# wubinzzu/NeuRec

Measured on AMD Instinct MI355X. Metric: BPR triplets/sec (LightGCN-gowalla), higher is better.
Workload: dtype f32; 1 GPU; LightGCN on synthetic gowalla-shaped interactions (U=29858, I=40981, E=813886), 3 layers, dim 64, B=1024 per GPU, adj=pre, Adam lr=0.01 reg=1e-3; global_batch=1024, parallelism=single GPU

## Files before the change

### include/neurec_hip.h

```cpp
#ifndef NEUREC_HIP_H
#define NEUREC_HIP_H

#include <stddef.h>
#include <stdint.h>

#ifdef __cplusplus
extern "C" {
#endif

#define NRHIP_OK 0
#define NRHIP_ERR_ARG 1
#define NRHIP_ERR_UNSUPPORTED 2
#define NRHIP_ERR_HIP 3
#define NRHIP_ERR_WORKSPACE 4

#define NRHIP_ABI_VERSION 4
#define NRHIP_MAX_TOPK 128

int nrhip_abi_version(void);
const char* nrhip_last_error(void);
int nrhip_device_info(int* cu_count, int* clock_khz, size_t* hbm_bytes, char* name, int name_len);


int nrhip_eval_workspace_bytes(int rows, int top_k, size_t* bytes);
// ... 38 lines not shown

int nrhip_tile_strike_plan(const int64_t* d_indptr, const int32_t* d_indices, int n_users, int cols,
                           int32_t* d_plan_user, uint32_t* d_plan_mask, int64_t* d_tile_ptr, int32_t* d_chunk_tile,
                           int64_t* d_chunk_begin, int32_t* d_counts, void* d_ws, size_t ws_bytes, void* stream);
int nrhip_score_filter_workspace_bytes(int rows, int cols, int d, size_t* bytes);
int nrhip_score_filter_kappa(int d, float* kappa);
int nrhip_score_filter_prepare_items(const float* d_Q, int64_t ldq, int cols, int d, void* d_ws, size_t ws_bytes,
                                     int max_rows, void* stream);
int nrhip_score_filter_tilemax(const float* d_P, int64_t ldp, const int32_t* d_users, int rows, int cols, int d,
                               float* d_M, int64_t mld, float* d_eps, void* d_ws, size_t ws_bytes, int max_rows,
                               void* stream);
int nrhip_score_filter_i8_workspace_bytes(int rows, int cols, int d, size_t* bytes);
int nrhip_score_filter_i8_prepare_items(const float* d_Q, int64_t ldq, int cols, int d, void* d_ws, size_t ws_bytes,
                                        int max_rows, void* stream);
int nrhip_score_filter_i8_tilemax(const float* d_P, int64_t ldp, const int32_t* d_users, int rows, int cols, int d,
                                  float* d_M, int64_t mld, float* d_eps, void* d_ws, size_t ws_bytes, int max_rows,
                                  void* stream);
int nrhip_eval_tiles_workspace_bytes(int rows, int top_k, size_t* bytes);
int nrhip_score_gemm_items_kmajor(const void* d_ws, int cols, int d, const float** qt, int* ipad);
int nrhip_eval_tiles(const float* d_M, int64_t mld, const float* d_P, int64_t ldp,
                     const void* d_gemm_ws, int d, const int32_t* d_users, int rows, int cols,
                     const int64_t* d_tr_indptr, const int32_t* d_tr_indices,
                     const int64_t* d_truth_indptr, const int32_t* d_truth_indices,
                     const int32_t* metric_ids_host, int n_metric, int top_k, float* d_out,
                     int32_t* d_flag_out, void* d_ws, size_t ws_bytes, void* stream);
int nrhip_eval_tiles_bounded_workspace_bytes(int rows, int cols, int top_k, int n_keep, size_t* bytes);
int nrhip_eval_tiles_bounded(const float* d_M, int64_t mld, const float* d_eps, int n_keep, const float* d_P,
                             int64_t ldp, const void* d_gemm_ws, int d, const int32_t* d_users, int rows, int cols,
                             const int64_t* d_tr_indptr, const int32_t* d_tr_indices,
                             const int64_t* d_truth_indptr, const int32_t* d_truth_indices,
                             const int32_t* metric_ids_host, int n_metric, int top_k, float* d_out,
                             int32_t* d_flag_out, void* d_ws, size_t ws_bytes, void* stream);

typedef struct nrhip_eval_pruned_args {
  const float* d_P; int64_t ldp;
  const float* d_Q; int64_t ldq;
  int d, cols;
  const int32_t* d_users; int n_users, batch_rows;
  const int64_t* d_tr_indptr; const int32_t* d_tr_indices;
  const int64_t* d_truth_indptr; const int32_t* d_truth_indices;
  const int32_t* d_chunk_tile; const int64_t* d_chunk_begin; int n_chunks;
  const int64_t* d_tile_ptr; const int32_t* d_plan_user; const uint32_t* d_plan_mask;
  const int32_t* d_row_of;
  const int32_t* metric_ids; int n_metric, top_k, n_keep;
  int use_filter, prepare_items;
  void* d_gemm_ws; size_t gemm_ws_bytes;
  void* d_filter_ws; size_t filter_ws_bytes;
  void* d_tiles_ws; size_t tiles_ws_bytes;
  float* d_M; int64_t mld;
  float* d_eps;
  float* d_out;
  int32_t* d_flags;
  double* d_sums;
  void* d_colsum_ws; size_t colsum_ws_bytes;
} NrhipEvalPruned;
int nrhip_eval_pruned(const NrhipEvalPruned* args, void* stream);

typedef struct nrhip_eval_redo_args {
  const NrhipEvalPruned* ev;
  int n_flagged;
  int reload_items;
  float* d_scores; int64_t lds; int slab_rows;
  int32_t* d_rows;
  int32_t* d_row_users;
  int32_t* d_count;
  float* d_fixed;
  void* d_ws; size_t ws_bytes;
} NrhipEvalRedo;
int nrhip_eval_redo(const NrhipEvalRedo* args, void* stream);

int nrhip_sample_bpr_epoch(const int64_t* d_tr_indptr, const int32_t* d_tr_indices,
                           const int32_t* d_row_of, int64_t n_inter, int n_items, int neg_num,
                           uint64_t seed, uint64_t epoch, int shuffle, int64_t out_begin,
                           int64_t out_count, int32_t* d_users_out, int32_t* d_pos_out,
                           int32_t* d_neg_out, void* stream);

int nrhip_sample_instances_epoch(const int64_t* d_seq_ptr, const int32_t* d_seq,
                                 const int64_t* d_excl_ptr, const int32_t* d_excl,
                                 const int64_t* d_inst_ptr, const int32_t* d_inst_row,
                                 const int32_t* d_row_user, int64_t n_inst, int high_order,
                                 int n_items, int neg_num, int pointwise, uint64_t seed,
                                 uint64_t epoch, int shuffle, int64_t out_begin, int64_t out_count,
                                 int32_t* d_users_out, int32_t* d_recent_out, int32_t* d_items_out,
                                 int32_t* d_neg_out, float* d_labels_out, void* stream);

int nrhip_randint_choice_batch(int high, int n_req, int64_t total, const int64_t* d_out_offsets,
                               const int64_t* d_excl_indptr, const int32_t* d_excl, int replace,
                               uint64_t seed, uint64_t call_counter, int32_t* d_out, void* stream);

int nrhip_bpr_plan(const int32_t* d_users, const int32_t* d_items, const int32_t* d_third,
                   int64_t n_total, int batch, int n_users, uint64_t* d_plan_out, void* stream);
int nrhip_bpr_mf_grad(const float* d_P, const float* d_Q, int d, int n_users,
                      const int32_t* d_users, const int32_t* d_pos, const int32_t* d_neg, int batch,
                      float reg, float* d_GP, float* d_GQ, float* d_work, float* d_loss2,
                      const uint64_t* d_plan, void* stream);
int nrhip_adam_sparse_tf(float* d_var, float* d_m, float* d_v, float* d_grad, int64_t n,
                         float alpha, float beta1, float beta2, float eps, void* stream);
int nrhip_adam_sparse_tf_lazy(float* d_var, float* d_m, float* d_v, float* d_grad, int32_t* d_last,
                              const int32_t* d_stamp, int64_t n_rows, int d, const uint64_t* d_plan,
                              int n_occ, const uint64_t* d_next_plan, int n_next_occ,
                              const float* d_alpha_tab, int t, int period, float beta1, float beta2,
                              float eps, void* stream);
int nrhip_bpr_mf_grad_lazy(const float* d_table, const float* d_m, const float* d_v,
                           const int32_t* d_last, const float* d_alpha_tab, int32_t* d_stamp, int t,
                           float beta1, float beta2, float eps, int d, int n_users,
                           const int32_t* d_users, const int32_t* d_pos, const int32_t* d_neg, int batch,
                           float reg, float* d_G, float* d_work, float* d_loss2, const uint64_t* d_plan,
                           void* stream);
int nrhip_adam_dense_tf(float* d_var, float* d_m, float* d_v, float* d_grad, int64_t n,
                        float alpha, float beta1, float beta2, float eps, int clear_grad,
                        void* stream);

int nrhip_adam_dense_tf2(float* d_var, float* d_m, float* d_v, const float* d_grad_a,
                         const float* d_grad_b, int64_t n, float alpha, float beta1, float beta2,
                         float eps, void* stream);
int nrhip_adam_dense_tf_multi(int n_tensors, float* const* d_vars_host, float* const* d_ms_host,
                              float* const* d_vs_host, float* const* d_grads_host,
                              const int64_t* sizes_host, const int32_t* clear_grad_host, float alpha,
                              float beta1, float beta2, float eps, void* stream);
int nrhip_rows_div(const int32_t* d_rows, int n_listed, int d, const float* d_src, float denom,
                   float* d_dst, void* stream);
int nrhip_rows_clear(const int32_t* d_rows, int n_listed, int d, float* d_b0, float* d_b1,
                     float* d_b2, float* d_b3, uint8_t* d_flag, void* stream);

int nrhip_spmm_plan_bytes(int64_t n_rows, int64_t nnz, size_t* bytes);
int nrhip_spmm_plan_create(const int64_t* h_indptr, int64_t n_rows, int item_rows, int item_nnz,
                           int64_t split_row, void* d_plan_buf, size_t plan_bytes, void* stream,
                           void** plan_out);
int nrhip_spmm_plan_destroy(void* plan);
int nrhip_spmm_plan_info(const void* plan, int64_t* n_work_items, int64_t* n_split_rows);
int nrhip_spmm_workspace_bytes(const void* plan, int d, size_t* bytes);
int nrhip_spmm_csr(const void* plan, const int64_t* d_indptr, const int32_t* d_indices,
                   const float* d_vals, const float* d_X, int d, float* d_Y,
                   const float* d_addend, const float* d_sum_in, float* d_sum_out, void* d_ws,
                   size_t ws_bytes, void* stream);

int nrhip_spmm_csr_masked(const void* plan, const int64_t* d_indptr, const int32_t* d_indices,
                          const float* d_vals, const float* d_X, const uint8_t* d_x_row_nonzero,
                          const uint8_t* d_y_row_wanted, int d, float* d_Y, const float* d_addend,
                          const float* d_sum_in, float* d_sum_out, void* d_ws, size_t ws_bytes,
                          void* stream);
int nrhip_spmm_blocked_plan_bytes(int64_t n_rows, int64_t nnz, int d, size_t* bytes);
int nrhip_spmm_blocked_plan_create(const int64_t* h_indptr, const int32_t* h_indices,
                                   int64_t n_rows, int64_t split_row, int d, int64_t block_bytes,
                                   int n_workgroups, int waves_per_wg, int seg_len, int r_max,
                                   int p_max, void* d_plan_buf, size_t plan_bytes, void* stream,
                                   void** plan_out);
int nrhip_spmm_blocked_plan_destroy(void* plan);
int nrhip_spmm_blocked_plan_info(const void* plan, int* n_workgroups, int* n_phases,
                                 int64_t* n_entries, int64_t* n_split);
int nrhip_spmm_blocked_tune(int gathers_in_flight);
int nrhip_spmm_blocked_tune_store(int masked_store);
int nrhip_spmm_blocked_pack(void* plan, const int32_t* d_indices, const float* d_vals, void* stream);
int nrhip_spmm_blocked(const void* plan, const int32_t* d_indices, const float* d_vals,
                       const float* d_X, float* d_Y, const float* d_addend, const float* d_sum_in,
                       float* d_sum_out, const uint8_t* d_x_row_nonzero,
                       const uint8_t* d_y_row_wanted, void* stream);
int nrhip_spmm_blocked_flagged(const void* plan, const int32_t* d_indices, const float* d_vals,
                               const float* d_X, float* d_Y, const float* d_addend,
                               const uint8_t* d_addend_row_flag, const float* d_sum_in, float* d_sum_out,
                               const uint8_t* d_x_row_nonzero, const uint8_t* d_y_row_wanted, void* stream);
int nrhip_spmm_csr_flagged(const void* plan, const int64_t* d_indptr, const int32_t* d_indices,
                           const float* d_vals, const float* d_X, int d, float* d_Y,
                           const float* d_addend, const uint8_t* d_addend_row_flag, const float* d_sum_in,
                           float* d_sum_out, void* d_ws, size_t ws_bytes, void* stream);
int nrhip_spmm_blocked_tune_addend_flag(int on);
int nrhip_spmm_plan_attach_blocked(void* plan, const void* blocked_plan, int d);

int nrhip_spmm_csr_adam(const void* plan, const int32_t* d_indices, const float* d_vals,
                        const float* d_X, int d, float* d_addend, float* d_grad_b, float* d_var,
                        float* d_m, float* d_v, float alpha, float beta1, float beta2, float eps,
                        int clear_consumed, uint8_t* d_row_flag, void* stream);
int nrhip_spmm_blocked_adam(const void* plan, const int32_t* d_indices, const float* d_vals,
                            const float* d_X, float* d_addend, float* d_grad_b, float* d_var,
                            float* d_m, float* d_v, float alpha, float beta1, float beta2,
                            float eps, int clear_consumed, uint8_t* d_row_flag, void* stream);
int nrhip_spmm_plan_has_blocked(const void* plan, int d);

int nrhip_spmm_csr_wanted_layers(const void* plan, const int32_t* d_indices, const float* d_vals,
                                 const float* d_X, int d, const float* d_sum_in,
                                 const float* d_layer_a, const float* d_layer_b, float* d_sum_out,
                                 const uint8_t* d_y_row_wanted, void* stream);
int nrhip_spmm_blocked_wanted_layers(const void* plan, const int32_t* d_indices, const float* d_vals,
                                     const float* d_X, const float* d_sum_in, const float* d_layer_a,
                                     const float* d_layer_b, float* d_sum_out,
                                     const uint8_t* d_y_row_wanted, void* stream);
int nrhip_spmm_csr_wanted_batch(const void* plan, const int32_t* d_indices, const float* d_vals,
                                const float* d_X, int d, const float* d_sum_in, const float* d_layer_a,
                                const float* d_layer_b, float* d_sum_out, const int32_t* d_users,
                                const int32_t* d_pos, const int32_t* d_neg, int batch, int n_users,
                                uint8_t* d_row_flag, int32_t* d_rows_out, void* stream);
int nrhip_spmm_blocked_wanted_batch(const void* plan, const int32_t* d_indices, const float* d_vals,
                                    const float* d_X, const float* d_sum_in, const float* d_layer_a,
                                    const float* d_layer_b, float* d_sum_out, const int32_t* d_users,
                                    const int32_t* d_pos, const int32_t* d_neg, int batch, int n_users,
                                    uint8_t* d_row_flag, int32_t* d_rows_out, void* stream);
int nrhip_spmm_plan_has_wanted(const void* plan, int d);
int nrhip_spmm_blocked_has_wanted(const void* blocked_plan);
int nrhip_spmm_plan_has_wanted_planned(const void* plan, int d);
int nrhip_spmm_blocked_has_wanted_planned(const void* blocked_plan);
int nrhip_spmm_wanted_epoch_plan_bytes(const void* plan, int d, int batch, int64_t n_batches, size_t* bytes,
                                       int* stride);
int nrhip_spmm_blocked_wanted_epoch_plan_bytes(const void* blocked_plan, int batch, int64_t n_batches, size_t* bytes,
                                               int* stride);
int nrhip_spmm_wanted_epoch_plan(const void* plan, int d, const int64_t* d_indptr, const uint64_t* d_plans, int batch,
                                 int64_t n_batches, int last_len, void* d_sched, size_t sched_bytes, void* stream);
int nrhip_spmm_blocked_wanted_epoch_plan(const void* blocked_plan, const int64_t* d_indptr, const uint64_t* d_plans,
                                         int batch, int64_t n_batches, int last_len, void* d_sched, size_t sched_bytes,
                                         void* stream);
int nrhip_spmm_csr_wanted_planned(const void* plan, const int32_t* d_indices, const float* d_vals, const float* d_X,
                                  int d, const float* d_sum_in, const float* d_layer_a, const float* d_layer_b,
                                  float* d_sum_out, const int32_t* d_users, const int32_t* d_pos, const int32_t* d_neg,
                                  int batch, int n_users, uint8_t* d_row_flag, int32_t* d_rows_out,
                                  const void* d_batch_sched, int stride, void* stream);
int nrhip_spmm_blocked_wanted_planned(const void* blocked_plan, const int32_t* d_indices, const float* d_vals,
                                      const float* d_X, const float* d_sum_in, const float* d_layer_a,
                                      const float* d_layer_b, float* d_sum_out, const int32_t* d_users,
                                      const int32_t* d_pos, const int32_t* d_neg, int batch, int n_users,
                                      uint8_t* d_row_flag, int32_t* d_rows_out, const void* d_batch_sched, int stride,
                                      void* stream);

int nrhip_spmm_csr_carry(const void* plan, const int64_t* d_indptr, const int32_t* d_indices, const float* d_vals,
                         const float* d_X, const float* d_X2, int x_split, int d, float* d_Yv, int has_carry,
                         const uint8_t* d_row_mask, void* stream);
int nrhip_spmm_chunks_finish(const int32_t* d_first_vrow, int64_t n_rows, const float* d_Yv, int d, float* d_Y,
                             const float* d_addend, const float* d_sum_in, float* d_sum_out,
                             const uint8_t* d_row_mask, void* stream);

int nrhip_partials_sum_rows(const float* d_parts, int world, int64_t n_rows, int d, float* d_Y, const float* d_addend,
                            const float* d_sum_in, float* d_sum_out, const uint8_t* d_row_mask, void* stream);

int nrhip_spmm_csr_rows(const int64_t* d_indptr, const int32_t* d_indices, const float* d_vals,
                        const float* d_X, int d, const int32_t* d_rows, int n_listed, float* d_Y,
                        const float* d_addend, const float* d_sum_in, float* d_sum_out,
                        void* stream);

int nrhip_lightgcn_bpr_grad(const float* d_Esum, const float* d_E0, int n_users, int d,
                            int n_layers, const int32_t* d_users, const int32_t* d_pos,
                            const int32_t* d_neg, int batch, float reg, float* d_Gstar,
                            float* d_Greg, float* d_work, float* d_loss2, const uint64_t* d_plan,
                            void* stream);

int nrhip_lightgcn_bpr_grad_h(const float* d_Esum, const float* d_E0, int n_users, int d,
                              int n_layers, const int32_t* d_users, const int32_t* d_pos,
                              const int32_t* d_neg, int batch, float reg, float* d_H,
                              float* d_Greg, float* d_work, float* d_loss2, const uint64_t* d_plan,
                              void* stream);

int nrhip_lightgcn_mark_batch(const int32_t* d_users, const int32_t* d_pos, const int32_t* d_neg,
                              int batch, int n_users, int32_t* d_rows_out, uint8_t* d_row_flag,
                              void* stream);

typedef struct nrhip_lightgcn_buffers {
  const void* plan;
  const void* plan_t;
  const int64_t* indptr;  const int32_t* indices;  const float* vals;
  const int64_t* indptr_t; const int32_t* indices_t; const float* vals_t;
  float* E0; float* m; float* v;
  float* Ea; float* Eb; float* Esum; float* Esum_rows;
  float* Gstar; float* Greg; float* H; float* Ga; float* Gb;
  int32_t* batch_rows;
  uint8_t* row_flag;
  float* terms;
  void* spmm_ws; size_t spmm_ws_bytes;
  int n_users; int n_nodes; int d; int n_layers; int max_batch;
  float reg;
} nrhip_lightgcn_buffers;
int nrhip_lightgcn_ctx_create(const nrhip_lightgcn_buffers* bufs, void** ctx_out);
int nrhip_lightgcn_ctx_destroy(void* ctx);
int nrhip_lightgcn_step(void* ctx, const int32_t* d_users, const int32_t* d_pos,
                        const int32_t* d_neg, int batch, const uint64_t* d_plan, float alpha,
                        float beta1, float beta2, float eps, float* d_loss2, void* stream);
int nrhip_lightgcn_step_planned(void* ctx, const int32_t* d_users, const int32_t* d_pos, const int32_t* d_neg,
                                int batch, const uint64_t* d_plan, const void* d_hop_sched, int hop_stride,
                                float alpha, float beta1, float beta2, float eps, float* d_loss2, void* stream);

int nrhip_lightgcn_step_colshard_fwd(void* ctx, const int32_t* d_users, const int32_t* d_pos, const int32_t* d_neg,
                                     int batch, float* d_partials, void* stream);
int nrhip_lightgcn_step_colshard_fwd_planned(void* ctx, const int32_t* d_users, const int32_t* d_pos,
                                             const int32_t* d_neg, int batch, const void* d_hop_sched, int hop_stride,
                                             float* d_partials, void* stream);
int nrhip_lightgcn_step_colshard_bwd(void* ctx, const int32_t* d_users, const int32_t* d_pos, const int32_t* d_neg,
                                     int batch, const uint64_t* d_plan, const float* d_given, float alpha,
                                     float beta1, float beta2, float eps, float* d_loss2, void* stream);
int nrhip_lightgcn_partial_dots(const float* d_Esum, const float* d_E0, int n_users, int d, int n_layers,
                                const int32_t* d_users, const int32_t* d_pos, const int32_t* d_neg, int batch,
                                float* d_out, void* stream);
int nrhip_partials_sum(const float* d_parts, int world, int n, float* d_given, void* stream);
int nrhip_lightgcn_bpr_grad_given(const float* d_Esum, const float* d_E0, int n_users, int d, int n_layers,
                                  const int32_t* d_users, const int32_t* d_pos, const int32_t* d_neg, int batch,
                                  float reg, float* d_Gstar, float* d_Greg, float* d_work, float* d_loss2,
                                  const uint64_t* d_plan, const float* d_given, int divided, void* stream);
int nrhip_lightgcn_step_grad(void* ctx, const int32_t* d_users, const int32_t* d_pos,
                             const int32_t* d_neg, int batch, const uint64_t* d_plan,
                             float* d_loss2, float* d_grad_out, void* stream);
int nrhip_lightgcn_step_apply(void* ctx, float* d_grad, float alpha, float beta1, float beta2,
                              float eps, void* stream);

typedef struct nrhip_mf_buffers {
  float* P; float* Q; float* mP; float* vP; float* mQ; float* vQ; float* GP; float* GQ;
  float* terms;
  int n_users; int n_items; int d; int max_batch;
  float reg;
  int32_t* last; int32_t* stamp; const float* alpha_tab; int alpha_len; int lazy_period;
  int32_t* tw; int32_t* inb;
} nrhip_mf_buffers;
// ... 643 lines not shown
```

### neurec_amd/_lib.py

```python
import ctypes as C
import os

from . import build as _build

_HERE = os.path.dirname(os.path.abspath(__file__))
LIB_PATH = os.path.join(_HERE, "libneurec_hip.so")

ERR_ARG, ERR_UNSUPPORTED, ERR_HIP, ERR_WORKSPACE = 1, 2, 3, 4


class NeuRecHipError(RuntimeError):
    """A HIP runtime failure or workspace error reported by the native library."""


def _load():
    if not os.path.isfile(LIB_PATH):
        raise ImportError(
            "libneurec_hip.so is not built (expected at %s). Run `python -m neurec_amd.build` "
            "(needs hipcc; the engine has no CPU fallback)." % LIB_PATH)
    if os.path.isfile(_build.STAMP) and not _build.is_current() and not os.environ.get("NEUREC_ALLOW_STALE_LIB"):
        raise ImportError(
            "libneurec_hip.so was built from other sources than neurec_amd/csrc now holds (digest in %s differs). "
            "Run `python -m neurec_amd.build`; NEUREC_ALLOW_STALE_LIB=1 loads it anyway." % _build.STAMP)
    try:
# ... 160 lines not shown
    _fields_ = [(n, C.c_void_p) for n in (
        "UI", "IU", "IL", "LI", "W", "b", "h", "G_UI", "G_IU", "G_IL", "G_LI", "G_W", "G_b", "G_h", "flag_UI",
        "flag_IU", "flag_IL", "flag_LI", "users", "recents", "items", "third", "keys", "contrib", "scal", "delta",
        "partial", "loss2")] + \
        [(n, C.c_int) for n in ("n_users", "n_items", "d", "w", "L", "batch", "pairwise", "loss_kind")] + \
        [("reg_mf", C.c_float), ("reg_w", C.c_float)]


class FpmcplusScoresArgs(C.Structure):
    _fields_ = [(n, C.c_void_p) for n in (
        "UI", "IU", "IL", "LI", "W", "b", "h", "last", "users", "c", "p", "out")] + [("ld", C.c_int64)] + \
        [(n, C.c_int) for n in ("n_users", "n_items", "d", "w", "L", "batch")]


class TransrecStepArgs(C.Structure):
    _fields_ = [(n, C.c_void_p) for n in (
        "P", "Q", "b", "T", "G_P", "G_Q", "G_b", "G_T", "flag_P", "flag_Q", "flag_b", "users", "recent", "items",
        "third", "keys", "scal", "partial", "loss2")] + \
        [(n, C.c_int) for n in ("n_users", "n_items", "d", "batch", "pairwise", "loss_kind")] + [("reg", C.c_float)]


GRU4REC_MAX_LAYERS = 3


class Gru4recWeights(C.Structure):
    _fields_ = [(n, C.c_void_p * GRU4REC_MAX_LAYERS) for n in ("Wg", "bg", "Wc", "bc")] + [("width", C.c_int * GRU4REC_MAX_LAYERS),
                                                                          ("n_layers", C.c_int), ("hidden_act", C.c_int)]


class Gru4recStepArgs(C.Structure):
    _fields_ = [(n, C.c_void_p) for n in ("Ein", "Q", "b")] + [("w", Gru4recWeights)] + \
        [(n, C.c_void_p) for n in ("G_Ein", "G_Q", "G_b")] + \
        [(n, C.c_void_p * GRU4REC_MAX_LAYERS) for n in ("G_Wg", "G_bg", "G_Wc", "G_bc", "state", "h_new")] + \
        [(n, C.c_void_p) for n in ("X", "Y", "keys", "ws", "loss2")] + \
        [(n, C.c_int) for n in ("n_items", "batch", "final_act", "loss_kind")] + [("reg", C.c_float)]


SIGNATURES = {
    "nrhip_device_info": [C.POINTER(i32), C.POINTER(i32), psz, C.c_char_p, i32],
    "nrhip_eval_workspace_bytes": [i32, i32, psz],
    "nrhip_mask_train": [p, i64, p, i32, i32, p, p, p],
    "nrhip_eval_scores": [p, i64, i32, i32, p, p, p, C.POINTER(i32), i32, i32, p, p, p, p, sz, p],
    "nrhip_eval_any_k_workspace_bytes": [i32, i32, i32, psz],
    "nrhip_eval_scores_any_k": [p, i64, i32, i32, p, p, p, C.POINTER(i32), i32, i32, p, p, p, sz, p],
    "nrhip_arg_topk": [p, i64, i32, i32, i32, p, p, p, sz, p],
    "nrhip_colsum_workspace_bytes": [i32, i32, psz],
    "nrhip_colsum_f64": [p, i64, i32, i32, p, p, sz, p],
    "nrhip_score_gemm_workspace_bytes": [i32, i32, i32, psz],
    "nrhip_score_gemm_prepare_items": [p, i64, i32, i32, p, sz, p],
    "nrhip_score_tilemax": [p, i64, p, i32, i32, i32, p, p, p, i64, p, sz, p],
    "nrhip_tile_strike_plan": [p, p, i32, i32, p, p, p, p, p, p, p, sz, p],
    "nrhip_score_tilemax_fix": [p, i64, i32, i32, p, p, i32, p, p, p, p, i32, i32, p, i64, p, sz, p],
    "nrhip_score_filter_workspace_bytes": [i32, i32, i32, psz],
    "nrhip_score_filter_kappa": [i32, p],
    "nrhip_score_filter_prepare_items": [p, i64, i32, i32, p, sz, i32, p],
    "nrhip_score_filter_tilemax": [p, i64, p, i32, i32, i32, p, i64, p, p, sz, i32, p],
    "nrhip_score_filter_i8_workspace_bytes": [i32, i32, i32, psz],
    "nrhip_score_filter_i8_prepare_items": [p, i64, i32, i32, p, sz, i32, p],
    "nrhip_score_filter_i8_tilemax": [p, i64, p, i32, i32, i32, p, i64, p, p, sz, i32, p],
    "nrhip_eval_tiles_workspace_bytes": [i32, i32, psz],
    "nrhip_eval_tiles": [p, i64, p, i64, p, i32, p, i32, i32, p, p, p, p, p, i32, i32, p, p, p, sz, p],
    "nrhip_eval_tiles_bounded_workspace_bytes": [i32, i32, i32, i32, psz],
    "nrhip_eval_tiles_bounded": [p, i64, p, i32, p, i64, p, i32, p, i32, i32, p, p, p, p, p, i32, i32, p, p, p, sz, p],
    "nrhip_eval_pruned": [C.POINTER(EvalPrunedArgs), p],
    "nrhip_eval_redo": [C.POINTER(EvalRedoArgs), p],
    "nrhip_vae_step": [C.POINTER(VaeStepArgs), p, i32, f32, f32, f32, u64, i32, i32, p],
    "nrhip_score_gemm_items_kmajor": [p, i32, i32, p, p],
    "nrhip_score_gemm": [p, i64, p, i32, i32, i32, p, i64, p, sz, p],
    "nrhip_sample_bpr_epoch": [p, p, p, i64, i32, i32, u64, u64, i32, i64, i64, p, p, p, p],
    "nrhip_sample_instances_epoch": [p, p, p, p, p, p, p, i64, i32, i32, i32, i32, u64, u64, i32, i64, i64, p, p, p, p, p, p],
    "nrhip_randint_choice_batch": [i32, i32, i64, p, p, p, i32, u64, u64, p, p],
    "nrhip_bpr_plan": [p, p, p, i64, i32, i32, p, p],
    "nrhip_bpr_mf_grad": [p, p, i32, i32, p, p, p, i32, f32, p, p, p, p, p, p],
    "nrhip_adam_sparse_tf": [p, p, p, p, i64, f32, f32, f32, f32, p],
    "nrhip_adam_dense_tf": [p, p, p, p, i64, f32, f32, f32, f32, i32, p],
    "nrhip_adam_dense_tf2": [p, p, p, p, p, i64, f32, f32, f32, f32, p],
    "nrhip_adam_dense_tf_multi": [i32, p, p, p, p, p, p, f32, f32, f32, f32, p],
    "nrhip_rows_div": [p, i32, i32, p, f32, p, p],
    "nrhip_rows_clear": [p, i32, i32, p, p, p, p, p, p],
    "nrhip_spmm_plan_bytes": [i64, i64, psz],
    "nrhip_spmm_plan_create": [p, i64, i32, i32, i64, p, sz, p, C.POINTER(p)],
    "nrhip_spmm_plan_destroy": [p],
    "nrhip_spmm_plan_info": [p, C.POINTER(i64), C.POINTER(i64)],
    "nrhip_spmm_workspace_bytes": [p, i32, psz],
    "nrhip_spmm_csr": [p, p, p, p, p, i32, p, p, p, p, p, sz, p],
    "nrhip_spmm_csr_masked": [p, p, p, p, p, p, p, i32, p, p, p, p, p, sz, p],
    "nrhip_spmm_csr_carry": [p, p, p, p, p, p, i32, i32, p, i32, p, p],
    "nrhip_spmm_chunks_finish": [p, i64, p, i32, p, p, p, p, p, p],
    "nrhip_partials_sum_rows": [p, i32, i64, i32, p, p, p, p, p, p],
    "nrhip_spmm_csr_rows": [p, p, p, p, i32, p, i32, p, p, p, p, p],
    "nrhip_lightgcn_mark_batch": [p, p, p, i32, i32, p, p, p],
    "nrhip_lightgcn_bpr_grad": [p, p, i32, i32, i32, p, p, p, i32, f32, p, p, p, p, p, p],
    "nrhip_lightgcn_bpr_grad_h": [p, p, i32, i32, i32, p, p, p, i32, f32, p, p, p, p, p, p],
    "nrhip_lightgcn_ctx_create": [C.POINTER(LightGCNBuffers), C.POINTER(p)],
    "nrhip_lightgcn_ctx_destroy": [p],
    "nrhip_lightgcn_step": [p, p, p, p, i32, p, f32, f32, f32, f32, p, p],
    "nrhip_lightgcn_step_grad": [p, p, p, p, i32, p, p, p, p],
    "nrhip_lightgcn_step_apply": [p, p, f32, f32, f32, f32, p],
    "nrhip_mf_ctx_create": [C.POINTER(MFBuffers), C.POINTER(p)],
    "nrhip_mf_ctx_destroy": [p],
    "nrhip_mf_step": [p, p, p, p, i32, p, p, i32, i32, f32, f32, f32, f32, p, p],
    "nrhip_mf_flush": [p, i32, f32, f32, f32, p],
    "nrhip_ngcf_ctx_create": [C.POINTER(NGCFBuffers), C.POINTER(p)],
    "nrhip_ngcf_ctx_destroy": [p],
    "nrhip_ngcf_forward": [p, C.c_uint64, C.c_uint64, i32, p],
    "nrhip_ngcf_step": [p, p, p, p, i32, p, C.c_uint64, C.c_uint64, i32, f32, f32, f32, f32, p, p],
    "nrhip_mf_steps": [p, p, p, p, i64, i32, p, i32, p, f32, f32, f32, p, p, p],
    "nrhip_loss_reduce_steps": [p, i32, i32, i32, f32, p, p],
    "nrhip_lightgcn_step_colshard_fwd": [p, p, p, p, i32, p, p],
    "nrhip_lightgcn_step_colshard_fwd_planned": [p, p, p, p, i32, p, i32, p, p],
    "nrhip_lightgcn_step_planned": [p, p, p, p, i32, p, p, i32, f32, f32, f32, f32, p, p],
    "nrhip_lightgcn_step_colshard_bwd": [p, p, p, p, i32, p, p, f32, f32, f32, f32, p, p],
    "nrhip_lightgcn_partial_dots": [p, p, i32, i32, i32, p, p, p, i32, p, p],
    "nrhip_partials_sum": [p, i32, i32, p, p],
    "nrhip_lightgcn_bpr_grad_given": [p, p, i32, i32, i32, p, p, p, i32, f32, p, p, p, p, p, p, i32, p],
    "nrhip_gemm_workspace_bytes": [i32, i32, i32, p],
    "nrhip_gemm_kmajor": [p, i64, p, i64, i32, i32, i32, p, i64, i32, p, i32, i32, p, sz, p],
    "nrhip_gemm_f32": [p, i64, i32, p, i64, i32, i32, i32, i32, p, i64, i32, p, i32, i32, p, sz, p],
    "nrhip_transpose2d": [p, i64, i32, i32, p, i64, p],
    "nrhip_ngcf_wide_forward": [C.POINTER(NGCFWideBuffers), i32, u64, u64, p],
    "nrhip_ngcf_wide_step": [C.POINTER(NGCFWideBuffers), p, p, p, i32, p, i32, u64, u64, f32, f32, f32, f32, p, p],
    "nrhip_vae_bag_fwd": [p, p, p, i32, i32, p, p, i32, f32, p, u64, u64, p, p, p],
    "nrhip_act_bwd": [p, p, i64, i32, p, p],
    "nrhip_vae_sample": [p, i32, i32, p, f32, u64, u64, p, p, p, p],
    "nrhip_vae_sample_bwd": [p, p, p, i32, i32, f32, p, p],
    "nrhip_vae_softmax_dlogits": [p, i64, i32, i32, p, p, p, p, p],
    "nrhip_vae_dwq0_wide": [p, p, p, i32, i32, p, p, p, p],
    "nrhip_colsum_rows": [p, i64, i32, i32, p, p, sz, p],
    "nrhip_ew_mul": [p, i64, p, i64, i64, i32, p, i64, p],
    "nrhip_ngcf_act_fwd": [p, p, i64, i64, i32, i32, f32, p, i32, u64, u64, i32, p, i64, p, i64, p],
    "nrhip_ngcf_act_bwd": [p, i64, p, i64, p, i64, p, p, i64, p, i64, i32, f32, p, p, p],
    "nrhip_lrelu_drop_fwd": [p, i64, i64, i32, i32, f32, p, i32, u64, u64, i32, i32, p, i64, p, i64, p],
    "nrhip_lrelu_drop_bwd": [p, i64, p, i64, p, i64, p, i64, i32, f32, i32, p, p],
    "nrhip_edge_dropout": [p, i64, f32, p, i32, u64, u64, p, p],
    "nrhip_gather_f32": [p, p, i64, p, p],
    "nrhip_ngcf_mix_bwd": [p, p, i64, p, p, i64, i64, i32, i32, p, p, p],
    "nrhip_route_batch": [p, p, p, i32, i32, i32, i32, i32, p, p, p, p, p, i32, p],
    "nrhip_route_owner_keys": [p, p, i32, p, p, i32, i32, i32, p, p, p],
    "nrhip_sort_u64_segments": [p, p, p, i32, i32, p],
    "nrhip_route_epoch": [p, p, p, i64, i32, i32, i32, i32, i32, i32, p, p, p, p, p, p, p, p],
    "nrhip_route_epoch_owner_keys": [p, p, p, i64, p, p, i32, i32, p, p, p, i32, i32, i64, p, p, p],
    "nrhip_bpr_mf_step_fused": [p, p, p, p, p, p, i32, f32, f32, f32, i32, i32, i32, p, p, p, i32, f32, p, p, p,
                                i32, p, i32, i32, p],
    "nrhip_bpr_mf_fused_flush": [p, p, p, p, p, i32, f32, f32, f32, i32, i64, p],
    "nrhip_adam_sparse_tf_lazy": [p, p, p, p, p, p, i64, i32, p, i32, p, i32, p, i32, i32, f32, f32, f32, p],
    "nrhip_bpr_mf_grad_lazy": [p, p, p, p, p, p, i32, f32, f32, f32, i32, i32, p, p, p, i32, f32, p, p, p,
                               p, p],
    "nrhip_ngcf_workspace_bytes": [i64, psz],
    "nrhip_ngcf_layer_fwd": [p, p, p, p, p, p, i64, i32, f32, p, i32, u64, u64, i32, p, p, i64, p],
    "nrhip_ngcf_layer_bwd": [p, p, p, p, p, p, i64, i32, f32, p, p, i64, p, p, p, p, p, p, p, p, p,
                             p, sz, p],
    "nrhip_spmm_blocked_plan_bytes": [i64, i64, i32, psz],
    "nrhip_spmm_blocked_pack": [p, p, p, p],
    "nrhip_spmm_blocked_plan_create": [p, p, i64, i64, i32, i64, i32, i32, i32, i32, i32, p, sz, p,
                                       C.POINTER(p)],
    "nrhip_spmm_blocked_plan_destroy": [p],
    "nrhip_spmm_blocked_plan_info": [p, p, p, p, p],
    "nrhip_spmm_blocked_tune": [i32],
    "nrhip_spmm_blocked_tune_store": [i32],
    "nrhip_spmm_blocked": [p, p, p, p, p, p, p, p, p, p, p],
    "nrhip_spmm_blocked_flagged": [p, p, p, p, p, p, p, p, p, p, p, p],
    "nrhip_spmm_csr_flagged": [p, p, p, p, p, i32, p, p, p, p, p, p, sz, p],
    "nrhip_spmm_blocked_tune_addend_flag": [i32],
    "nrhip_spmm_plan_attach_blocked": [p, p, i32],
    "nrhip_spmm_plan_has_blocked": [p, i32],
    "nrhip_spmm_plan_has_wanted": [p, i32],
    "nrhip_spmm_blocked_has_wanted": [p],
    "nrhip_spmm_plan_has_wanted_planned": [p, i32],
    "nrhip_spmm_blocked_has_wanted_planned": [p],
    "nrhip_spmm_wanted_epoch_plan_bytes": [p, i32, i32, i64, psz, C.POINTER(i32)],
    "nrhip_spmm_blocked_wanted_epoch_plan_bytes": [p, i32, i64, psz, C.POINTER(i32)],
    "nrhip_spmm_wanted_epoch_plan": [p, i32, p, p, i32, i64, i32, p, sz, p],
    "nrhip_spmm_blocked_wanted_epoch_plan": [p, p, p, i32, i64, i32, p, sz, p],
    "nrhip_spmm_csr_wanted_planned": [p, p, p, p, i32, p, p, p, p, p, p, p, i32, i32, p, p, p, i32, p],
    "nrhip_spmm_blocked_wanted_planned": [p, p, p, p, p, p, p, p, p, p, p, i32, i32, p, p, p, i32, p],
    "nrhip_spmm_csr_wanted_layers": [p, p, p, p, i32, p, p, p, p, p, p],
    "nrhip_spmm_blocked_wanted_layers": [p, p, p, p, p, p, p, p, p, p],
    "nrhip_spmm_csr_wanted_batch": [p, p, p, p, i32, p, p, p, p, p, p, p, i32, i32, p, p, p],
    "nrhip_spmm_blocked_wanted_batch": [p, p, p, p, p, p, p, p, p, p, p, i32, i32, p, p, p],
    "nrhip_spmm_csr_adam": [p, p, p, p, i32, p, p, p, p, p, f32, f32, f32, f32, i32, p, p],
    "nrhip_spmm_blocked_adam": [p, p, p, p, p, p, p, p, p, f32, f32, f32, f32, i32, p, p],
    "nrhip_vae_encode": [p, p, p, i32, i32, i32, p, p, p, p, p, p, i32, f32, p, p, f32, u64, u64,
                         p, p, p, p, p, p, p, p, p],
    "nrhip_add_row_bias": [p, i64, i32, i32, p, p],
    "nrhip_vae_workspace_bytes": [i32, i32, psz],
    "nrhip_vae_decoder_loss_grad": [p, i64, i32, i32, i32, p, p, p, p, p, p, p, p, p, p, p, sz, p],
    "nrhip_vae_decoder_fused_workspace_bytes": [i32, i32, psz],
    "nrhip_vae_decoder_fused": [i32, i32, i32, p, p, p, p, p, p, p, p, p, p, p, sz, p, p],
    "nrhip_vae_mid_backward": [i32, i32, i32, i32, f32, p, p, p, p, p, p, p, p, p, p, p, p, p, p,
                               p, p, p, p],
    "nrhip_vae_dwq0": [p, p, p, i32, i32, p, p, p, p],
    "nrhip_axpy": [f32, p, p, i64, p],
    "nrhip_sumsq_accumulate": [p, i64, p, p],
    "nrhip_mean_f32": [p, i32, p, p],
    "nrhip_mean2_f32": [p, p, i32, p, p],
    "nrhip_pairwise_mf_grad": [p, p, i32, i32, p, p, p, i32, f32, i32, p, p, p, p, p, p],
    "nrhip_pointwise_mf_grad": [p, p, i32, i32, p, p, p, i32, f32, i32, p, p, p, p, p, p],
    "nrhip_gather_u8": [p, p, i64, p, p],
    "nrhip_mark_rows": [p, i32, i32, p, p],
    "nrhip_sort_u64": [p, i32, p],
    "nrhip_rows_sum_sorted": [p, i32, p, i32, p, i64, p, p],
    "nrhip_rows_sum_sorted2": [p, i32, p, i32, p, i64, p, p, i64, p, p],
    "nrhip_optimizer_rows_tf": [i32, p, p, p, p, p, i64, i32, f32, f32, f32, f32, p],
    "nrhip_optimizer_dense_tf": [i32, p, p, p, p, i64, f32, f32, f32, f32, i32, p],
    "nrhip_rows_gather": [p, i32, i32, p, p, i64, p],
    "nrhip_rows_gather_ld": [p, i32, i32, p, i64, p, i64, p],
    "nrhip_rows_gather2": [p, i32, i32, p, i64, p, i64, p, i64, p, i64, p],
    "nrhip_rows_scatter_add": [p, i32, i32, p, i64, p, p],
    "nrhip_scale": [p, f32, p, i64, p],
    "nrhip_add": [p, p, p, i64, p],
    "nrhip_div_scalar": [p, f32, p, i64, p],
    "nrhip_add2d": [p, i64, p, i64, p, i64, i64, i32, p],
    "nrhip_copy2d": [p, i64, p, i64, i64, i32, p],
    "nrhip_wrmf_chunk_plan": [p, i32, p, p, C.POINTER(i32)],
    "nrhip_wrmf_workspace_bytes": [i32, i32, psz],
    "nrhip_wrmf_gram": [p, i32, i32, p, p, sz, p],
    "nrhip_wrmf_solve": [p, p, i32, p, i32, p, i32, f32, f32, p, p, i32, p, p, sz, p],
    "nrhip_itemknn_workspace_bytes": [i32, i32, i32, psz],
    "nrhip_itemknn_build": [p, p, p, p, p, p, p, p, i32, i32, i32, f32, f32, f32, i32, i32, p, p, p, p, p, p, p, sz, p],
    "nrhip_itemknn_score": [p, i32, p, p, p, i32, i32, p, p, p, p, i64, p],
    "nrhip_fism_step": [C.POINTER(FismStepArgs), p],
    "nrhip_fism_user_factors": [p, p, i32, p, i32, f32, p, i32, p, i64, p],
    "nrhip_nais_step": [C.POINTER(NaisStepArgs), p],
    "nrhip_nais_scores": [C.POINTER(NaisScoresArgs), p],
    "nrhip_fpmc_step": [C.POINTER(FpmcStepArgs), p],
    "nrhip_fpmc_user_factors": [p, p, i32, i32, i32, p, p, i32, p, i64, p],
    "nrhip_fossil_step": [C.POINTER(FossilStepArgs), p],
    "nrhip_fossil_user_factors": [p, p, i32, i32, p, p, p, p, i32, i32, f32, p, i32, p, i64, p],
    "nrhip_hrm_step": [C.POINTER(HrmStepArgs), p],
    "nrhip_hrm_user_factors": [p, p, i32, i32, i32, i32, i32, i32, p, p, i32, p, i64, p],
    "nrhip_npe_step": [C.POINTER(NpeStepArgs), p],
    "nrhip_npe_user_factors": [p, p, i32, i32, i32, i32, p, p, i32, p, i64, p],
    "nrhip_npe_item_factors": [p, i32, i32, p, p],
    "nrhip_fpmcplus_step": [C.POINTER(FpmcplusStepArgs), p],
    "nrhip_fpmcplus_scores": [C.POINTER(FpmcplusScoresArgs), p],
    "nrhip_transrec_step": [C.POINTER(TransrecStepArgs), p],
    "nrhip_transrec_queries": [p, p, p, i32, i32, i32, p, p, i32, p, i64, p],
    "nrhip_transrec_scores": [p, i64, p, p, i32, i32, i32, p, i64, p],
    "nrhip_gru4rec_workspace_floats": [i32, C.POINTER(i32), i32, psz],
    "nrhip_gru4rec_step": [C.POINTER(Gru4recStepArgs), p],
    "nrhip_gru4rec_advance": [C.POINTER(p), C.POINTER(p), C.POINTER(i32), i32, i32, p, p],
    "nrhip_gru4rec_user_states": [p, p, i32, i32, p, p, i32, p, C.POINTER(Gru4recWeights), p, i64, p],
    "nrhip_gru4rec_scores": [p, i64, p, p, i32, i32, i32, i32, p, i64, p],
}

for _name, _args in SIGNATURES.items():
    _fn = getattr(lib, _name)
    _fn.argtypes = _args
    _fn.restype = C.c_int
lib.nrhip_abi_version.argtypes = []
lib.nrhip_abi_version.restype = C.c_int
lib.nrhip_last_error.argtypes = []
lib.nrhip_last_error.restype = C.c_char_p

EXPORTED = sorted(list(SIGNATURES) + ["nrhip_abi_version", "nrhip_last_error"])

ABI_VERSION = 4
if lib.nrhip_abi_version() != ABI_VERSION:
    raise ImportError("libneurec_hip.so ABI version %d, expected %d"
                      % (lib.nrhip_abi_version(), ABI_VERSION))


def last_error():
    return lib.nrhip_last_error().decode("utf-8", "replace")


def check(rc):
    if rc == 0:
        return
    msg = last_error()
    if rc == ERR_ARG:
        raise ValueError(msg)
    if rc == ERR_UNSUPPORTED:
        raise NotImplementedError(msg)
    raise NeuRecHipError("libneurec_hip status %d: %s" % (rc, msg))


def call(name, *args):
    check(getattr(lib, name)(*args))


def is_stale():
    return not _build.is_current()
```

### neurec_amd/build.py

```python
import hashlib
import os
import subprocess
import sys
from concurrent.futures import ThreadPoolExecutor

HERE = os.path.dirname(os.path.abspath(__file__))
ROOT = os.path.dirname(HERE)
CSRC = os.path.join(HERE, "csrc")
OBJ_DIR = os.path.join(CSRC, "_obj")
LIB_PATH = os.path.join(HERE, "libneurec_hip.so")
STAMP = os.path.join(OBJ_DIR, "sources.sha256")

SOURCES = ["eval_select.hip", "score_gemm.hip", "sampler.hip", "spmm.hip", "bpr.hip", "adam.hip",
           "step.hip", "dense.hip", "vae.hip", "spmm_blocked.hip", "route.hip", "gemm.hip", "vae_wide.hip", "ngcf_wide.hip", "vae_fused.hip",
           "score_bf16.hip", "score_i8.hip", "eval_pipeline.hip", "wrmf.hip", "itemknn.hip", "fism.hip", "nais.hip", "fpmc.hip", "fossil.hip", "hrm.hip",
           "npe.hip", "fpmcplus.hip", "transrec.hip", "gru4rec.hip"]
FILE_FLAGS = {"score_i8.hip": ["-mllvm", "-amdgpu-mfma-vgpr-form"]}
EXP_SOURCES = ["experiments/gather_experiments.hip"]
EXP_LIB_PATH = os.path.join(HERE, "libneurec_exp.so")
HEADERS = ["nr_core.h", "nr_common.h", "history_common.h", "spmm_blocked_plan.h", "spmm_wanted_plan.h"]

HIPCC = os.environ.get("HIPCC", "/opt/rocm/bin/hipcc")
FLAGS = ["-O3", "--offload-arch=gfx950", "-std=c++17", "-fPIC", "-ffp-contract=off",
         "-munsafe-fp-atomics", "-Wall", "-Wno-unused-function",
         "-I", CSRC, "-I", os.path.join(ROOT, "include")] + os.environ.get("NEUREC_HIPCC_EXTRA", "").split()


def _existing_sources():
    return [s for s in SOURCES if os.path.isfile(os.path.join(CSRC, s))]


def _digest():
    h = hashlib.sha256()
    for name in _existing_sources() + HEADERS:
        with open(os.path.join(CSRC, name), "rb") as f:
            h.update(name.encode())
            h.update(f.read())
    with open(os.path.join(ROOT, "include", "neurec_hip.h"), "rb") as f:
        h.update(f.read())
    h.update(" ".join(f.replace(ROOT, "<root>") for f in FLAGS).encode())
    h.update(repr(sorted(FILE_FLAGS.items())).encode())
    return h.hexdigest()


def is_current():
    if not (os.path.isfile(LIB_PATH) and os.path.isfile(STAMP)):
        return False
    with open(STAMP) as f:
        return f.read().strip() == _digest()


def build_extension(force=False, verbose=True):
    if not force and is_current():
        return LIB_PATH
    os.makedirs(OBJ_DIR, exist_ok=True)
    srcs = _existing_sources()

    def compile_one(src):
        obj = os.path.join(OBJ_DIR, src.replace(".hip", ".o"))
        cmd = [HIPCC] + FLAGS + FILE_FLAGS.get(src, []) + ["-c", os.path.join(CSRC, src), "-o", obj]
        r = subprocess.run(cmd, capture_output=True, text=True)
        if r.returncode != 0 and FILE_FLAGS.get(src):
            r2 = subprocess.run([HIPCC] + FLAGS + ["-c", os.path.join(CSRC, src), "-o", obj], capture_output=True, text=True)
            if r2.returncode == 0:
                sys.stderr.write("neurec_amd.build: %s compiled WITHOUT %s (not accepted by this hipcc)\n"
                                 % (src, " ".join(FILE_FLAGS[src])))
                r = r2
        return src, obj, r

    objs = []
    with ThreadPoolExecutor(max_workers=min(8, len(srcs))) as ex:
        for src, obj, r in ex.map(compile_one, srcs):
            if r.returncode != 0:
                raise RuntimeError("hipcc failed on %s:\n%s\n%s" % (src, r.stdout, r.stderr))
            if verbose and r.stderr.strip():
                sys.stderr.write(r.stderr)
            objs.append(obj)
    cmd = [HIPCC, "--offload-arch=gfx950", "-shared", "-fPIC", "-o", LIB_PATH] + objs
    r = subprocess.run(cmd, capture_output=True, text=True)
    if r.returncode != 0:
        raise RuntimeError("link failed:\n%s\n%s" % (r.stdout, r.stderr))
    with open(STAMP, "w") as f:
        f.write(_digest())
    if verbose:
        print("built", LIB_PATH)
    return LIB_PATH


def build_experiments(verbose=True):
    os.makedirs(OBJ_DIR, exist_ok=True)
    objs = []
    for src in EXP_SOURCES:
        obj = os.path.join(OBJ_DIR, os.path.basename(src).replace(".hip", ".o"))
        r = subprocess.run([HIPCC] + FLAGS + ["-c", os.path.join(CSRC, src), "-o", obj],
                           capture_output=True, text=True)
        if r.returncode != 0:
            raise RuntimeError("hipcc failed on %s:\n%s\n%s" % (src, r.stdout, r.stderr))
        objs.append(obj)
    r = subprocess.run([HIPCC, "--offload-arch=gfx950", "-shared", "-fPIC", "-o", EXP_LIB_PATH] + objs +
                       ["-L", HERE, "-lneurec_hip", "-Wl,-rpath,$ORIGIN"], capture_output=True, text=True)
    if r.returncode != 0:
        raise RuntimeError("link failed:\n%s\n%s" % (r.stdout, r.stderr))
    if verbose:
        print("built", EXP_LIB_PATH)
    return EXP_LIB_PATH


if __name__ == "__main__":
    build_extension(force="--force" in sys.argv)
    if "--experiments" in sys.argv:
        build_experiments()
```

### neurec_amd/csrc/spmm_blocked.hip

```cpp
#include "nr_common.h"
#include "spmm_blocked_plan.h"
#include "spmm_wanted_plan.h"
#include <algorithm>
#include <new>
#include <cstdlib>
#include <initializer_list>
#include <vector>

namespace {

using nr_plan::kMaxLdsBytes;
using nr_plan::blocked_plan_bytes;
static_assert((int)nr_plan::kOk == NR_OK && (int)nr_plan::kErrArg == NR_ERR_ARG &&
              (int)nr_plan::kErrUnsupported == NR_ERR_UNSUPPORTED, "the planner returns the C ABI's status codes");

struct BlockedPlan : nr_plan::PlanArrays<int4> {
  int64_t n_rows, nnz, n_ent, n_cmb;
  int n_wg, n_phases;
  int seg, r_max, p_max, waves, d;
  const int32_t* pk_from_idx;
  const float* pk_from_val;
  int nnz_cap, ent_cap;
  int colmask_ok;
  int wanted_ok, w_ent_cap, w_nnz_cap, w_bitmap_words;
  int ww_ok, ww_ent_cap;
  int ww_lds_slots;
  int wp_ok, n_hubs;
  nr_wplan::SlotProfile wp_profile;
};


enum { kStorePlain = 0, kStoreNt = 1, kStoreWt = 2 };
typedef float nr_f32x4 __attribute__((ext_vector_type(4)));
typedef unsigned int nr_u32x4 __attribute__((ext_vector_type(4)));

template <int ST>
__device__ __forceinline__ void row_store(float4* __restrict__ Y, uint32_t y_bytes, int64_t o, float4 y) {
  if constexpr (ST == kStoreNt) {
    __builtin_nontemporal_store(nr_f32x4{y.x, y.y, y.z, y.w}, (nr_f32x4*)(Y + o));
  } else if constexpr (ST == kStoreWt) {
    const __amdgpu_buffer_rsrc_t rs = __builtin_amdgcn_make_buffer_rsrc((void*)Y, 0, (int)y_bytes, 0x00020000);
    __builtin_amdgcn_raw_buffer_store_b128(nr_u32x4{__float_as_uint(y.x), __float_as_uint(y.y), __float_as_uint(y.z),
                                                    __float_as_uint(y.w)},
                                           rs, (int)(uint32_t)(o * 16), 0, 16);
  } else {
    Y[o] = y;
  }
}


struct AdamEpilogue {
  float4* var; float4* m; float4* v; const float4* grad_b;
  float alpha, omb1, omb2, eps;
  float4* addend_rw; float4* grad_b_rw; uint8_t* flag_rw;
};


constexpr int kRowBits = 0x7FFFFFFF;
constexpr int kRowUnflagged = (int)0x80000000u;

template <bool MASKED, bool ADAM, int LPR>
__device__ __forceinline__ void blocked_epilogue(const float4* s_acc, int r0, int nr, int tid, int nthreads,
                                                 float4* __restrict__ Y, const float4* __restrict__ addend,
                                                 const float4* sum_in, float4* sum_out,
                                                 const uint8_t* __restrict__ row_mask, const AdamEpilogue& ad,
                                                 const int32_t* s_rows = nullptr) {
  for (int i = tid; i < nr * LPR; i += nthreads) {
    const int rw = s_rows ? s_rows[i / LPR] : r0 + i / LPR;
    const int row = rw & kRowBits;
    if constexpr (MASKED) {
      if (row_mask && row_mask[row] == 0) continue;
    }
    const int64_t o = (int64_t)row * LPR + (i & (LPR - 1));
    float4 y = s_acc[i];
    const bool flagged = rw >= 0;
    float4 hv = make_float4(0.f, 0.f, 0.f, 0.f);
    if (addend) {
      if (flagged) hv = addend[o];
      y.x = __fadd_rn(y.x, hv.x); y.y = __fadd_rn(y.y, hv.y);
      y.z = __fadd_rn(y.z, hv.z); y.w = __fadd_rn(y.w, hv.w);
    }
    if constexpr (ADAM) {
      float4 gb = make_float4(0.f, 0.f, 0.f, 0.f);
      if (flagged) gb = ad.grad_b[o];
      if (ad.addend_rw) {
        const float4 zero = make_float4(0.f, 0.f, 0.f, 0.f);
        if (hv.x != 0.f || hv.y != 0.f || hv.z != 0.f || hv.w != 0.f) ad.addend_rw[o] = zero;
        if (gb.x != 0.f || gb.y != 0.f || gb.z != 0.f || gb.w != 0.f) ad.grad_b_rw[o] = zero;
        if ((i & (LPR - 1)) == 0 && ad.flag_rw && flagged) ad.flag_rw[row] = 0;
      }
      float4 w = ad.var[o], mm = ad.m[o], vv = ad.v[o];
      nr::adam_dense_tf(__fadd_rn(y.x, gb.x), w.x, mm.x, vv.x, ad.alpha, ad.omb1, ad.omb2, ad.eps);
      nr::adam_dense_tf(__fadd_rn(y.y, gb.y), w.y, mm.y, vv.y, ad.alpha, ad.omb1, ad.omb2, ad.eps);
      nr::adam_dense_tf(__fadd_rn(y.z, gb.z), w.z, mm.z, vv.z, ad.alpha, ad.omb1, ad.omb2, ad.eps);
      nr::adam_dense_tf(__fadd_rn(y.w, gb.w), w.w, mm.w, vv.w, ad.alpha, ad.omb1, ad.omb2, ad.eps);
      ad.var[o] = w; ad.m[o] = mm; ad.v[o] = vv;
      continue;
    }
    if (Y) {
      if constexpr (LPR == 16 && !MASKED) {
        if ((uint64_t)o * 16 + 16 <= 0xFFFFFFFFull) row_store<kStoreWt>(Y, 0xFFFFFFFFu, o, y);
        else Y[o] = y;
      } else {
        Y[o] = y;
      }
    }
    if (sum_out) {
      const float4 si = sum_in[o];
      sum_out[o] = make_float4(__fadd_rn(si.x, y.x), __fadd_rn(si.y, y.y), __fadd_rn(si.z, y.z),
                               __fadd_rn(si.w, y.w));
    }
  }
}

#ifdef NR_BLK_TIMELINE
__device__ unsigned long long g_blk_dbg[4096 * 24];
#define NR_BLK_STAMP(i) do { if (threadIdx.x == 0 && blockIdx.x < 4096) g_blk_dbg[blockIdx.x * 24 + (i)] = wall_clock64(); } while (0)
#define NR_BLK_WSTAMP() do { if ((threadIdx.x & 63) == 0 && blockIdx.x < 4096) g_blk_dbg[blockIdx.x * 24 + 8 + (threadIdx.x >> 6)] = wall_clock64(); } while (0)
extern "C" int nrhip_exp_blk_timeline(unsigned long long* h_out) {
  if (hipDeviceSynchronize() != hipSuccess) return NR_ERR_HIP;
  return hipMemcpyFromSymbol(h_out, HIP_SYMBOL(g_blk_dbg), sizeof(unsigned long long) * 4096 * 24) == hipSuccess ? NR_OK : NR_ERR_HIP;
}
#else
#define NR_BLK_STAMP(i) do {} while (0)
#define NR_BLK_WSTAMP() do {} while (0)
#endif

template <bool MASKED, int kWaves, int kG, int D, bool ADAM = false>
__global__ __launch_bounds__(kWaves* NR_WAVE) void spmm_blocked_kernel(
    const int32_t* __restrict__ wg_row0, const int32_t* __restrict__ wg_nrows,
    const int32_t* __restrict__ wg_ent_off, const int32_t* __restrict__ wg_cmb_off,
    const int4* __restrict__ ent, const int4* __restrict__ cmb, int n_phases,
    const int32_t* __restrict__ indices, const float* __restrict__ vals,
    const float4* __restrict__ X, float4* __restrict__ Y, const float4* __restrict__ addend,
    const float4* sum_in, float4* sum_out, const uint8_t* __restrict__ col_mask,
    const uint8_t* __restrict__ row_mask, int kRMax, AdamEpilogue ad, const int32_t* __restrict__ row_of,
    int kPMax, const uint8_t* __restrict__ addend_flag) {
  constexpr int LPR = D / 4;
  constexpr int GPW = NR_WAVE / LPR;
  constexpr int kGroups = kWaves * GPW;
  constexpr int CL = LPR < 16 ? LPR : 16;
  constexpr int IPL = 16 / CL;
  static_assert(kG % IPL == 0, "broadcast component must be a compile-time index");
  extern __shared__ float4 s_acc[];
  const int tid = threadIdx.x, lane = tid & 63, wave = tid >> 6;
  const int c = lane & (LPR - 1), g = lane / LPR, gbase = lane & ~(LPR - 1);
  const int wg = blockIdx.x;
  NR_BLK_STAMP(0);
  const int r0 = wg_row0[wg], nr = wg_nrows[wg];
  int32_t* s_rows = (int32_t*)(s_acc + (size_t)(kRMax + kPMax) * LPR);
  const uint8_t* fl = ADAM ? ad.flag_rw : addend_flag;
  for (int i = tid; i < nr; i += kWaves * NR_WAVE) {
    int row = row_of[r0 + i];
    if (fl && fl[row] == 0) row |= kRowUnflagged;
    s_rows[i] = row;
  }
  for (int i = tid; i < nr * LPR; i += kWaves * NR_WAVE) s_acc[i] = make_float4(0.f, 0.f, 0.f, 0.f);
  __syncthreads();
  NR_BLK_STAMP(1);
  const int32_t* eoff = wg_ent_off + (int64_t)wg * (n_phases + 1);
  const int32_t* coff = wg_cmb_off + (int64_t)wg * (n_phases + 1);
  for (int k = 0; k < n_phases; ++k) {
    const int e0 = eoff[k], e1 = eoff[k + 1];
    int ei = e0 + wave * GPW + g;
    int4 cur = make_int4(0, 0, 0, 0);
    if (ei < e1) cur = ent[ei];
    int cur_idx[IPL];
    float cur_val[IPL];
#pragma unroll
    for (int i = 0; i < IPL; ++i) {
      cur_idx[i] = 0;
      cur_val[i] = 0.f;
      if (c < CL && c * IPL + i < cur.y) {
        cur_idx[i] = indices[(uint32_t)cur.z + c * IPL + i];
        cur_val[i] = vals[(uint32_t)cur.z + c * IPL + i];
      }
    }
    int cur_want = 1;
    if constexpr (MASKED) {
      if (row_mask && ei < e1) cur_want = row_mask[cur.w];
    }
    for (int base = e0 + wave * GPW; base < e1; base += kGroups) {
      const bool live = ei < e1;
      const int ein = ei + kGroups;
      int4 nxt = make_int4(0, 0, 0, 0);
      if (ein < e1) nxt = ent[ein];
      const int slot = cur.x;
      int len = cur.y;
      const uint32_t begin = (uint32_t)cur.z;
      if constexpr (MASKED) {
        if (cur_want == 0) len = 0;
      }
      int nxt_want = 1;
      float4 acc = make_float4(0.f, 0.f, 0.f, 0.f);
      if (live && slot < kRMax) acc = s_acc[slot * LPR + c];
      int maxlen = len;
#pragma unroll
      for (int m = LPR; m < NR_WAVE; m <<= 1) maxlen = max(maxlen, __shfl_xor(maxlen, m, NR_WAVE));
      maxlen = __builtin_amdgcn_readfirstlane(maxlen);
      int nxt_idx[IPL];
      float nxt_val[IPL];
#pragma unroll
      for (int i = 0; i < IPL; ++i) { nxt_idx[i] = 0; nxt_val[i] = 0.f; }
      int ch_idx[IPL];
      float ch_val[IPL];
#pragma unroll
      for (int i = 0; i < IPL; ++i) { ch_idx[i] = 0; ch_val[i] = 0.f; }
      for (int k0 = 0; k0 < maxlen || k0 == 0; k0 += 16) {
        int my_idx[IPL];
        float my_val[IPL];
#pragma unroll
        for (int i = 0; i < IPL; ++i) {
          my_idx[i] = k0 == 0 ? cur_idx[i] : ch_idx[i];
          my_val[i] = k0 == 0 ? cur_val[i] : ch_val[i];
          if constexpr (MASKED) {
            if (col_mask && c < CL && k0 + c * IPL + i < len && col_mask[my_idx[i]] == 0)
              my_idx[i] = -1;
          }
        }
        const int nn = min(16, maxlen - k0);
        for (int t0 = 0; t0 < nn || (k0 == 0 && t0 == 0); t0 += kG) {
          float a[kG];
          float4 x[kG];
          bool on[kG];
#pragma unroll
          for (int u = 0; u < kG; ++u) {
            const int src = gbase | (((t0 + u) & 15) / IPL);
            const int col = __shfl(my_idx[u % IPL], src, NR_WAVE);
            a[u] = __shfl(my_val[u % IPL], src, NR_WAVE);
            on[u] = k0 + t0 + u < len;
            if constexpr (MASKED) {
              on[u] = on[u] && col >= 0;
              x[u] = make_float4(0.f, 0.f, 0.f, 0.f);
              if (on[u]) x[u] = X[(int64_t)col * LPR + c];
            } else {
              x[u] = make_float4(0.f, 0.f, 0.f, 0.f);
              if (t0 + u < nn) x[u] = X[(int64_t)max(col, 0) * LPR + c];
            }
          }
          if (t0 == 0 && k0 + 16 < maxlen) {
#pragma unroll
            for (int i = 0; i < IPL; ++i) {
              ch_idx[i] = 0;
              ch_val[i] = 0.f;
              if (c < CL && k0 + 16 + c * IPL + i < len) {
                ch_idx[i] = indices[begin + k0 + 16 + c * IPL + i];
                ch_val[i] = vals[begin + k0 + 16 + c * IPL + i];
              }
            }
          }
          if (k0 == 0 && t0 == 0) {
#pragma unroll
            for (int i = 0; i < IPL; ++i)
              if (c < CL && c * IPL + i < nxt.y) {
                nxt_idx[i] = indices[(uint32_t)nxt.z + c * IPL + i];
                nxt_val[i] = vals[(uint32_t)nxt.z + c * IPL + i];
              }
            if constexpr (MASKED) {
              if (row_mask && ein < e1) nxt_want = row_mask[nxt.w];
            }
          }
#pragma unroll
          for (int u = 0; u < kG; ++u)
            if (on[u]) {
              acc.x = __fadd_rn(acc.x, __fmul_rn(a[u], x[u].x));
              acc.y = __fadd_rn(acc.y, __fmul_rn(a[u], x[u].y));
              acc.z = __fadd_rn(acc.z, __fmul_rn(a[u], x[u].z));
              acc.w = __fadd_rn(acc.w, __fmul_rn(a[u], x[u].w));
            }
        }
      }
      if (live) s_acc[slot * LPR + c] = acc;
      cur = nxt;
#pragma unroll
      for (int i = 0; i < IPL; ++i) { cur_idx[i] = nxt_idx[i]; cur_val[i] = nxt_val[i]; }
      cur_want = nxt_want;
      ei = ein;
    }
    NR_BLK_WSTAMP();
    const int c0 = coff[k], c1 = coff[k + 1];
    if (c1 > c0) {
      __syncthreads();
      NR_BLK_STAMP(2);
      for (int ci = c0 + wave * GPW + g; ci < c1; ci += kGroups) {
        const int4 cm = cmb[ci];
        float4 acc = s_acc[cm.x * LPR + c];
        for (int s = 0; s < cm.z; ++s) {
          const float4 p = s_acc[(cm.y + s) * LPR + c];
          acc.x = __fadd_rn(acc.x, p.x); acc.y = __fadd_rn(acc.y, p.y);
          acc.z = __fadd_rn(acc.z, p.z); acc.w = __fadd_rn(acc.w, p.w);
        }
        s_acc[cm.x * LPR + c] = acc;
      }
    }
    __syncthreads();
  }
  NR_BLK_STAMP(3);
  blocked_epilogue<MASKED, ADAM, LPR>(s_acc, r0, nr, tid, kWaves * NR_WAVE, Y, addend, sum_in, sum_out,
                                      row_mask, ad, s_rows);
  NR_BLK_STAMP(4);
}



struct LayerChain { const float4* a; const float4* b; };
__device__ __forceinline__ int4 zero_int4() { return make_int4(0, 0, 0, 0); }

__device__ __forceinline__ float4 chain_sum(float4 si, const LayerChain& ch, int64_t o) {
  if (ch.a) {
    const float4 t = ch.a[o];
    si = make_float4(__fadd_rn(si.x, t.x), __fadd_rn(si.y, t.y), __fadd_rn(si.z, t.z), __fadd_rn(si.w, t.w));
  }
  if (ch.b) {
    const float4 t = ch.b[o];
    si = make_float4(__fadd_rn(si.x, t.x), __fadd_rn(si.y, t.y), __fadd_rn(si.z, t.z), __fadd_rn(si.w, t.w));
  }
  return si;
}

template <int ST = kStorePlain>
__device__ __forceinline__ void masked_row_out(float4 y, int64_t o, const float4* __restrict__ addend,
                                               bool addend_row_nonzero, float4* __restrict__ Y,
                                               const float4* sum_in, float4* sum_out,
                                               const LayerChain* chain = nullptr, uint32_t y_bytes = 0) {
  if (addend) {
    float4 av = make_float4(0.f, 0.f, 0.f, 0.f);
    if (addend_row_nonzero) av = addend[o];
    y.x = __fadd_rn(y.x, av.x); y.y = __fadd_rn(y.y, av.y);
    y.z = __fadd_rn(y.z, av.z); y.w = __fadd_rn(y.w, av.w);
  }
  if (Y) row_store<ST>(Y, y_bytes, o, y);
  if (sum_out) {
    float4 si = sum_in[o];
    if (chain) si = chain_sum(si, *chain, o);
    sum_out[o] = make_float4(__fadd_rn(si.x, y.x), __fadd_rn(si.y, y.y), __fadd_rn(si.z, y.z),
                             __fadd_rn(si.w, y.w));
  }
}

template <int ST = kStorePlain>
__device__ __forceinline__ void staged_walk(const int4* s_ent, const int2* s_iv, int ne, int r0,
                                            const float4* __restrict__ X, float4* __restrict__ Y,
                                            const float4* __restrict__ addend, const float4* sum_in,
                                            float4* sum_out, float4* s_part, int kRMax, int wave,
                                            int g, int c, LayerChain chain = LayerChain{nullptr, nullptr},
                                            uint32_t y_bytes = 0) {
  constexpr int RS = 16, LPR = 16, GPW = 4, kGroups = 64;
  constexpr int kQ = 4;
  struct Round { float4 x[kQ]; float4 pre; int off, n, slot, owner; bool first, last, live, valid; };
  const float4* pre_src = addend ? addend : (sum_in ? sum_in : X);
  int ibase = wave * GPW, it0 = 0, imax = 0;
  int4 ids = make_int4(0, 0, 0, 0);
  bool ihas = ibase < ne;
  auto open = [&]() {
    ids = make_int4(0, 0, 0, 0);
    if (ibase + g < ne) ids = s_ent[ibase + g];
    int m = ids.y;
#pragma unroll
    for (int sh = LPR; sh < NR_WAVE; sh <<= 1) m = max(m, __shfl_xor(m, sh, NR_WAVE));
    imax = __builtin_amdgcn_readfirstlane(m);
  };
  auto issue = [&](Round& r) {
    r.valid = ihas;
    r.off = ids.z + it0;
    r.n = ihas ? ids.y - it0 : 0;
    r.slot = ids.x;
    r.owner = ids.w;
    r.first = it0 == 0;
    r.live = ihas && ibase + g < ne;
    r.last = ihas && it0 + kQ >= imax;
#pragma unroll
    for (int u = 0; u < kQ; ++u) {
      int col = s_iv[u < r.n ? r.off + u : 0].x;
      if (u >= r.n) col = 0;
      r.x[u] = X[(int64_t)col * RS + c];
    }
    const bool want_pre = r.last && r.live && r.slot < kRMax && !((r.owner >> 29) & 1) &&
                          (!addend || ((r.owner >> 30) & 1));
    r.pre = pre_src[(want_pre ? ((int64_t)r0 + (r.owner & 0xFFFFFF)) * RS : 0) + c];
    if (r.last) {
      ibase += kGroups;
      it0 = 0;
      ihas = ibase < ne;
      if (ihas) open();
    } else if (ihas) {
      it0 += kQ;
    }
  };
  float4 acc = make_float4(0.f, 0.f, 0.f, 0.f);
  auto retire = [&](const Round& r) {
    if (r.first) acc = make_float4(0.f, 0.f, 0.f, 0.f);
    float a[kQ];
#pragma unroll
    for (int u = 0; u < kQ; ++u) a[u] = __int_as_float(s_iv[u < r.n ? r.off + u : 0].y);
#pragma unroll
    for (int u = 0; u < kQ; ++u) {
      const float4 t = make_float4(__fadd_rn(acc.x, __fmul_rn(a[u], r.x[u].x)),
                                   __fadd_rn(acc.y, __fmul_rn(a[u], r.x[u].y)),
                                   __fadd_rn(acc.z, __fmul_rn(a[u], r.x[u].z)),
                                   __fadd_rn(acc.w, __fmul_rn(a[u], r.x[u].w)));
      if (u < r.n) acc = t;
    }
    if (r.last && r.live && !((r.owner >> 29) & 1)) {
      if (r.slot < kRMax) {
        const int64_t o = ((int64_t)r0 + (r.owner & 0xFFFFFF)) * RS + c;
        float4 y = acc;
        if (addend) {
          float4 av = make_float4(0.f, 0.f, 0.f, 0.f);
          if ((r.owner >> 30) & 1) av = r.pre;
          y.x = __fadd_rn(y.x, av.x); y.y = __fadd_rn(y.y, av.y);
          y.z = __fadd_rn(y.z, av.z); y.w = __fadd_rn(y.w, av.w);
        }
        if (Y) row_store<ST>(Y, y_bytes, o, y);
        if (sum_out) {
          float4 si = r.pre;
          if (addend) si = sum_in[o];
          si = chain_sum(si, chain, o);
          sum_out[o] = make_float4(__fadd_rn(si.x, y.x), __fadd_rn(si.y, y.y), __fadd_rn(si.z, y.z),
                                   __fadd_rn(si.w, y.w));
        }
      } else {
        s_part[(size_t)(r.slot - kRMax) * RS + c] = acc;
      }
    }
  };
  Round q0, q1, q2;
// ... 499 lines not shown
      const int32_t prev = i > 0 ? (int32_t)(keys[i - 1] >> 32) : -1;
      if (row != prev) k = nr_wplan::sort_key(indptr[row + 1] - indptr[row], row);
    }
    s_key[i] = k;
  }
  __syncthreads();
  for (int k = 2; k <= n2; k <<= 1)
    for (int j = k >> 1; j > 0; j >>= 1) {
      for (int i = tid; i < n2; i += kWpThreads) {
        const int p = i ^ j;
        if (p > i) {
          const uint32_t x = s_key[i], y = s_key[p];
          if ((x > y) == ((i & k) == 0)) { s_key[i] = y; s_key[p] = x; }
        }
      }
      __syncthreads();
    }
  const int per = n2 / kWpThreads;
  int sum = 0, hubs = 0, rows = 0;
  for (int j = tid * per; j < (tid + 1) * per; ++j) {
    const uint32_t k = s_key[j];
    s_off[j] = sum;
    if (k != ~0u) {
      const int32_t row = nr_wplan::key_row(k);
      const int64_t len = indptr[row + 1] - indptr[row];
      sum += nr_wplan::slots_of(len);
      hubs += nr_wplan::is_hub(len) ? 1 : 0;
      ++rows;
    }
  }
  s_scan[tid] = sum;
  if (hubs) atomicAdd(&s_nhub, hubs);
  if (rows) atomicAdd(&s_nrows, rows);
  __syncthreads();
  for (int off = 1; off < kWpThreads; off <<= 1) {
    const int v = tid >= off ? s_scan[tid - off] : 0;
    __syncthreads();
    s_scan[tid] += v;
    __syncthreads();
  }
  const int before = s_scan[tid] - sum, total = s_scan[kWpThreads - 1];
  for (int j = tid * per; j < (tid + 1) * per; ++j) s_off[j] += before;
  __syncthreads();
  const int cap = stride - 1;
  const int n_hub_rows = s_nhub;
  for (int j = 0; j < n_hub_rows; ++j) {
    const int32_t row = nr_wplan::key_row(s_key[j]);
    const int64_t first = indptr[row], len = indptr[row + 1] - first;
    int lo = 0, hi = n_hubs - 1;
    while (lo < hi) {
      const int mid = (lo + hi) >> 1;
      if (ww_hub[mid].x < row) lo = mid + 1; else hi = mid;
    }
    const int part0 = ww_hub[lo].y, sl = nr_wplan::slots_of(len), o = s_off[j];
    for (int s = tid; s < sl; s += kWpThreads)
      if (o + s < cap) {
        const nr_plan::Int4 it = nr_wplan::item_of(row, first, len, s, lo, part0);
        items[1 + o + s] = make_int4(it.x, it.y, it.z, it.w);
      }
  }
  for (int j = n_hub_rows + tid; j < n2; j += kWpThreads) {
    const uint32_t k = s_key[j];
    if (k == ~0u) continue;
    const int32_t row = nr_wplan::key_row(k);
    const int64_t first = indptr[row], len = indptr[row + 1] - first;
    const int sl = nr_wplan::slots_of(len), o = s_off[j];
    for (int s = 0; s < sl; ++s)
      if (o + s < cap) {
        const nr_plan::Int4 it = nr_wplan::item_of(row, first, len, s, 0, 0);
        items[1 + o + s] = make_int4(it.x, it.y, it.z, it.w);
      }
  }
  for (int i = 1 + min(total, cap) + tid; i < stride; i += kWpThreads) items[i] = make_int4(0, 0, 0, -1);
  if (tid == 0) items[0] = make_int4(min(total, cap), s_nrows, 0, 0);
}

__global__ __launch_bounds__(16 * NR_WAVE) void spmm_wanted_planned_kernel(
    const int4* __restrict__ items, const int4* __restrict__ ww_hub, float* ww_part, unsigned* ww_cnt,
    const int32_t* __restrict__ indices, const float* __restrict__ vals, const float4* __restrict__ X, WantedEpi ep,
    BatchLists bl) {
  constexpr int RS = 16;
  __shared__ float4 s_part[16 * RS];
  const int tid = threadIdx.x, lane = tid & 63, wave = tid >> 6;
  const int c = lane & 15, g = lane >> 4;
  const int wg = blockIdx.x;
  const int n_items = items[0].x;
  ww_publish_batch(bl, wg, (int)gridDim.x, tid);
  if (wg * 16 >= n_items) return;
  const int idx = wg * 16 + wave;
  const int4 it = idx < n_items ? items[1 + idx] : make_int4(0, 0, 0, -1);
  const int slot = it.x, len = it.y & 255, hub = (it.y >> 8) - 1, row = it.w;
  const int64_t o = (int64_t)row * RS + c;
  const bool head = slot < 0 && ((-slot - 1) & 15) == 0;
  int4 hd = zero_int4();
  WwPre pre;
  if (row >= 0) {
    int col = 0;
    float val = 0.f;
    if (lane < len) {
      col = indices[(uint32_t)it.z + lane];
      val = vals[(uint32_t)it.z + lane];
    }
    if (hub >= 0) hd = ww_hub[hub];
    const float4 carry = ww_sublist_sum(col, val, len, X, c, g,
                                        [&]() { pre = ww_prefetch(ep, (slot == 0 || head) ? o : (int64_t)c); });
    if (g == 0) ww_sublist_out(carry, slot, o, c, pre, ep, s_part + wave * RS, ww_part);
  }
  __builtin_amdgcn_fence(__ATOMIC_RELEASE, "workgroup");
  __builtin_amdgcn_s_waitcnt(0);
  __syncthreads();
  if (row < 0) return;
  if (head && g == 0) {
    const int ns = (-slot - 1) >> 4;
    float4 acc = make_float4(0.f, 0.f, 0.f, 0.f);
    for (int sgm = 0; sgm < ns; ++sgm) {
      const float4 q = s_part[(wave + sgm) * RS + c];
      acc.x = __fadd_rn(acc.x, q.x); acc.y = __fadd_rn(acc.y, q.y);
      acc.z = __fadd_rn(acc.z, q.z); acc.w = __fadd_rn(acc.w, q.w);
    }
    ww_sublist_out(acc, 0, o, c, pre, ep, nullptr, nullptr);
  }
  if (hub >= 0) ww_chunk_done(hub, hd, ww_cnt, ww_part, ep, lane, c, g);
}

size_t wanted_lds_bytes(const BlockedPlan* p) {
  return (size_t)p->p_max * 256 + 2 * (size_t)p->w_ent_cap * 16 + (size_t)p->w_bitmap_words * 4 +
         (size_t)p->w_nnz_cap * 8;
}
int ww_bitmap_words(const BlockedPlan* p) { return (int)((p->n_rows + 127) / 128 * 4); }
size_t ww_lds_bytes(const BlockedPlan* p) {
  return (size_t)p->ww_lds_slots * 256 + (size_t)p->ww_ent_cap * 16 + (size_t)ww_bitmap_words(p) * 4 + 16;
}
size_t colmask_lds_bytes(const BlockedPlan* p) {
  return (size_t)p->p_max * 256 + (size_t)p->ent_cap * 16 + (size_t)p->nnz_cap * 8;
}

int launch_wanted_wave(const BlockedPlan* p, const int32_t* d_indices, const float* d_vals, const float* d_X,
                       float* d_Y, const float* d_addend, const float* d_sum_in, float* d_sum_out,
                       const uint8_t* d_y_row_wanted, LayerChain chain, BatchLists bl, hipStream_t st) {
  hipLaunchKernelGGL(spmm_wanted_wave_kernel, dim3((unsigned)p->n_wg), dim3(16 * NR_WAVE), ww_lds_bytes(p), st,
                     p->ww_off, p->ww_choff, p->ww_ent, p->ww_gch, p->ww_hub, p->ww_lcoff, p->ww_lcmb, p->ww_part,
                     p->ww_cnt, d_indices, d_vals, (const float4*)d_X,
                     WantedEpi{(float4*)d_Y, (const float4*)d_addend, (const float4*)d_sum_in,
                               (float4*)d_sum_out, chain},
                     d_y_row_wanted, bl, ww_bitmap_words(p), p->ww_ent_cap, p->ww_lds_slots);
  NR_LAUNCH_CHECK();
  return NR_OK;
}

int s_gathers_in_flight = 8;
constexpr int kMaskedStoreDefault = kStoreWt;
int s_addend_by_flag = 1;
int s_masked_store = kMaskedStoreDefault;

__global__ __launch_bounds__(256) void row_order_pack_kernel(const uint32_t* __restrict__ src, const uint32_t* __restrict__ dst,
                                                             int64_t n_rows, const int32_t* __restrict__ indices,
                                                             const float* __restrict__ vals, int32_t* __restrict__ pk_idx,
                                                             float* __restrict__ pk_val) {
  const int c = threadIdx.x & 15;
  for (int64_t k = (int64_t)blockIdx.x * 16 + (threadIdx.x >> 4); k < n_rows; k += (int64_t)gridDim.x * 16) {
    const uint32_t s0 = src[k], d0 = dst[k], len = dst[k + 1] - d0;
    for (uint32_t j = c; j < len; j += 16) {
      pk_idx[d0 + j] = indices[s0 + j];
      pk_val[d0 + j] = vals[s0 + j];
    }
  }
}

static hipError_t allow_plan_lds(const BlockedPlan* p) {
  hipError_t e = hipSuccess;
  auto allow = [&](const void* fn, size_t lds) {
    if (e == hipSuccess) e = hipFuncSetAttribute(fn, hipFuncAttributeMaxDynamicSharedMemorySize, (int)lds);
  };
  const size_t lds = (size_t)(p->r_max + p->p_max) * p->d * 4 + (size_t)p->r_max * 4;
#define NR_ALLOW(DD)                                                                                                         \
  allow((const void*)spmm_blocked_kernel<false, 16, 8, DD>, lds); allow((const void*)spmm_blocked_kernel<true, 16, 8, DD>, lds); \
  allow((const void*)spmm_blocked_kernel<false, 16, 4, DD>, lds); allow((const void*)spmm_blocked_kernel<true, 16, 4, DD>, lds); \
  allow((const void*)spmm_blocked_kernel<false, 8, 8, DD>, lds); allow((const void*)spmm_blocked_kernel<true, 8, 8, DD>, lds);   \
  allow((const void*)spmm_blocked_kernel<false, 8, 4, DD>, lds); allow((const void*)spmm_blocked_kernel<true, 8, 4, DD>, lds)
  if (p->d == 16) { NR_ALLOW(16); } else if (p->d == 32) { NR_ALLOW(32); }
  else if (p->d == 64) {
    NR_ALLOW(64);
    allow((const void*)spmm_blocked_kernel<false, 16, 8, 64, true>, lds);
  }
  else if (p->d == 128) { NR_ALLOW(128); } else { NR_ALLOW(256); }
#undef NR_ALLOW
  if (p->wanted_ok) allow((const void*)spmm_wanted_rows_kernel, wanted_lds_bytes(p));
  if (p->ww_ok) allow((const void*)spmm_wanted_wave_kernel, ww_lds_bytes(p));
  if (p->colmask_ok)
    for (const void* fn : {(const void*)spmm_staged_masked_kernel<true, false>,
                           (const void*)spmm_staged_masked_kernel<true, false, kStoreNt>,
                           (const void*)spmm_staged_masked_kernel<true, false, kStoreWt>,
                           (const void*)spmm_staged_masked_kernel<false, true>,
                           (const void*)spmm_staged_masked_kernel<true, true>})
      allow(fn, colmask_lds_bytes(p));
  return e;
}

}

extern "C" {

int nrhip_spmm_blocked_plan_bytes(int64_t n_rows, int64_t nnz, int d, size_t* bytes) {
  NR_REQUIRE(bytes && n_rows >= 0 && nnz >= 0, NR_ERR_ARG, "spmm_blocked_plan_bytes: bad arguments");
  (void)d;
  *bytes = blocked_plan_bytes(n_rows, nnz);
  return NR_OK;
}

int nrhip_spmm_blocked_plan_create(const int64_t* h_indptr, const int32_t* h_indices,
                                   int64_t n_rows, int64_t split_row, int d, int64_t block_bytes,
                                   int n_workgroups, int waves_per_wg, int seg_len, int r_max,
                                   int p_max, void* d_plan_buf, size_t plan_bytes, void* stream,
                                   void** plan_out) {
  nr_plan::Options opt;
  nr_plan::Error err;
  int rc = nr_plan::resolve_options(d, waves_per_wg, seg_len, r_max, p_max, block_bytes, split_row, n_rows, &opt, &err);
  NR_REQUIRE(rc == NR_OK, rc, "%s", err.msg.c_str());
  NR_REQUIRE(h_indptr && h_indices && d_plan_buf && plan_out && n_rows > 0, NR_ERR_ARG,
             "spmm_blocked_plan_create: bad arguments");
  const int64_t nnz = h_indptr[n_rows] - h_indptr[0];
  NR_REQUIRE(h_indptr[0] == 0 && nnz < ((int64_t)1 << 32), NR_ERR_UNSUPPORTED,
             "spmm_blocked: indptr must start at 0 and hold < 2^32 non-zeros");
  const size_t need_bytes = blocked_plan_bytes(n_rows, nnz);
  NR_REQUIRE(plan_bytes >= need_bytes, NR_ERR_WORKSPACE,
             "spmm_blocked_plan_create: plan buffer %zu < %zu bytes", plan_bytes, need_bytes);
  int n_wg = n_workgroups;
  if (n_wg <= 0) {
    int dev = 0;
    hipDeviceProp_t prop;
    NR_CHECK_HIP(hipGetDevice(&dev));
    NR_CHECK_HIP(hipGetDeviceProperties(&prop, dev));
    n_wg = prop.multiProcessorCount * (16 / opt.waves);
  }
  rc = nr_plan::choose_workgroup_count(n_wg, n_workgroups <= 0, n_rows, &opt, &err);
  NR_REQUIRE(rc == NR_OK, rc, "%s", err.msg.c_str());
  const char* env = getenv("NEUREC_SPMM_MASKED_FAST");
  opt.masked_fast = !(env && env[0] == '0');
  env = getenv("NEUREC_SPMM_WANTED_WAVE");
  opt.wanted_wave = !(env && env[0] == '0');
  env = getenv("NEUREC_SPMM_WANTED_NNZ_CAP");
  opt.wanted_nnz_cap = env ? std::max(atoi(env), 1) : 0;

  nr_plan::Plan h;
  rc = nr_plan::build_plan(h_indptr, h_indices, n_rows, opt, &h, &err);
  NR_REQUIRE(rc == NR_OK, rc, "%s", err.msg.c_str());

  BlockedPlan* p = new (std::nothrow) BlockedPlan();
  NR_REQUIRE(p, NR_ERR_ARG, "spmm_blocked_plan_create: out of host memory");
  p->n_rows = n_rows; p->nnz = nnz; p->n_wg = h.n_wg; p->n_phases = h.n_phases;
  p->seg = opt.seg; p->r_max = opt.r_max; p->p_max = opt.p_max; p->waves = opt.waves; p->d = d;
  p->n_ent = (int64_t)h.ent.size(); p->n_cmb = (int64_t)h.cmb.size();
  p->nnz_cap = h.nnz_cap; p->ent_cap = h.ent_cap; p->colmask_ok = h.colmask_ok;
  p->wanted_ok = h.wanted_ok; p->w_ent_cap = h.w_ent_cap; p->w_nnz_cap = h.w_nnz_cap; p->w_bitmap_words = h.w_bitmap_words;
  p->ww_ok = h.ww_ok; p->ww_ent_cap = h.ww_ent_cap; p->ww_lds_slots = h.ww_lds_slots;
  env = getenv("NEUREC_SPMM_WANTED_PLANNED");
  p->n_hubs = (int)h.ww_hub.size();
  p->wp_ok = h.ww_ok && opt.seg == nr_wplan::kSeg && n_rows <= nr_wplan::kMaxRows && !(env && env[0] == '0');
  if (p->wp_ok) p->wp_profile = nr_wplan::slot_profile(h_indptr, n_rows);
  std::vector<nr_plan::Section> sections = nr_plan::plan_sections(*p, h);
  const size_t used = nr_plan::carve_sections(&sections, d_plan_buf);
  if (used > plan_bytes) {
    delete p;
    nrhip_set_error("spmm_blocked_plan_create: plan needs %zu bytes, buffer has %zu", used, plan_bytes);
    return NR_ERR_WORKSPACE;
  }
  hipStream_t st = (hipStream_t)stream;
  hipError_t e = hipSuccess;
  for (const nr_plan::Section& s : sections) {
    if (e != hipSuccess) break;
    if (s.src && s.bytes) e = hipMemcpyAsync(s.addr, s.src, s.bytes, hipMemcpyHostToDevice, st);
    else if (s.zero) e = hipMemsetAsync(s.addr, 0, s.bytes + s.pad, st);
  }
  if (e == hipSuccess) e = hipStreamSynchronize(st);
  if (e == hipSuccess) e = allow_plan_lds(p);
  if (e != hipSuccess) {
    delete p;
    nrhip_set_error("spmm_blocked_plan_create: %s", hipGetErrorString(e));
    return NR_ERR_HIP;
  }
  *plan_out = p;
  return NR_OK;
}

int nrhip_spmm_blocked_pack(void* plan, const int32_t* d_indices, const float* d_vals, void* stream) {
  NR_REQUIRE(plan && d_indices && d_vals, NR_ERR_ARG, "spmm_blocked_pack: null pointer argument");
  BlockedPlan* p = (BlockedPlan*)plan;
  if (p->nnz > 0) {
    const unsigned blocks = (unsigned)std::min<int64_t>((p->n_rows + 15) / 16, 8192);
    hipLaunchKernelGGL(row_order_pack_kernel, dim3(blocks), dim3(256), 0, (hipStream_t)stream, p->pk_src, p->pk_dst,
                       p->n_rows, d_indices, d_vals, p->pk_idx, p->pk_val);
    NR_LAUNCH_CHECK();
  }
  p->pk_from_idx = d_indices;
  p->pk_from_val = d_vals;
  return NR_OK;
}

static int ensure_packed(const BlockedPlan* p, const int32_t* d_indices, const float* d_vals, void* stream) {
  if (p->pk_from_idx == d_indices && p->pk_from_val == d_vals) return NR_OK;
  return nrhip_spmm_blocked_pack((void*)p, d_indices, d_vals, stream);
}

#ifdef NR_WW_TIMELINE
int nrhip_ww_timeline(unsigned long long* h_out) {
  NR_CHECK_HIP(hipDeviceSynchronize());
  NR_CHECK_HIP(hipMemcpyFromSymbol(h_out, HIP_SYMBOL(g_ww_dbg), sizeof(unsigned long long) * 256 * 8));
  return NR_OK;
}
#endif

int nrhip_spmm_blocked_tune(int gathers_in_flight) {
  NR_REQUIRE(gathers_in_flight == 4 || gathers_in_flight == 8, NR_ERR_UNSUPPORTED,
             "spmm_blocked_tune: gathers in flight %d (4, 8)", gathers_in_flight);
  s_gathers_in_flight = gathers_in_flight;
  return NR_OK;
}

int nrhip_spmm_blocked_tune_store(int masked_store) {
  NR_REQUIRE(masked_store >= -1 && masked_store <= kStoreWt, NR_ERR_ARG,
             "spmm_blocked_tune_store: store policy %d (-1 the default, 0 plain, 1 nontemporal, 2 written through)",
             masked_store);
  s_masked_store = masked_store < 0 ? kMaskedStoreDefault : masked_store;
  return NR_OK;
}

int nrhip_spmm_blocked_tune_addend_flag(int on) {
  s_addend_by_flag = on ? 1 : 0;
  return NR_OK;
}

int nrhip_spmm_blocked_plan_destroy(void* plan) {
  delete (BlockedPlan*)plan;
  return NR_OK;
}

int nrhip_spmm_blocked_plan_info(const void* plan, int* n_workgroups, int* n_phases,
                                 int64_t* n_entries, int64_t* n_split) {
  NR_REQUIRE(plan, NR_ERR_ARG, "spmm_blocked_plan_info: null plan");
  const BlockedPlan* p = (const BlockedPlan*)plan;
  if (n_workgroups) *n_workgroups = p->n_wg;
  if (n_phases) *n_phases = p->n_phases;
  if (n_entries) *n_entries = p->n_ent;
  if (n_split) *n_split = p->n_cmb;
  return NR_OK;
}

int nrhip_spmm_blocked_flagged(const void* plan, const int32_t* d_indices, const float* d_vals,
                               const float* d_X, float* d_Y, const float* d_addend,
                               const uint8_t* d_addend_row_flag, const float* d_sum_in, float* d_sum_out,
                               const uint8_t* d_x_row_nonzero, const uint8_t* d_y_row_wanted, void* stream);

int nrhip_spmm_blocked(const void* plan, const int32_t* d_indices, const float* d_vals,
                       const float* d_X, float* d_Y, const float* d_addend, const float* d_sum_in,
                       float* d_sum_out, const uint8_t* d_x_row_nonzero,
                       const uint8_t* d_y_row_wanted, void* stream) {
  return nrhip_spmm_blocked_flagged(plan, d_indices, d_vals, d_X, d_Y, d_addend, nullptr, d_sum_in, d_sum_out,
                                    d_x_row_nonzero, d_y_row_wanted, stream);
}

int nrhip_spmm_blocked_flagged(const void* plan, const int32_t* d_indices, const float* d_vals,
                               const float* d_X, float* d_Y, const float* d_addend,
                               const uint8_t* d_addend_row_flag, const float* d_sum_in, float* d_sum_out,
                               const uint8_t* d_x_row_nonzero, const uint8_t* d_y_row_wanted, void* stream) {
  NR_REQUIRE(plan && d_indices && d_vals && d_X && (d_Y || d_sum_out), NR_ERR_ARG,
             "spmm_blocked: null pointer argument");
  NR_REQUIRE((d_sum_out == nullptr) || (d_sum_in != nullptr), NR_ERR_ARG,
             "spmm_blocked: sum_out needs sum_in");
  NR_REQUIRE(!d_addend_row_flag || (d_addend && !d_x_row_nonzero && !d_y_row_wanted), NR_ERR_ARG,
             "spmm_blocked: addend row flags need an addend and no masks");
  const uint8_t* addend_flag = s_addend_by_flag ? d_addend_row_flag : nullptr;
  const BlockedPlan* p = (const BlockedPlan*)plan;
  hipStream_t st = (hipStream_t)stream;
  dim3 grid((unsigned)p->n_wg), block(p->waves * NR_WAVE);
  const size_t lds = (size_t)(p->r_max + p->p_max) * p->d * 4 + (size_t)p->r_max * 4;
  const bool masked = d_x_row_nonzero || d_y_row_wanted;
  const int gif = s_gathers_in_flight;
  if (p->ww_ok && d_y_row_wanted && !d_x_row_nonzero)
    return launch_wanted_wave(p, d_indices, d_vals, d_X, d_Y, d_addend, d_sum_in, d_sum_out, d_y_row_wanted,
                              LayerChain{nullptr, nullptr}, BatchLists{}, st);
  if (p->wanted_ok && d_y_row_wanted && !d_x_row_nonzero) {
    hipLaunchKernelGGL(spmm_wanted_rows_kernel, grid, block, wanted_lds_bytes(p), st, p->w_ent_off,
                       p->w_cmb_off, p->w_ent, p->w_cmb, d_indices, d_vals, (const float4*)d_X,
                       (float4*)d_Y, (const float4*)d_addend, (const float4*)d_sum_in,
                       (float4*)d_sum_out, d_y_row_wanted, p->r_max, p->p_max, p->w_ent_cap,
                       p->w_nnz_cap, LayerChain{nullptr, nullptr}, BatchLists{}, p->w_bitmap_words);
    NR_LAUNCH_CHECK();
    return NR_OK;
  }
  NR_TRY(ensure_packed(p, d_indices, d_vals, stream));
  if (p->colmask_ok && masked) {
    const int addend_masked = d_x_row_nonzero && d_addend == d_X ? 1 : 0;
    const uint64_t y_all = (uint64_t)p->n_rows * p->d * 4;
    const int store = d_Y && y_all <= 0xFFFFFFFFull ? s_masked_store : kStorePlain;
#define NR_STAGED(CM, RM, ST)                                                                      \
  hipLaunchKernelGGL((spmm_staged_masked_kernel<CM, RM, ST>), grid, block, colmask_lds_bytes(p), st, \
                     p->wg_row0, p->wg_ent_off, p->wg_cmb_off, p->wg_nnz, p->ent, p->cmb, p->pk_idx, \
                     p->pk_val, (const float4*)d_X, (float4*)d_Y, (const float4*)d_addend,          \
                     (const float4*)d_sum_in, (float4*)d_sum_out, d_x_row_nonzero, d_y_row_wanted,  \
                     addend_masked, p->r_max, p->p_max, p->ent_cap, (uint32_t)y_all)
    if (d_x_row_nonzero && d_y_row_wanted) NR_STAGED(true, true, kStorePlain);
    else if (d_x_row_nonzero && store == kStoreNt) NR_STAGED(true, false, kStoreNt);
    else if (d_x_row_nonzero && store == kStoreWt) NR_STAGED(true, false, kStoreWt);
    else if (d_x_row_nonzero) NR_STAGED(true, false, kStorePlain);
    else NR_STAGED(false, true, kStorePlain);
#undef NR_STAGED
    NR_LAUNCH_CHECK();
    return NR_OK;
  }
#define NR_BLK(M, W, GG, DD)                                                                       \
  hipLaunchKernelGGL((spmm_blocked_kernel<M, W, GG, DD>), grid, block, lds, st, p->wg_row0,        \
                     p->wg_nrows, p->wg_ent_off, p->wg_cmb_off, p->ent, p->cmb, p->n_phases,        \
                     p->pk_idx, p->pk_val, (const float4*)d_X, (float4*)d_Y, (const float4*)d_addend, \
                     (const float4*)d_sum_in, (float4*)d_sum_out, d_x_row_nonzero, d_y_row_wanted,  \
                     p->r_max, AdamEpilogue{}, p->row_of, p->p_max, addend_flag)
#define NR_BLK_D(DD)                                                                               \
  if (p->waves == 16) {                                                                            \
    if (masked) { if (gif == 4) NR_BLK(true, 16, 4, DD); else NR_BLK(true, 16, 8, DD); }           \
    else { if (gif == 4) NR_BLK(false, 16, 4, DD); else NR_BLK(false, 16, 8, DD); }                \
  } else {                                                                                         \
    if (masked) { if (gif == 4) NR_BLK(true, 8, 4, DD); else NR_BLK(true, 8, 8, DD); }             \
    else { if (gif == 4) NR_BLK(false, 8, 4, DD); else NR_BLK(false, 8, 8, DD); }                  \
  }
  if (p->d == 16) { NR_BLK_D(16) } else if (p->d == 32) { NR_BLK_D(32) } else if (p->d == 64) { NR_BLK_D(64) }
  else if (p->d == 128) { NR_BLK_D(128) } else { NR_BLK_D(256) }
#undef NR_BLK_D
#undef NR_BLK
  NR_LAUNCH_CHECK();
  return NR_OK;
}

int nrhip_spmm_blocked_wanted_layers(const void* plan, const int32_t* d_indices, const float* d_vals,
                                     const float* d_X, const float* d_sum_in, const float* d_layer_a,
                                     const float* d_layer_b, float* d_sum_out,
                                     const uint8_t* d_y_row_wanted, void* stream) {
  NR_REQUIRE(plan && d_indices && d_vals && d_X && d_sum_in && d_sum_out && d_y_row_wanted, NR_ERR_ARG,
             "spmm_blocked_wanted_layers: null pointer argument");
  NR_REQUIRE(d_layer_a || !d_layer_b, NR_ERR_ARG, "spmm_blocked_wanted_layers: layer_b without layer_a");
  const BlockedPlan* p = (const BlockedPlan*)plan;
  if (p->ww_ok)
    return launch_wanted_wave(p, d_indices, d_vals, d_X, nullptr, nullptr, d_sum_in, d_sum_out, d_y_row_wanted,
                              LayerChain{(const float4*)d_layer_a, (const float4*)d_layer_b}, BatchLists{},
                              (hipStream_t)stream);
  NR_REQUIRE(p->wanted_ok, NR_ERR_UNSUPPORTED, "spmm_blocked_wanted_layers: no wanted-rows schedule");
  hipLaunchKernelGGL(spmm_wanted_rows_kernel, dim3((unsigned)p->n_wg), dim3(p->waves * NR_WAVE),
                     wanted_lds_bytes(p), (hipStream_t)stream, p->w_ent_off, p->w_cmb_off, p->w_ent,
                     p->w_cmb, d_indices, d_vals, (const float4*)d_X, (float4*)nullptr,
                     (const float4*)nullptr, (const float4*)d_sum_in, (float4*)d_sum_out,
                     d_y_row_wanted, p->r_max, p->p_max, p->w_ent_cap, p->w_nnz_cap,
                     LayerChain{(const float4*)d_layer_a, (const float4*)d_layer_b}, BatchLists{},
                     p->w_bitmap_words);
  NR_LAUNCH_CHECK();
  return NR_OK;
}

int nrhip_spmm_blocked_wanted_batch(const void* plan, const int32_t* d_indices, const float* d_vals,
                                    const float* d_X, const float* d_sum_in, const float* d_layer_a,
                                    const float* d_layer_b, float* d_sum_out, const int32_t* d_users,
                                    const int32_t* d_pos, const int32_t* d_neg, int batch, int n_users,
                                    uint8_t* d_row_flag, int32_t* d_rows_out, void* stream) {
  NR_REQUIRE(plan && d_indices && d_vals && d_X && d_sum_in && d_sum_out && d_users && d_pos && d_neg &&
                 d_row_flag && batch >= 0 && n_users >= 0,
             NR_ERR_ARG, "spmm_blocked_wanted_batch: bad arguments");
  NR_REQUIRE(d_layer_a || !d_layer_b, NR_ERR_ARG, "spmm_blocked_wanted_batch: layer_b without layer_a");
  const BlockedPlan* p = (const BlockedPlan*)plan;
  if (batch == 0) return NR_OK;
  if (p->ww_ok)
    return launch_wanted_wave(p, d_indices, d_vals, d_X, nullptr, nullptr, d_sum_in, d_sum_out, nullptr,
                              LayerChain{(const float4*)d_layer_a, (const float4*)d_layer_b},
                              BatchLists{d_users, d_pos, d_neg, batch, n_users, d_row_flag, d_rows_out},
                              (hipStream_t)stream);
  NR_REQUIRE(p->wanted_ok && p->w_bitmap_words > 0, NR_ERR_UNSUPPORTED,
             "spmm_blocked_wanted_batch: no wanted-rows schedule with a row bit set");
  hipLaunchKernelGGL(spmm_wanted_rows_kernel, dim3((unsigned)p->n_wg), dim3(p->waves * NR_WAVE),
                     wanted_lds_bytes(p), (hipStream_t)stream, p->w_ent_off, p->w_cmb_off, p->w_ent,
                     p->w_cmb, d_indices, d_vals, (const float4*)d_X, (float4*)nullptr,
                     (const float4*)nullptr, (const float4*)d_sum_in, (float4*)d_sum_out,
                     (const uint8_t*)nullptr, p->r_max, p->p_max, p->w_ent_cap, p->w_nnz_cap,
                     LayerChain{(const float4*)d_layer_a, (const float4*)d_layer_b},
                     BatchLists{d_users, d_pos, d_neg, batch, n_users, d_row_flag, d_rows_out},
                     p->w_bitmap_words);
  NR_LAUNCH_CHECK();
  return NR_OK;
}

int nrhip_spmm_blocked_has_wanted_planned(const void* plan) {
  return plan && ((const BlockedPlan*)plan)->wp_ok ? 1 : 0;
}

int nrhip_spmm_blocked_wanted_epoch_plan_bytes(const void* plan, int batch, int64_t n_batches, size_t* bytes,
                                               int* stride) {
  NR_REQUIRE(plan && bytes && stride && batch >= 1 && n_batches >= 0, NR_ERR_ARG,
             "spmm_blocked_wanted_epoch_plan_bytes: bad arguments");
  const BlockedPlan* p = (const BlockedPlan*)plan;
  NR_REQUIRE(p->wp_ok, NR_ERR_UNSUPPORTED, "spmm_blocked_wanted_epoch_plan_bytes: no planned form for this plan");
  NR_REQUIRE(3 * (int64_t)batch <= nr_wplan::kMaxKeys, NR_ERR_UNSUPPORTED,
             "spmm_blocked_wanted_epoch_plan_bytes: batch %d > %d", batch, nr_wplan::kMaxKeys / 3);
  const int64_t st = nr_wplan::stride_of(p->wp_profile, batch);
  NR_REQUIRE(st < ((int64_t)1 << 24), NR_ERR_UNSUPPORTED, "spmm_blocked_wanted_epoch_plan_bytes: %lld items per batch",
             (long long)st);
  *stride = (int)st;
  *bytes = (size_t)st * 16 * (size_t)n_batches;
  return NR_OK;
}

int nrhip_spmm_blocked_wanted_epoch_plan(const void* plan, const int64_t* d_indptr, const uint64_t* d_plans, int batch,
                                         int64_t n_batches, int last_len, void* d_sched, size_t sched_bytes,
                                         void* stream) {
  NR_REQUIRE(plan && d_indptr && d_plans && d_sched && batch >= 1 && n_batches >= 1 && last_len >= 1 &&
                 last_len <= batch && n_batches < ((int64_t)1 << 30),
             NR_ERR_ARG, "spmm_blocked_wanted_epoch_plan: bad arguments");
  const BlockedPlan* p = (const BlockedPlan*)plan;
  size_t need = 0;
  int stride = 0;
  NR_TRY(nrhip_spmm_blocked_wanted_epoch_plan_bytes(plan, batch, n_batches, &need, &stride));
  NR_REQUIRE(sched_bytes >= need, NR_ERR_WORKSPACE, "spmm_blocked_wanted_epoch_plan: buffer %zu < %zu bytes",
             sched_bytes, need);
  int n2 = kWpThreads;
  while (n2 < 3 * batch) n2 <<= 1;
  hipLaunchKernelGGL(spmm_wanted_epoch_plan_kernel, dim3((unsigned)n_batches), dim3(kWpThreads), (size_t)n2 * 8,
                     (hipStream_t)stream, d_plans, batch, (int)n_batches, last_len, d_indptr, p->ww_hub, p->n_hubs, n2,
                     stride, (int4*)d_sched);
  NR_LAUNCH_CHECK();
  return NR_OK;
}

int nrhip_spmm_blocked_wanted_planned(const void* plan, const int32_t* d_indices, const float* d_vals,
                                      const float* d_X, const float* d_sum_in, const float* d_layer_a,
                                      const float* d_layer_b, float* d_sum_out, const int32_t* d_users,
                                      const int32_t* d_pos, const int32_t* d_neg, int batch, int n_users,
                                      uint8_t* d_row_flag, int32_t* d_rows_out, const void* d_batch_sched, int stride,
                                      void* stream) {
  NR_REQUIRE(plan && d_indices && d_vals && d_X && d_sum_in && d_sum_out && d_users && d_pos && d_neg &&
                 d_row_flag && d_batch_sched && batch >= 1 && n_users >= 0 && stride > 1 && (stride - 1) % 16 == 0,
             NR_ERR_ARG, "spmm_blocked_wanted_planned: bad arguments");
  NR_REQUIRE(d_layer_a || !d_layer_b, NR_ERR_ARG, "spmm_blocked_wanted_planned: layer_b without layer_a");
  const BlockedPlan* p = (const BlockedPlan*)plan;
  NR_REQUIRE(p->wp_ok, NR_ERR_UNSUPPORTED, "spmm_blocked_wanted_planned: no planned form for this plan");
  hipLaunchKernelGGL(spmm_wanted_planned_kernel, dim3((unsigned)((stride - 1) / 16)), dim3(16 * NR_WAVE), 0,
                     (hipStream_t)stream, (const int4*)d_batch_sched, p->ww_hub, p->ww_part, p->ww_cnt, d_indices,
                     d_vals, (const float4*)d_X,
                     WantedEpi{nullptr, nullptr, (const float4*)d_sum_in, (float4*)d_sum_out,
                               LayerChain{(const float4*)d_layer_a, (const float4*)d_layer_b}},
                     BatchLists{d_users, d_pos, d_neg, batch, n_users, d_row_flag, d_rows_out});
  NR_LAUNCH_CHECK();
  return NR_OK;
}

int nrhip_spmm_blocked_has_wanted(const void* plan) {
  if (plan && ((const BlockedPlan*)plan)->ww_ok) return 2;
  if (!plan || !((const BlockedPlan*)plan)->wanted_ok) return 0;
  return ((const BlockedPlan*)plan)->w_bitmap_words > 0 ? 2 : 1;
}

int nrhip_spmm_blocked_adam(const void* plan, const int32_t* d_indices, const float* d_vals,
                            const float* d_X, float* d_addend, float* d_grad_b, float* d_var,
                            float* d_m, float* d_v, float alpha, float beta1, float beta2,
                            float eps, int clear_consumed, uint8_t* d_row_flag, void* stream) {
  NR_REQUIRE(plan && d_indices && d_vals && d_X && d_grad_b && d_var && d_m && d_v, NR_ERR_ARG,
             "spmm_blocked_adam: null pointer argument");
  const BlockedPlan* p = (const BlockedPlan*)plan;
  NR_REQUIRE(p->d == 64 && p->waves == 16, NR_ERR_UNSUPPORTED,
             "spmm_blocked_adam: built for d = 64 schedules with 16 waves");
  NR_REQUIRE(d_X != d_var, NR_ERR_ARG, "spmm_blocked_adam: the operand must not be the updated table");
  const size_t lds = (size_t)(p->r_max + p->p_max) * p->d * 4 + (size_t)p->r_max * 4;
  NR_TRY(ensure_packed(p, d_indices, d_vals, stream));
  NR_REQUIRE(!clear_consumed || d_addend, NR_ERR_ARG, "spmm_blocked_adam: clear_consumed needs an addend");
  AdamEpilogue ad{(float4*)d_var, (float4*)d_m, (float4*)d_v, (const float4*)d_grad_b,
                  alpha, 1.0f - beta1, 1.0f - beta2, eps,
                  clear_consumed ? (float4*)d_addend : nullptr,
                  clear_consumed ? (float4*)d_grad_b : nullptr, clear_consumed ? d_row_flag : nullptr};
  hipLaunchKernelGGL((spmm_blocked_kernel<false, 16, 8, 64, true>), dim3((unsigned)p->n_wg),
                     dim3(16 * NR_WAVE), lds, (hipStream_t)stream, p->wg_row0, p->wg_nrows,
                     p->wg_ent_off, p->wg_cmb_off, p->ent, p->cmb, p->n_phases, p->pk_idx, p->pk_val,
                     (const float4*)d_X, (float4*)nullptr, (const float4*)d_addend,
                     (const float4*)nullptr, (float4*)nullptr, (const uint8_t*)nullptr,
                     (const uint8_t*)nullptr, p->r_max, ad, p->row_of, p->p_max, (const uint8_t*)nullptr);
  NR_LAUNCH_CHECK();
  return NR_OK;
}

}
```

### neurec_amd/csrc/spmm_blocked_plan.h

```cpp
#pragma once
#include <stdarg.h>
#include <stdint.h>
#include <stdio.h>
#include <algorithm>
#include <functional>
#include <queue>
#include <string>
#include <utility>
#include <vector>

namespace nr_plan {

constexpr int kSegDefault = 64;
constexpr int kRMaxDefault = 416;
constexpr int kPMaxDefault = 192;
constexpr int kMaxPhases = 32;
constexpr int kMaxLdsBytes = 160 * 1024;
constexpr int kWaveChunk = 8;

struct Int4 { int32_t x, y, z, w; };
static_assert(sizeof(Int4) == 16, "descriptors are 16 bytes on the device");

enum Status { kOk = 0, kErrArg = 1, kErrUnsupported = 2 };
struct Error { std::string msg; };

inline int fail(Error* err, int code, const char* fmt, ...) {
  char buf[512];
  va_list ap;
  va_start(ap, fmt);
  vsnprintf(buf, sizeof(buf), fmt, ap);
  va_end(ap);
  err->msg = buf;
  return code;
}
#define NR_PLAN_REQUIRE(cond, code, ...) \
  do { if (!(cond)) return ::nr_plan::fail(err, (code), __VA_ARGS__); } while (0)
#define NR_PLAN_TRY(call) \
  do { const int rc_ = (call); if (rc_ != ::nr_plan::kOk) return rc_; } while (0)

inline size_t align_up(size_t x, size_t a) { return (x + a - 1) / a * a; }

struct Options {
  int d, waves, seg, r_max, p_max;
  int64_t block_bytes;
  int64_t split_row;
  int n_wg;
  bool masked_fast = true;
  bool wanted_wave = true;
  int wanted_nnz_cap = 0;
};

struct Plan {
  int64_t n_rows = 0, nnz = 0;
  int n_wg = 0, n_phases = 1;
  std::vector<int32_t> wg_row0, wg_nrows;
  std::vector<int32_t> row_of;
  std::vector<uint32_t> pk_src, pk_dst;
  std::vector<int32_t> ent_off, cmb_off;
  std::vector<Int4> ent;
  std::vector<Int4> cmb;
  std::vector<uint32_t> wg_nnz;
  int64_t nnz_cap_exact = 0;
  int nnz_cap = 0, ent_cap = 0;
  int colmask_ok = 0;
  std::vector<Int4> w_ent;
  std::vector<Int4> w_cmb;
  std::vector<int32_t> w_ent_off, w_cmb_off;
  int wanted_ok = 0, w_ent_cap = 0, w_nnz_cap = 0, w_bitmap_words = 0;
  std::vector<int32_t> ww_off, ww_choff, ww_lcoff;
  std::vector<Int4> ww_ent;
  std::vector<int32_t> ww_gch;
  std::vector<Int4> ww_hub;
  std::vector<Int4> ww_lcmb;
  int64_t ww_segments = 0;
  int ww_ok = 0, ww_ent_cap = 0, ww_lds_slots = 0;
};

struct ClassDesc { int64_t ra, rb; std::vector<int> wgs; int32_t cmin; int64_t width, K; };

constexpr int kEntCost = 4;
inline int64_t row_cost(int64_t len, int seg) {
  return len + (int64_t)kEntCost * std::max<int64_t>(1, (len + seg - 1) / seg);
}

inline int resolve_options(int d, int waves_per_wg, int seg_len, int r_max, int p_max, int64_t block_bytes,
                           int64_t split_row, int64_t n_rows, Options* opt, Error* err) {
  opt->d = d;
  opt->waves = waves_per_wg > 0 ? waves_per_wg : 16;
  opt->seg = seg_len > 0 ? seg_len : kSegDefault;
  opt->r_max = r_max > 0 ? r_max : kRMaxDefault * opt->waves / 16 * 64 / (d > 0 ? d : 64);
  opt->p_max = p_max > 0 ? p_max : kPMaxDefault * opt->waves / 16 * 64 / (d > 0 ? d : 64);
  NR_PLAN_REQUIRE(d == 16 || d == 32 || d == 64 || d == 128 || d == 256, kErrUnsupported,
                  "spmm_blocked: embedding dim %d not built (16, 32, 64, 128, 256)", d);
  NR_PLAN_REQUIRE(opt->waves == 16 || opt->waves == 8, kErrUnsupported,
                  "spmm_blocked: waves per workgroup %d (8, 16)", opt->waves);
  NR_PLAN_REQUIRE(opt->seg >= 16 && (size_t)(opt->r_max + opt->p_max) * d * 4 + (size_t)opt->r_max * 4 <= (size_t)kMaxLdsBytes,
                  kErrUnsupported, "spmm_blocked: seg %d / accumulators %d+%d do not fit", opt->seg, opt->r_max,
                  opt->p_max);
  opt->block_bytes = block_bytes > 0 ? block_bytes : (int64_t)1 << 40;
  opt->split_row = (split_row <= 0 || split_row >= n_rows) ? 0 : split_row;
  opt->n_wg = 0;
  return kOk;
}

inline int choose_workgroup_count(int n_wg, bool from_device, int64_t n_rows, Options* opt, Error* err) {
  n_wg = n_wg / 8 * 8;
  if (from_device && n_wg >= 8) {
    const int64_t per_class = opt->split_row ? n_wg / 2 : n_wg;
    const int64_t biggest = opt->split_row ? std::max<int64_t>(opt->split_row, n_rows - opt->split_row) : n_rows;
    const int64_t cap = (int64_t)opt->r_max * 9 / 10;
    const int64_t mult = (biggest + per_class * cap - 1) / (per_class * cap);
    if (mult > 1) n_wg = (int)std::min<int64_t>((int64_t)n_wg * mult, 4096 + n_rows / 32) / 8 * 8;
  }
  NR_PLAN_REQUIRE(n_wg >= 8 && n_wg <= 4096 + n_rows / 32, kErrUnsupported, "spmm_blocked: %d workgroups", n_wg);
  opt->n_wg = n_wg;
  return kOk;
}

inline std::vector<ClassDesc> assign_workgroups_to_classes(const int64_t* indptr, int64_t n_rows, const Options& opt) {
  const int n_wg = opt.n_wg;
  const int64_t split_row = opt.split_row;
  std::vector<ClassDesc> classes;
  if (!split_row) {
    ClassDesc a{0, n_rows, {}, 0, 1, 1};
    for (int w = 0; w < n_wg; ++w) a.wgs.push_back(w);
    classes.push_back(a);
    return classes;
  }
  ClassDesc a{0, split_row, {}, 0, 1, 1}, b{split_row, n_rows, {}, 0, 1, 1};
  int64_t cost_a = 0, cost_b = 0;
  for (int64_t r = 0; r < n_rows; ++r) (r < split_row ? cost_a : cost_b) += row_cost(indptr[r + 1] - indptr[r], opt.seg);
  int n_a = (int)((double)n_wg * (double)cost_a / (double)std::max<int64_t>(cost_a + cost_b, 1) + 0.5);
  n_a = std::min(std::max(n_a, 1), n_wg - 1);
  {
    const int64_t cap = (int64_t)opt.r_max * 9 / 10;
    const int need_a = (int)((split_row + cap - 1) / cap), need_b = (int)((n_rows - split_row + cap - 1) / cap);
    n_a = std::max(n_a, std::min(need_a, n_wg - 1));
    n_a = std::min(n_a, std::max(n_wg - need_b, 1));
  }
  std::vector<int> order;
  for (int x = 0; x < 8; ++x)
    for (int w = x; w < n_wg; w += 8) order.push_back(w);
  for (int i = 0; i < n_wg; ++i) (i < n_a ? a : b).wgs.push_back(order[i]);
  std::sort(a.wgs.begin(), a.wgs.end());
  std::sort(b.wgs.begin(), b.wgs.end());
  classes.push_back(a);
  classes.push_back(b);
  return classes;
}

inline int class_span_and_phases(const int64_t* indptr, const int32_t* indices, const Options& opt, ClassDesc* cl,
                                 Error* err) {
  int32_t cmin = INT32_MAX, cmax = -1;
  for (int64_t t = indptr[cl->ra]; t < indptr[cl->rb]; ++t) {
    cmin = std::min(cmin, indices[t]);
    cmax = std::max(cmax, indices[t]);
  }
  if (cmax < cmin) { cmin = 0; cmax = 0; }
  const int64_t span = (int64_t)cmax + 1 - cmin;
  const int64_t K = std::max<int64_t>((span * opt.d * 4 + opt.block_bytes - 1) / opt.block_bytes, 1);
  NR_PLAN_REQUIRE(K <= kMaxPhases, kErrUnsupported,
                  "spmm_blocked: gathered table of %lld rows needs %lld column blocks (max %d) — "
                  "use the work-item kernel", (long long)span, (long long)K, kMaxPhases);
  cl->cmin = cmin;
  cl->width = (span + K - 1) / K;
  cl->K = K;
  return kOk;
}

inline int deal_rows(const int64_t* indptr, const ClassDesc& cl, const Options& opt,
// ... 124 lines not shown
  h->wanted_ok = on && opt.seg <= 255 && h->n_rows < ((int64_t)1 << 24);
}

inline void wanted_rows_schedule(const int64_t* indptr, const Options& opt, Plan* h) {
  const int n_wg = h->n_wg;
  const int64_t n_rows = h->n_rows;
  h->w_ent_off.assign((size_t)n_wg * 2, 0);
  h->w_cmb_off.assign((size_t)n_wg * 2, 0);
  if (!h->wanted_ok) return;
  std::vector<int32_t> order((size_t)n_rows);
  for (int64_t r = 0; r < n_rows; ++r) order[(size_t)r] = (int32_t)r;
  std::stable_sort(order.begin(), order.end(), [&](int32_t a, int32_t b) {
    return indptr[a + 1] - indptr[a] > indptr[b + 1] - indptr[b];
  });
  std::vector<std::vector<Int4>> we((size_t)n_wg), wc((size_t)n_wg);
  std::vector<int> wp((size_t)n_wg, 0);
  for (int64_t k = 0; k < n_rows && h->wanted_ok; ++k) {
    const int32_t row = order[(size_t)k];
    const size_t w = (size_t)(k % n_wg);
    const int64_t b = indptr[row], len = indptr[row + 1] - b;
    if (len <= opt.seg) {
      we[w].push_back(Int4{0, (int32_t)len, (int32_t)(uint32_t)b, row});
    } else {
      const int ns = (int)((len + opt.seg - 1) / opt.seg);
      if (wp[w] + ns > opt.p_max) { h->wanted_ok = 0; break; }
      for (int sg = 0; sg < ns; ++sg)
        we[w].push_back(Int4{opt.r_max + wp[w] + sg, (int32_t)std::min<int64_t>(opt.seg, len - (int64_t)sg * opt.seg),
                             (int32_t)(uint32_t)(b + (int64_t)sg * opt.seg), row});
      wc[w].push_back(Int4{row, opt.r_max + wp[w], ns, 0});
      wp[w] += ns;
    }
  }
  for (int w = 0; w < n_wg && h->wanted_ok; ++w) {
    h->w_ent_off[2 * (size_t)w] = (int32_t)h->w_ent.size();
    h->w_cmb_off[2 * (size_t)w] = (int32_t)h->w_cmb.size();
    h->w_ent.insert(h->w_ent.end(), we[(size_t)w].begin(), we[(size_t)w].end());
    h->w_cmb.insert(h->w_cmb.end(), wc[(size_t)w].begin(), wc[(size_t)w].end());
    h->w_ent_off[2 * (size_t)w + 1] = (int32_t)h->w_ent.size();
    h->w_cmb_off[2 * (size_t)w + 1] = (int32_t)h->w_cmb.size();
    h->w_ent_cap = std::max<int>(h->w_ent_cap, (int)we[(size_t)w].size());
  }
  h->w_ent_cap = (h->w_ent_cap + 15) / 16 * 16;
  h->w_bitmap_words = n_rows <= 131072 ? (int)((n_rows + 127) / 128 * 4) : 0;
  const int64_t left = (int64_t)kMaxLdsBytes - 256 - (int64_t)opt.p_max * 256 - 2 * (int64_t)h->w_ent_cap * 16 -
                       (int64_t)h->w_bitmap_words * 4;
  h->w_nnz_cap = (int)std::min<int64_t>(left / 8, (int64_t)1 << 22);
  if (opt.wanted_nnz_cap > 0) h->w_nnz_cap = std::min(h->w_nnz_cap, std::max(opt.wanted_nnz_cap, 4 * opt.seg));
  if (h->w_nnz_cap < 4 * opt.seg) h->wanted_ok = 0;
}

inline void wanted_wave_schedule(const int64_t* indptr, const Options& opt, Plan* h) {
  const int n_wg = h->n_wg;
  const int64_t n_rows = h->n_rows;
  h->ww_off.assign((size_t)n_wg + 1, 0);
  h->ww_choff.assign((size_t)n_wg + 1, 0);
  h->ww_lcoff.assign((size_t)n_wg + 1, 0);
  if (!(opt.d == 64 && opt.waves == 16 && opt.seg <= 64 && n_rows <= 131072 * 4 && opt.wanted_wave)) return;
  struct Unit { int64_t len; int32_t row; int hub, seg0, nseg; };
  std::vector<Unit> units;
  for (int64_t r = 0; r < n_rows; ++r) {
    const int64_t len = indptr[r + 1] - indptr[r];
    if (len <= opt.seg) {
      units.push_back(Unit{len, (int32_t)r, -1, 0, 0});
      continue;
    }
    const int ns = (int)((len + opt.seg - 1) / opt.seg), nch = (ns + kWaveChunk - 1) / kWaveChunk;
    if (nch == 1) {
      units.push_back(Unit{len, (int32_t)r, -2, 0, ns});
      continue;
    }
    const int hub = (int)h->ww_hub.size();
    h->ww_hub.push_back(Int4{(int32_t)r, (int32_t)h->ww_segments, ns, nch});
    for (int ch = 0; ch < nch; ++ch) {
      const int s0 = ch * kWaveChunk, s1 = std::min(ns, s0 + kWaveChunk);
      units.push_back(Unit{std::min<int64_t>(len - (int64_t)s0 * opt.seg, (int64_t)(s1 - s0) * opt.seg), (int32_t)r,
                           hub, s0, s1 - s0});
    }
    h->ww_segments += ns;
  }
  std::stable_sort(units.begin(), units.end(), [](const Unit& a, const Unit& b) { return a.len > b.len; });
  std::vector<std::vector<Int4>> per((size_t)n_wg), perl((size_t)n_wg);
  std::vector<std::vector<int32_t>> perch((size_t)n_wg);
  std::vector<int> lds_used((size_t)n_wg, 0);
  for (size_t k = 0; k < units.size(); ++k) {
    const Unit& u = units[k];
    const size_t w = k % (size_t)n_wg;
    const int64_t b = indptr[u.row], len = indptr[u.row + 1] - b;
    auto segment = [&](int32_t slot, int sg) {
      return Int4{slot, (int32_t)std::min<int64_t>(opt.seg, len - (int64_t)sg * opt.seg),
                  (int32_t)(uint32_t)(b + (int64_t)sg * opt.seg), u.row};
    };
    if (u.hub == -1) {
      per[w].push_back(Int4{0, (int32_t)len, (int32_t)(uint32_t)b, u.row});
    } else if (u.hub == -2) {
      perl[w].push_back(Int4{u.row, lds_used[w], u.nseg, 0});
      for (int sg = 0; sg < u.nseg; ++sg) per[w].push_back(segment(-(1 + lds_used[w] + sg), sg));
      lds_used[w] += u.nseg;
    } else {
      for (int sg = u.seg0; sg < u.seg0 + u.nseg; ++sg) per[w].push_back(segment(1 + h->ww_hub[(size_t)u.hub].y + sg, sg));
      perch[w].push_back(u.hub);
    }
  }
  for (int w = 0; w < n_wg; ++w) {
    h->ww_off[(size_t)w] = (int32_t)h->ww_ent.size();
    h->ww_choff[(size_t)w] = (int32_t)h->ww_gch.size();
    h->ww_lcoff[(size_t)w] = (int32_t)h->ww_lcmb.size();
    h->ww_ent.insert(h->ww_ent.end(), per[(size_t)w].begin(), per[(size_t)w].end());
    h->ww_gch.insert(h->ww_gch.end(), perch[(size_t)w].begin(), perch[(size_t)w].end());
    h->ww_lcmb.insert(h->ww_lcmb.end(), perl[(size_t)w].begin(), perl[(size_t)w].end());
    h->ww_ent_cap = std::max<int>(h->ww_ent_cap, (int)per[(size_t)w].size());
    h->ww_lds_slots = std::max(h->ww_lds_slots, lds_used[(size_t)w]);
  }
  h->ww_off[(size_t)n_wg] = (int32_t)h->ww_ent.size();
  h->ww_choff[(size_t)n_wg] = (int32_t)h->ww_gch.size();
  h->ww_lcoff[(size_t)n_wg] = (int32_t)h->ww_lcmb.size();
  h->ww_ent_cap = (h->ww_ent_cap + 15) / 16 * 16;
  h->ww_ok = h->ww_segments < ((int64_t)1 << 30) &&
             (size_t)h->ww_lds_slots * 256 + (size_t)h->ww_ent_cap * 16 + (size_t)((n_rows + 127) / 128 * 16) + 1024 <=
                 (size_t)kMaxLdsBytes;
}

inline int build_plan(const int64_t* indptr, const int32_t* indices, int64_t n_rows, const Options& opt, Plan* h,
                      Error* err) {
  *h = Plan();
  h->n_rows = n_rows;
  h->nnz = indptr[n_rows] - indptr[0];
  h->n_wg = opt.n_wg;
  std::vector<ClassDesc> classes = assign_workgroups_to_classes(indptr, n_rows, opt);
  std::vector<std::vector<int32_t>> wg_rows((size_t)opt.n_wg);
  for (ClassDesc& cl : classes) {
    NR_PLAN_TRY(class_span_and_phases(indptr, indices, opt, &cl, err));
    h->n_phases = std::max<int>(h->n_phases, (int)cl.K);
    NR_PLAN_TRY(deal_rows(indptr, cl, opt, &wg_rows, err));
  }
  NR_PLAN_TRY(packed_order(indptr, wg_rows, h, err));
  std::vector<std::vector<std::vector<Int4>>> wg_ent((size_t)opt.n_wg), wg_cmb((size_t)opt.n_wg);
  for (const ClassDesc& cl : classes)
    for (int w : cl.wgs)
      NR_PLAN_TRY(cut_rows_into_entries(indptr, indices, cl, wg_rows[(size_t)w], h->pk_dst.data() + h->wg_row0[(size_t)w],
                                        opt, &wg_ent[(size_t)w], &wg_cmb[(size_t)w], err));
  flatten_entries(wg_ent, wg_cmb, h);
  masked_hop_switches(opt, h);
  wanted_rows_schedule(indptr, opt, h);
  wanted_wave_schedule(indptr, opt, h);
  return kOk;
}

template <class I4>
struct PlanArrays {
  I4* ent; I4* cmb;
  int32_t* wg_row0; int32_t* wg_nrows;
  int32_t* row_of; uint32_t* pk_src; uint32_t* pk_dst;
  int32_t* pk_idx; float* pk_val;
  int32_t* wg_ent_off; int32_t* wg_cmb_off;
  uint32_t* wg_nnz;
  I4* w_ent; I4* w_cmb; int32_t* w_ent_off; int32_t* w_cmb_off;
  int32_t* ww_off; int32_t* ww_choff; I4* ww_ent; int32_t* ww_gch; I4* ww_hub; int32_t* ww_lcoff; I4* ww_lcmb;
  float* ww_part;
  unsigned* ww_cnt;
};

struct Section {
  void* field;
  void (*set)(void* field, void* addr);
  const void* src;
  size_t bytes, pad;
  bool zero;
  void* addr;
};
template <class T>
Section section(T*& field, const void* src, size_t bytes, size_t pad = 0, bool zero = false) {
  return Section{&field, [](void* f, void* a) { *(T**)f = (T*)a; }, src, bytes, pad, zero, nullptr};
}
template <class T, class V>
Section section(T*& field, const std::vector<V>& v, size_t pad = 0) {
  return section(field, v.data(), v.size() * sizeof(V), pad);
}

template <class I4>
std::vector<Section> plan_sections(PlanArrays<I4>& p, const Plan& h) {
  std::vector<Section> s = {
      section(p.ent, h.ent, 16),
      section(p.cmb, h.cmb, 16),
      section(p.wg_row0, h.wg_row0),
      section(p.wg_nrows, h.wg_nrows),
      section(p.row_of, h.row_of),
      section(p.pk_src, h.pk_src),
      section(p.pk_dst, h.pk_dst),
      section(p.pk_idx, nullptr, (size_t)h.nnz * 4, 4),
      section(p.pk_val, nullptr, (size_t)h.nnz * 4, 4),
      section(p.wg_ent_off, h.ent_off),
      section(p.wg_cmb_off, h.cmb_off),
      section(p.wg_nnz, h.wg_nnz),
      section(p.w_ent, h.w_ent, 16),
      section(p.w_cmb, h.w_cmb, 16),
      section(p.w_ent_off, h.w_ent_off),
      section(p.w_cmb_off, h.w_cmb_off),
  };
  if (h.ww_ok) {
    s.push_back(section(p.ww_off, h.ww_off));
    s.push_back(section(p.ww_choff, h.ww_choff));
    s.push_back(section(p.ww_ent, h.ww_ent, 16));
    s.push_back(section(p.ww_gch, h.ww_gch, 4));
    s.push_back(section(p.ww_hub, h.ww_hub, 16));
    s.push_back(section(p.ww_lcoff, h.ww_lcoff));
    s.push_back(section(p.ww_lcmb, h.ww_lcmb, 16));
    s.push_back(section(p.ww_part, nullptr, (size_t)h.ww_segments * 256, 256));
    s.push_back(section(p.ww_cnt, nullptr, h.ww_hub.size() * 4, 4, true));
  }
  return s;
}

inline size_t carve_sections(std::vector<Section>* sections, void* base) {
  size_t off = 0;
  for (Section& s : *sections) {
    s.addr = (void*)((uintptr_t)base + off);
    s.set(s.field, s.addr);
    off += align_up(s.bytes + s.pad, 256);
  }
  return off;
}

inline size_t blocked_plan_bytes(int64_t n_rows, int64_t nnz) {
  const size_t max_ent = (size_t)std::min<int64_t>(nnz, n_rows * (int64_t)kMaxPhases) + (size_t)(nnz / 16) + 64;
  const size_t max_cmb = (size_t)(nnz / 16) + 64;
  const size_t wg = 4096 + (size_t)(n_rows / 32);
  const size_t w_ent = (size_t)n_rows + (size_t)(nnz / 16) + 64;
  const size_t ww_seg = (size_t)(nnz / 32) + 64, ww_ents = (size_t)n_rows + ww_seg;
  const size_t ww = 3 * align_up((wg + 1) * 4, 256)  +
                    align_up(ww_ents * 16 + 16, 256)  + align_up(ww_seg * 4 + 4, 256)  +
                    2 * align_up(max_cmb * 16 + 16, 256)  +
                    align_up(ww_seg * 256 + 256, 256)  + align_up(max_cmb * 4 + 4, 256) ;
  const size_t dealt = 3 * align_up(((size_t)n_rows + 1) * 4, 256)  +
                       2 * align_up((size_t)nnz * 4 + 4, 256) ;
  return ww + dealt + align_up(max_ent * 16, 256)  + align_up(max_cmb * 16, 256)  +
         3 * align_up(wg * 8, 256)  +
         2 * align_up(wg * (kMaxPhases + 1) * 4, 256)  +
         align_up(w_ent * 16, 256)  + align_up(max_cmb * 16, 256)  +
         2 * align_up(wg * 8, 256) ;
}

}
```

### neurec_amd/engine.py

```python
import ctypes as C
import os

import numpy as np
import torch

from . import _lib
from ._lib import call

NGCF_MAX_LAYERS = _lib.NGCF_MAX_LAYERS

METRIC_IDS = {"Precision": 1, "Recall": 2, "MAP": 3, "NDCG": 4, "MRR": 5}


def require_gpu():
    if not torch.cuda.is_available():
        raise RuntimeError("neurec_amd needs a ROCm GPU (MI355X / gfx950); no CPU path exists")
    return torch.device("cuda", torch.cuda.current_device())


def _stream():
    return C.c_void_p(torch.cuda.current_stream().cuda_stream)


def _ptr(t, dtype=None, allow_none=False):
    if t is None:
        if allow_none:
            return C.c_void_p(0)
        raise ValueError("tensor argument is None")
    if not isinstance(t, torch.Tensor) or not t.is_cuda:
        raise TypeError("expected a CUDA/ROCm tensor, got %r" % (type(t),))
    if dtype is not None and t.dtype != dtype:
        raise TypeError("expected dtype %s, got %s" % (dtype, t.dtype))
    if not t.is_contiguous():
        raise ValueError("tensor must be contiguous")
    return C.c_void_p(t.data_ptr())


class Workspace:

    def __init__(self):
        self.buf = None

    def get(self, nbytes):
        nbytes = max(int(nbytes), 256)
        if self.buf is None or self.buf.numel() < nbytes:
            self.buf = torch.empty(nbytes, dtype=torch.uint8, device=require_gpu())
        return self.buf


class DeviceCSR:

    def __init__(self, indptr, indices, n_cols):
        dev = require_gpu()
        if isinstance(indices, torch.Tensor):
            self.indptr = indptr.to(dev, torch.int64).contiguous()
            self.indices = indices.to(dev, torch.int32).contiguous()
            indptr = self.indptr.cpu().numpy()
        else:
            indptr = np.ascontiguousarray(indptr, dtype=np.int64)
            indices = np.ascontiguousarray(indices, dtype=np.int32)
            self.indptr = torch.from_numpy(indptr).to(dev)
            self.indices = torch.from_numpy(indices if len(indices) else np.zeros(1, np.int32)).to(dev)
        self.n_rows = len(indptr) - 1
        self.n_cols = int(n_cols)
        self.nnz = int(indptr[-1])
        self.h_indptr = indptr

    @staticmethod
    def from_scipy(mat):
        m = mat.tocsr().copy()
        m.sum_duplicates()
        m.sort_indices()
        return DeviceCSR(m.indptr, m.indices, m.shape[1])

    @staticmethod
    def from_dict(d, n_rows, n_cols):
        counts = np.zeros(n_rows + 1, dtype=np.int64)
        for r, items in d.items():
            counts[int(r) + 1] = len(items)
        indptr = np.cumsum(counts)
        indices = np.empty(int(indptr[-1]), dtype=np.int32)
        for r, items in d.items():
            b = indptr[int(r)]
            indices[b:b + len(items)] = np.sort(np.asarray(items, dtype=np.int32))
        return DeviceCSR(indptr, indices, n_cols)

    def rows(self, lo, hi):
        lo, hi = int(lo), int(hi)
        b, e = int(self.h_indptr[lo]), int(self.h_indptr[hi])
        idx = self.indices[b:e] if e > b else torch.zeros(1, dtype=torch.int32, device=self.indices.device)
        return DeviceCSR(self.indptr[lo:hi + 1] - b, idx, self.n_cols)

    def check_sorted(self, n_cols=None):
        n_cols = self.n_cols if n_cols is None else int(n_cols)
        if self.nnz == 0:
            return
        idx = self.indices[:self.nnz].long()
        lo, hi = int(idx.min()), int(idx.max())
        if lo < 0 or hi >= n_cols:
            raise ValueError("CSR column ids span [%d, %d], outside [0, %d)" % (lo, hi, n_cols))
        if self.nnz > 1:
            key = self.row_of().long() * n_cols + idx
            if bool((key[1:] < key[:-1]).any()):
                raise ValueError("CSR rows must hold ascending column ids (sort the rows: DeviceCSR.from_scipy does)")

    def row_of(self):
        if self.nnz == 0:
            return torch.zeros(1, dtype=torch.int32, device=self.indptr.device)
        return torch.repeat_interleave(torch.arange(self.n_rows, dtype=torch.int32, device=self.indptr.device),
                                       self.indptr[1:] - self.indptr[:-1], output_size=self.nnz)


_eval_ws = Workspace()
_gemm_ws = Workspace()
_misc_ws = Workspace()


def mask_train(scores, users, train_csr, cols=None):
    if scores.dim() != 2 or scores.stride(1) != 1 or scores.dtype != torch.float32:
        raise ValueError("scores must be a 2-D float32 tensor with unit inner stride")
    rows = scores.shape[0]
    cols = scores.shape[1] if cols is None else cols
    call("nrhip_mask_train", C.c_void_p(scores.data_ptr()), scores.stride(0),
         _ptr(users, torch.int32, allow_none=True), rows, cols, _ptr(train_csr.indptr),
         _ptr(train_csr.indices), _stream())


def eval_scores(scores, truth_csr, metric_ids, top_k, users=None, cols=None, out=None,
                want_topk=False, want_exact_count=False):
    if scores.dim() != 2 or scores.stride(1) != 1:
        raise ValueError("scores must be 2-D with unit inner stride")
    rows = scores.shape[0]
    cols = scores.shape[1] if cols is None else cols
    dev = scores.device
    nm = len(metric_ids)
    if out is None:
        out = torch.empty((rows, nm * top_k), dtype=torch.float32, device=dev)
    topk = torch.empty((rows, top_k), dtype=torch.int32, device=dev) if want_topk else None
    nex = torch.zeros(1, dtype=torch.int32, device=dev) if want_exact_count else None
    nbytes = C.c_size_t(0)
    ids = (C.c_int * nm)(*[int(m) for m in metric_ids])
    if top_k > 128:
        call("nrhip_eval_any_k_workspace_bytes", rows, cols, top_k, C.byref(nbytes))
        ws = _eval_ws.get(nbytes.value)
        call("nrhip_eval_scores_any_k", C.c_void_p(scores.data_ptr()), scores.stride(0), rows, cols,
             _ptr(users, torch.int32, allow_none=True), _ptr(truth_csr.indptr), _ptr(truth_csr.indices), ids, nm,
             top_k, _ptr(out, torch.float32), _ptr(topk, allow_none=True), _ptr(ws), ws.numel(), _stream())
        if nex is not None:
            nex.fill_(rows)
        res = [out] + ([topk] if want_topk else []) + ([nex] if want_exact_count else [])
        return res[0] if len(res) == 1 else tuple(res)
    call("nrhip_eval_workspace_bytes", rows, top_k, C.byref(nbytes))
    ws = _eval_ws.get(nbytes.value)
    call("nrhip_eval_scores", C.c_void_p(scores.data_ptr()), scores.stride(0), rows, cols,
         _ptr(users, torch.int32, allow_none=True), _ptr(truth_csr.indptr),
         _ptr(truth_csr.indices), ids, nm, top_k, _ptr(out, torch.float32),
         _ptr(topk, allow_none=True), _ptr(nex, allow_none=True), _ptr(ws), ws.numel(), _stream())
    res = [out]
    if want_topk:
# ... 469 lines not shown
    call("nrhip_route_owner_keys", _ptr(rows, torch.int32, allow_none=True), _ptr(codes, torch.int32, allow_none=True),
         keys.numel(), _ptr(recv_prefix, torch.int32), _ptr(size_off, torch.int32), int(world), int(global_batch),
         int(code_base), _ptr(keys, torch.int64), _ptr(index_of_pos, torch.int32), _stream())


def rows_scatter_add(rows, src, dst):
    d = dst.shape[1]
    call("nrhip_rows_scatter_add", _ptr(rows, torch.int32), rows.numel(), d,
         C.c_void_p(src.data_ptr()), src.stride(0), _ptr(dst, torch.float32), _stream())


def rows_sum_sorted(keys, index_of_pos, src, dst):
    call("nrhip_rows_sum_sorted", _ptr(keys, torch.int64), keys.numel(), _ptr(index_of_pos, torch.int32),
         dst.shape[1], C.c_void_p(src.data_ptr()), src.stride(0), _ptr(dst, torch.float32), _stream())


def rows_sum_sorted2(keys, index_of_pos, src_a, dst_a, src_b, dst_b):
    call("nrhip_rows_sum_sorted2", _ptr(keys, torch.int64), keys.numel(), _ptr(index_of_pos, torch.int32),
         dst_a.shape[1], C.c_void_p(src_a.data_ptr()), src_a.stride(0), _ptr(dst_a, torch.float32),
         C.c_void_p(src_b.data_ptr()), src_b.stride(0), _ptr(dst_b, torch.float32), _stream())


def sort_keys(keys):
    call("nrhip_sort_u64", _ptr(keys, torch.int64), keys.numel(), _stream())
    return keys


def rows_clear(rows, d, bufs=(), flag=None):
    b = list(bufs) + [None] * (4 - len(bufs))
    call("nrhip_rows_clear", _ptr(rows, torch.int32), rows.numel(), int(d),
         _ptr(b[0], allow_none=True), _ptr(b[1], allow_none=True), _ptr(b[2], allow_none=True),
         _ptr(b[3], allow_none=True), _ptr(flag, allow_none=True), _stream())


def bpr_plan(users, items, third, batch, n_users, out=None):
    n = users.numel()
    n_cls = 2 if third is None else 3
    if out is None:
        out = torch.empty(max(n_cls * n, 1), dtype=torch.int64, device=users.device)
    call("nrhip_bpr_plan", _ptr(users, torch.int32), _ptr(items, torch.int32),
         _ptr(third, torch.int32, allow_none=True), n, int(batch), int(n_users),
         _ptr(out, torch.int64), _stream())
    return out[:n_cls * n]


def _work(terms, batch):
    if terms.numel() < 8 * batch:
        raise ValueError("work buffer holds %d floats, 8 * batch = %d needed" % (terms.numel(), 8 * batch))
    return _ptr(terms, torch.float32)


def bpr_mf_grad(P, Q, users, pos, neg, reg, GP, GQ, terms, loss2, plan=None):
    call("nrhip_bpr_mf_grad", _ptr(P, torch.float32), _ptr(Q, torch.float32), P.shape[1], P.shape[0],
         _ptr(users, torch.int32), _ptr(pos, torch.int32), _ptr(neg, torch.int32), users.numel(),
         float(reg), _ptr(GP), _ptr(GQ), _work(terms, users.numel()), _ptr(loss2),
         _ptr(plan, torch.int64, allow_none=True), _stream())


PAIRWISE_LOSSES = {"bpr": 0, "hinge": 1, "square": 2}
POINTWISE_LOSSES = {"cross_entropy": 0, "square": 1}
ROW_OPTIMIZERS = {"gd": 0, "adagrad": 1, "rmsprop": 2, "momentum": 3}


def pairwise_mf_grad(P, Q, users, pos, neg, reg, loss, GP, GQ, terms, loss2, plan=None):
    call("nrhip_pairwise_mf_grad", _ptr(P, torch.float32), _ptr(Q, torch.float32), P.shape[1],
         P.shape[0], _ptr(users, torch.int32), _ptr(pos, torch.int32), _ptr(neg, torch.int32),
         users.numel(), float(reg), PAIRWISE_LOSSES[loss], _ptr(GP), _ptr(GQ),
         _work(terms, users.numel()), _ptr(loss2), _ptr(plan, torch.int64, allow_none=True), _stream())


def pointwise_mf_grad(P, Q, users, items, labels, reg, loss, GP, GQ, terms, loss2, plan=None):
    call("nrhip_pointwise_mf_grad", _ptr(P, torch.float32), _ptr(Q, torch.float32), P.shape[1],
         P.shape[0], _ptr(users, torch.int32), _ptr(items, torch.int32), _ptr(labels, torch.float32),
         users.numel(), float(reg), POINTWISE_LOSSES[loss], _ptr(GP), _ptr(GQ),
         _work(terms, users.numel()), _ptr(loss2), _ptr(plan, torch.int64, allow_none=True), _stream())


def gather_u8(src, index, dst):
    call("nrhip_gather_u8", _ptr(src, torch.uint8), _ptr(index, torch.int32), index.numel(), _ptr(dst, torch.uint8),
         _stream())


def mark_rows(ids, flag, offset=0):
    call("nrhip_mark_rows", _ptr(ids, torch.int32), ids.numel(), int(offset), _ptr(flag, torch.uint8),
         _stream())


def optimizer_rows(kind, var, slot0, slot1, grad, flag, lr, hyper1=0.0, hyper2=0.0, eps=0.0):
    call("nrhip_optimizer_rows_tf", ROW_OPTIMIZERS[kind], _ptr(var, torch.float32),
         _ptr(slot0, torch.float32, allow_none=True), _ptr(slot1, torch.float32, allow_none=True),
         _ptr(grad, torch.float32), _ptr(flag, torch.uint8), var.shape[0], var.shape[1], float(lr),
         float(hyper1), float(hyper2), float(eps), _stream())


class DenseLearner:

    KINDS = ("gd", "adagrad", "rmsprop", "momentum")

    def __init__(self, kind, lr, momentum=0.9):
        kind = str(kind).lower()
        if kind not in self.KINDS:
            raise ValueError("please select a suitable optimizer")
        self.kind, self.lr, self.momentum = kind, float(lr), float(momentum)

    def init_slots(self, slot0, slot1):
        v0 = {"gd": 0.0, "adagrad": 1e-8, "rmsprop": 1.0, "momentum": 0.0}[self.kind]
        for t in slot0:
            t.fill_(v0)
        for t in slot1:
            t.zero_()

    def apply(self, tensors):
        h1, h2, eps = {"gd": (0.0, 0.0, 0.0), "adagrad": (0.0, 0.0, 0.0), "rmsprop": (0.9, 0.0, 1e-10),
                       "momentum": (self.momentum, 0.0, 0.0)}[self.kind]
        for t in tensors:
            var, s0, s1, grad = t[:4]
            call("nrhip_optimizer_dense_tf", ROW_OPTIMIZERS[self.kind], _ptr(var, torch.float32),
                 _ptr(s0, torch.float32, allow_none=True), _ptr(s1, torch.float32, allow_none=True),
                 _ptr(grad, torch.float32), var.numel(), self.lr, h1, h2, eps, 1 if (len(t) > 4 and t[4]) else 0,
                 _stream())


def make_learner(learner, lr):
    return None if str(learner).lower() == "adam" else DenseLearner(learner, lr)


def lightgcn_mark_batch(users, pos, neg, n_users, rows_out, row_flag):
    call("nrhip_lightgcn_mark_batch", _ptr(users, torch.int32), _ptr(pos, torch.int32),
         _ptr(neg, torch.int32), users.numel(), int(n_users), _ptr(rows_out, torch.int32),
         _ptr(row_flag, torch.uint8), _stream())


def lightgcn_bpr_grad(Esum, E0, n_users, n_layers, users, pos, neg, reg, Gstar, Greg, terms, loss2,
                      plan=None, divided=False):
    call("nrhip_lightgcn_bpr_grad_h" if divided else "nrhip_lightgcn_bpr_grad", _ptr(Esum, torch.float32), _ptr(E0, torch.float32), n_users,
         E0.shape[1], n_layers, _ptr(users, torch.int32), _ptr(pos, torch.int32),
         _ptr(neg, torch.int32), users.numel(), float(reg), _ptr(Gstar), _ptr(Greg),
         _work(terms, users.numel()), _ptr(loss2, allow_none=True),
         _ptr(plan, torch.int64, allow_none=True), _stream())


def scale(x, a, out):
    call("nrhip_scale", _ptr(x), float(a), _ptr(out), x.numel(), _stream())


def add(x, y, out):
    call("nrhip_add", _ptr(x), _ptr(y), _ptr(out), x.numel(), _stream())


def div_scalar(x, denom, out):
    call("nrhip_div_scalar", _ptr(x), float(denom), _ptr(out), x.numel(), _stream())


class SpmmCSR:

    def __init__(self, indptr, indices, vals, n_cols=None, item_rows=0, item_nnz=0, split_row=0):
        dev = require_gpu()
        if isinstance(indices, torch.Tensor):
            self.indptr = indptr.to(dev, torch.int64).contiguous()
            self.h_indptr = self.indptr.cpu().numpy()
            self.indices = indices.to(dev, torch.int32).contiguous()
            self.vals = vals.to(dev, torch.float32).contiguous()
            self._h_indices = None
        else:
            self.h_indptr = np.ascontiguousarray(indptr, dtype=np.int64)
            idx = np.ascontiguousarray(indices, dtype=np.int32)
            val = np.ascontiguousarray(vals, dtype=np.float32)
            self._h_indices = idx
            self.indices = torch.from_numpy(idx if len(idx) else np.zeros(1, np.int32)).to(dev)
            self.vals = torch.from_numpy(val if len(val) else np.zeros(1, np.float32)).to(dev)
            self.indptr = torch.from_numpy(self.h_indptr).to(dev)
        self.n_rows = len(self.h_indptr) - 1
        self.nnz = int(self.h_indptr[-1])
        self.n_cols = self.n_rows if n_cols is None else n_cols
        self.split_row = int(split_row)
        self.lane_group = True
        self.blocked = None
        self._blocked = {}
        nbytes = C.c_size_t(0)
        call("nrhip_spmm_plan_bytes", self.n_rows, self.nnz, C.byref(nbytes))
        self.plan_buf = torch.empty(max(nbytes.value, 256), dtype=torch.uint8, device=dev)
        self.plan = C.c_void_p(0)
        call("nrhip_spmm_plan_create", self.h_indptr.ctypes.data_as(C.c_void_p), self.n_rows,
             int(item_rows), int(item_nnz), int(split_row), _ptr(self.plan_buf), self.plan_buf.numel(), _stream(), C.byref(self.plan))
        nseg, nsplit = C.c_int64(0), C.c_int64(0)
        call("nrhip_spmm_plan_info", self.plan, C.byref(nseg), C.byref(nsplit))
        self.n_segments, self.n_split_rows = nseg.value, nsplit.value
        self._ws = {}

    @property
    def h_indices(self):
        if self._h_indices is None:
            self._h_indices = self.indices[:self.nnz].cpu().numpy()
        return self._h_indices

    @staticmethod
    def from_scipy(mat, item_rows=0, item_nnz=0, split_row=0, keep_order=False):
        m = mat.tocsr().astype(np.float32)
        if not keep_order:
            m.sort_indices()
        return SpmmCSR(m.indptr, m.indices, m.data, m.shape[1], item_rows, item_nnz, split_row)

    def __del__(self):
        try:
            for plan, _buf in getattr(self, "_blocked", {}).values():
                if plan is not None and plan.value:
                    _lib.lib.nrhip_spmm_blocked_plan_destroy(plan)
            self._blocked = {}
            if getattr(self, "plan", None) is not None and self.plan.value:
                _lib.lib.nrhip_spmm_plan_destroy(self.plan)
                self.plan = C.c_void_p(0)
        except Exception:
            pass

    def ensure_schedule(self, d, force=False):
        if d not in (16, 32, 64, 128, 256) or not self.lane_group or \
                (d in (128, 256) and not force and d not in self._blocked):
            return False
        if d not in self._blocked:
            self._blocked[d] = (None, None)
            if os.environ.get("NEUREC_SPMM_BLOCKED", "1") != "0" and self.nnz > 0:
                nbytes = C.c_size_t(0)
                call("nrhip_spmm_blocked_plan_bytes", self.n_rows, self.nnz, int(d), C.byref(nbytes))
                buf = torch.empty(max(nbytes.value, 256), dtype=torch.uint8, device=self.indices.device)
                plan = C.c_void_p(0)
                try:
                    call("nrhip_spmm_blocked_plan_create", self.h_indptr.ctypes.data_as(C.c_void_p),
                         self.h_indices.ctypes.data_as(C.c_void_p), self.n_rows, self.split_row, d,
                         0, 0, 0, 0, 0, 0, _ptr(buf), buf.numel(), _stream(), C.byref(plan))
                    call("nrhip_spmm_plan_attach_blocked", self.plan, plan, d)
                    call("nrhip_spmm_blocked_pack", plan, _ptr(self.indices), _ptr(self.vals), _stream())
                    self._blocked[d] = (plan, buf)
                except NotImplementedError:
                    pass
        self.blocked = self._blocked[d][0]
        return self.blocked is not None

    def values_changed(self):
        for plan, _buf in self._blocked.values():
            if plan is not None and plan.value:
                call("nrhip_spmm_blocked_pack", plan, _ptr(self.indices), _ptr(self.vals), _stream())

    def exact_row_nnz(self, d):
        return 64 if self.ensure_schedule(d) else 256

    def _workspace(self, d):
        if d not in self._ws:
            nbytes = C.c_size_t(0)
            call("nrhip_spmm_workspace_bytes", self.plan, d, C.byref(nbytes))
            self._ws[d] = torch.empty(max(nbytes.value, 256), dtype=torch.uint8,
                                      device=self.indices.device)
        return self._ws[d]

    def matmul(self, X, out=None, addend=None, sum_in=None, sum_out=None, x_row_nonzero=None,
               y_row_wanted=None, addend_row_flag=None):
        d = X.shape[1]
        self.ensure_schedule(d)
        ws = self._workspace(d)
        if addend_row_flag is not None:
            if x_row_nonzero is not None or y_row_wanted is not None:
                raise ValueError("addend_row_flag goes with the unmasked product")
            call("nrhip_spmm_csr_flagged", self.plan, _ptr(self.indptr), _ptr(self.indices),
                 _ptr(self.vals), _ptr(X, torch.float32), d,
                 _ptr(out, torch.float32, allow_none=True), _ptr(addend, allow_none=True),
                 _ptr(addend_row_flag, torch.uint8), _ptr(sum_in, allow_none=True),
                 _ptr(sum_out, allow_none=True), _ptr(ws), ws.numel(), _stream())
        elif x_row_nonzero is None and y_row_wanted is None:
            call("nrhip_spmm_csr", self.plan, _ptr(self.indptr), _ptr(self.indices),
                 _ptr(self.vals), _ptr(X, torch.float32), d,
                 _ptr(out, torch.float32, allow_none=True), _ptr(addend, allow_none=True),
                 _ptr(sum_in, allow_none=True), _ptr(sum_out, allow_none=True), _ptr(ws),
                 ws.numel(), _stream())
        else:
            call("nrhip_spmm_csr_masked", self.plan, _ptr(self.indptr), _ptr(self.indices),
                 _ptr(self.vals), _ptr(X, torch.float32),
                 _ptr(x_row_nonzero, torch.uint8, allow_none=True),
                 _ptr(y_row_wanted, torch.uint8, allow_none=True), d,
                 _ptr(out, torch.float32, allow_none=True), _ptr(addend, allow_none=True),
                 _ptr(sum_in, allow_none=True), _ptr(sum_out, allow_none=True), _ptr(ws),
                 ws.numel(), _stream())
        return out

    def matmul_adam(self, X, addend, grad_b, var, m, v, st, row_flag=None):
        d = X.shape[1]
        if d != 64 or not self.ensure_schedule(64):
            return False
        call("nrhip_spmm_csr_adam", self.plan, _ptr(self.indices), _ptr(self.vals), _ptr(X, torch.float32), d,
             _ptr(addend, torch.float32), _ptr(grad_b, torch.float32), _ptr(var, torch.float32), _ptr(m), _ptr(v),
             float(st.alpha()), float(st.beta1), float(st.beta2), float(st.eps), 1 if row_flag is not None else 0,
             _ptr(row_flag, torch.uint8, allow_none=True), _stream())
        return True

    def matmul_rows(self, X, rows, out=None, addend=None, sum_in=None, sum_out=None):
        d = X.shape[1]
        call("nrhip_spmm_csr_rows", _ptr(self.indptr), _ptr(self.indices), _ptr(self.vals),
             _ptr(X, torch.float32), d, _ptr(rows, torch.int32), rows.numel(),
             _ptr(out, torch.float32, allow_none=True), _ptr(addend, allow_none=True),
             _ptr(sum_in, allow_none=True), _ptr(sum_out, allow_none=True), _stream())
        return out

    def algorithmic_bytes(self, d):
        return self.nnz * 8 + (self.n_rows + 1) * 4 + 2 * self.n_rows * d * 4

    def masked_bytes(self, d):
        return self.nnz * 8 + (self.n_rows + 1) * 4 + self.n_rows * d * 4

    def full_pass_kernel(self, d):
        if self.ensure_schedule(d):
            return "spmm_blocked_kernel<false, 16, 8, %d, false>" % d
        return "spmm_item_kernel<%d, ...>" % d


def add2d(x, y, out):
    call("nrhip_add2d", C.c_void_p(x.data_ptr()), x.stride(0), C.c_void_p(y.data_ptr()), y.stride(0),
         C.c_void_p(out.data_ptr()), out.stride(0), x.shape[0], x.shape[1], _stream())


def copy2d(x, out):
    call("nrhip_copy2d", C.c_void_p(x.data_ptr()), x.stride(0), C.c_void_p(out.data_ptr()),
         out.stride(0), x.shape[0], x.shape[1], _stream())


def ngcf_layer_fwd(ego, S, W, keep, mask, mask_given, seed, step, layer, ego_out, out_block):
    call("nrhip_ngcf_layer_fwd", _ptr(ego, torch.float32), _ptr(S, torch.float32), _ptr(W[0]),
         _ptr(W[1]), _ptr(W[2]), _ptr(W[3]), ego.shape[0], ego.shape[1], float(keep),
         _ptr(mask, torch.uint8), 1 if mask_given else 0, C.c_uint64(seed & (2**64 - 1)),
         C.c_uint64(step), int(layer), _ptr(ego_out, torch.float32),
         C.c_void_p(out_block.data_ptr()), out_block.stride(0), _stream())


def ngcf_layer_bwd(ego, S, W, keep, mask, dout_block, dego_next, dS, dego_direct, dT1, dT2, dW, ws):
    call("nrhip_ngcf_layer_bwd", _ptr(ego, torch.float32), _ptr(S, torch.float32), _ptr(W[0]),
         _ptr(W[1]), _ptr(W[2]), _ptr(W[3]), ego.shape[0], ego.shape[1], float(keep),
         _ptr(mask, torch.uint8), C.c_void_p(dout_block.data_ptr()), dout_block.stride(0),
         _ptr(dego_next, allow_none=True), _ptr(dS), _ptr(dego_direct), _ptr(dT1), _ptr(dT2),
         _ptr(dW[0]), _ptr(dW[1]), _ptr(dW[2]), _ptr(dW[3]), _ptr(ws), ws.numel(), _stream())


def ngcf_workspace(n_rows, device):
    nbytes = C.c_size_t(0)
    call("nrhip_ngcf_workspace_bytes", int(n_rows), C.byref(nbytes))
    return torch.empty(nbytes.value, dtype=torch.uint8, device=device)


class EpochHopSchedule:

    def __init__(self, A, d):
        self.A, self.d = A, int(d)
        self.ok = bool(_lib.lib.nrhip_spmm_plan_has_wanted_planned(A.plan, self.d)) and \
            _lib.lib.nrhip_spmm_plan_has_wanted(A.plan, self.d) == 2
        self.key, self.buf, self.stride, self.batch, self.n_batches, self.last_len = None, None, 0, 0, 0, 0

    def for_batch(self, plan, n_triplets):
        stream = getattr(plan, "epoch_plans", None) if plan is not None else None
        if not self.ok or stream is None:
            return None
        plans, batch, epoch = stream
        if 3 * batch > 16384:
            return None
        key = (plans.data_ptr(), plans.numel(), int(batch), int(epoch))
        if key != self.key:
            self._build(plans, int(batch))
            self.key = key
        k = int(plan.batch_index)
        if not (0 <= k < self.n_batches) or n_triplets != (self.last_len if k == self.n_batches - 1 else self.batch):
            raise ValueError("batch %d of %d triplets is not a batch of its epoch stream" % (k, n_triplets))
        return self.buf.data_ptr() + k * self.stride * 16, self.stride

    def _build(self, plans, batch):
        n = plans.numel() // 3
        n_batches = (n + batch - 1) // batch
        nbytes, stride = C.c_size_t(0), C.c_int(0)
        call("nrhip_spmm_wanted_epoch_plan_bytes", self.A.plan, self.d, batch, n_batches, C.byref(nbytes),
             C.byref(stride))
        if self.buf is None or self.buf.numel() < nbytes.value:
            self.buf = torch.empty(nbytes.value, dtype=torch.uint8, device=plans.device)
        self.stride, self.batch, self.n_batches = stride.value, batch, n_batches
        self.last_len = n - (n_batches - 1) * batch
        call("nrhip_spmm_wanted_epoch_plan", self.A.plan, self.d, _ptr(self.A.indptr), _ptr(plans, torch.int64), batch,
             n_batches, self.last_len, _ptr(self.buf), self.buf.numel(), _stream())


class NativeStep:

    def __init__(self, kind, handle, owner):
        self.kind, self.handle, self.owner = kind, handle, owner

    @staticmethod
    def for_lightgcn(eng):
        b = _lib.LightGCNBuffers()
        eng.A.ensure_schedule(eng.d)
        eng.At.ensure_schedule(eng.d)
        ws = eng.A._workspace(eng.d)
        wst = eng.At._workspace(eng.d)
# ... 274 lines not shown
```

### neurec_amd/graph.py

```python
import numpy as np
import scipy.sparse as sp

ADJ_TYPES = ("plain", "norm", "gcmc", "pre", "mean")


def _inv_power(rowsum, p):
    with np.errstate(divide="ignore"):
        out = np.power(rowsum, p)
    out[np.isinf(out)] = 0.0
    return out


def bipartite_adjacency(user_idx, item_idx, n_users, n_items):
    u = np.asarray(user_idx, dtype=np.int64)
    i = np.asarray(item_idx, dtype=np.int64) + n_users
    n = n_users + n_items
    rows = np.concatenate([u, i])
    cols = np.concatenate([i, u])
    a = sp.csr_matrix((np.ones(len(rows), np.float32), (rows, cols)), shape=(n, n))
    a.sum_duplicates()
    a.sort_indices()
    return a


def lightgcn_adjacency(user_idx, item_idx, n_users, n_items, adj_type="pre", tf_order=False):
    a = bipartite_adjacency(user_idx, item_idx, n_users, n_items)
    n = a.shape[0]
    row_of = np.repeat(np.arange(n), np.diff(a.indptr))
    if adj_type == "plain":
        out = a
    elif adj_type == "pre":
        deg = np.asarray(a.sum(1)).ravel().astype(np.float32)
        dinv = _inv_power(deg, np.float32(-0.5)).astype(np.float32)
        vals = (dinv[row_of] * a.data) * dinv[a.indices]
        out = sp.csr_matrix((vals.astype(np.float32), a.indices.copy(), a.indptr.copy()), shape=a.shape)
    elif adj_type == "gcmc":
        deg = np.asarray(a.sum(1)).ravel().astype(np.float32)
        dinv = _inv_power(deg, np.float32(-1)).astype(np.float32)
        out = sp.csr_matrix(((dinv[row_of] * a.data).astype(np.float32), a.indices.copy(),
                             a.indptr.copy()), shape=a.shape)
    elif adj_type == "norm":
        ai = (a.astype(np.float64) + sp.eye(n, dtype=np.float64)).tocsr()
        ai.sort_indices()
        deg = np.asarray(ai.sum(1)).ravel()
        dinv = _inv_power(deg, -1.0)
        r_of = np.repeat(np.arange(n), np.diff(ai.indptr))
        out = sp.csr_matrix(((dinv[r_of] * ai.data).astype(np.float32), ai.indices, ai.indptr),
                            shape=ai.shape)
    elif adj_type == "mean":
        deg = np.asarray(a.sum(1)).ravel().astype(np.float32)
        dinv = _inv_power(deg, np.float32(-1)).astype(np.float32)
        mean_adj = sp.csr_matrix(((dinv[row_of] * a.data).astype(np.float32), a.indices.copy(),
                                  a.indptr.copy()), shape=a.shape)
        out = (mean_adj.astype(np.float64) + sp.eye(n, dtype=np.float64)).tocsr().astype(np.float32)
    else:
        raise ValueError("adj_type must be one of %s" % (ADJ_TYPES,))
    out = out.tocsr().astype(np.float32)
    out.sort_indices()
    if tf_order and adj_type == "gcmc":
        out = reverse_rows(out)
    return out


def reverse_rows(a):
    a = a.tocsr()
    nnz = a.nnz
    row_of = np.repeat(np.arange(a.shape[0]), np.diff(a.indptr))
    src = a.indptr[row_of] + a.indptr[row_of + 1] - 1 - np.arange(nnz)
    out = sp.csr_matrix((a.data[src], a.indices[src], a.indptr.copy()), shape=a.shape)
    out.has_sorted_indices = False
    return out


def transpose_csr(a):
    t = a.T.tocsr().astype(np.float32)
    t.sort_indices()
    return t


def is_symmetric(a):
    return (a != a.T).nnz == 0


def ngcf_adjacency(train_matrix, adj_type="norm"):
    r = sp.csr_matrix(train_matrix, dtype=np.float32)
    r.sum_duplicates()
    n = r.shape[0] + r.shape[1]
    a = sp.bmat([[None, r], [r.T.tocsr(), None]], format="csr", dtype=np.float32)
    a.sort_indices()

    def row_normalised(m):
        deg = np.asarray(m.sum(1)).ravel()
        dinv = _inv_power(deg, -1)
        rows = np.repeat(np.arange(m.shape[0]), np.diff(m.indptr))
        return sp.csr_matrix((dinv[rows] * m.data, m.indices.copy(), m.indptr.copy()), shape=m.shape)

    if adj_type == "plain":
        out = a
    elif adj_type == "norm":
        ai = (a.astype(np.float64) + sp.eye(n, dtype=np.float64)).tocsr()
        ai.sort_indices()
        out = row_normalised(ai)
    elif adj_type == "gcmc":
        out = row_normalised(a)
    else:
        out = (row_normalised(a).astype(np.float64) + sp.eye(n, dtype=np.float64)).tocsr()
    out = out.tocsr().astype(np.float32)
    out.sort_indices()
    return out
```

### neurec_amd/ngcf_wide.py

```python
import ctypes as C

import numpy as np
import torch

from . import _lib
from . import engine as E
from ._lib import call
from .engine import _ptr, _stream

_SPMM_WIDTHS = (16, 32, 64, 128, 256)


def _pad(w):
    for p in _SPMM_WIDTHS:
        if w <= p:
            return p
    raise NotImplementedError("NGCF layer width %d > 256 is not built" % w)


class NGCFWideEngine:
    ALGS = ("ngcf", "gcn", "gcmc")

    def __init__(self, adj, adj_t, n_users, n_items, embed, weights, lr, reg, mess_dropout, max_batch, seed=2017,
                 learner="adam", alg_type="ngcf", node_dropout=0.0):
# ... 21 lines not shown
        self.d = self.w[0]
        blocks = ([0] if self.alg == "gcmc" else [self.w[0]]) + self.w[1:]
        self.dsum = sum(blocks)
        if self.dsum > 256:
            raise NotImplementedError("NGCF: concatenated output width %d > 256 is not built (BPR head rows)" % self.dsum)
        self.off = np.concatenate([[0], np.cumsum(blocks)]).astype(int)
        self.E0p = z(N, self.wp[0])
        self.E0p[:, :self.w[0]] = f(embed)
        self.W = [tuple(f(np.reshape(x, -1) if j % 2 else x) for j, x in enumerate(ws)) for ws in weights]
        self.Out, self.dOut = z(N, self.dsum), z(N, self.dsum)
        self.ego = [self.E0p] + [z(N, self.wp[k + 1]) for k in range(self.L)]
        self.S = [z(N, self.wp[k]) for k in range(self.L)]
        self.X2 = [z(N, self.wp[k]) for k in range(self.L)]
        self.T1 = [z(N, self.w[k + 1]) for k in range(self.L)]
        self.T2 = [z(N, self.w[k + 1]) for k in range(self.L)]
        self.mask = [torch.zeros(N, self.w[k + 1], dtype=torch.uint8, device=dev) for k in range(self.L)]
        wmax = max(self.w)
        self.dT1, self.dT2, self.Y1, self.Y2 = (z(N * wmax) for _ in range(4))
        self.dS = [z(N, p) for p in sorted(set(self.wp))]
        self.dEd = [z(N, p) for p in sorted(set(self.wp))]
        self.dEgo = [[z(N, p) for p in sorted(set(self.wp))] for _ in range(2)]
        self.gE0 = z(N, self.wp[0])
        self.mE, self.vE = z(N, self.wp[0]), z(N, self.wp[0])
        self.gW = [tuple(torch.zeros_like(x) for x in ws) for ws in self.W]
        self.mW = [tuple(torch.zeros_like(x) for x in ws) for ws in self.W]
        self.vW = [tuple(torch.zeros_like(x) for x in ws) for ws in self.W]
        self.keep = 1.0 - float(mess_dropout)
        self.reg, self.seed, self.t = float(reg), int(seed), 0
        self.adam = E.AdamState(lr)
        self.terms = torch.empty(8 * max_batch, dtype=torch.float32, device=dev)
        self.rows = torch.zeros(3 * max_batch, dtype=torch.int32, device=dev)
        self.flag = torch.zeros(N, dtype=torch.uint8, device=dev)
        self.max_batch = max_batch
        self.cs_ws = z(((N + 511) // 512) * wmax)
        self.splits = max(1, min(768, (N + 255) // 256))
        nbytes = C.c_size_t(0)
        call("nrhip_gemm_workspace_bytes", wmax, wmax, self.splits, C.byref(nbytes))
        self.ws = torch.empty(max(nbytes.value, 256), dtype=torch.uint8, device=dev)
        self.learner = E.make_learner(learner, lr)
        if self.learner is not None:
            self.learner.init_slots([self.mE] + [m for ms in self.mW for m in ms], [self.vE] + [v for vs in self.vW for v in vs])
        self._native = self._native_buffers() if (self.L <= _lib.NGCF_WIDE_MAX_LAYERS and self.learner is None and
                                                  self.alg == "ngcf") else None
        self.node_keep = 1.0 - float(node_dropout)
        if self.alg != "ngcf":
            self.node_keep = 1.0
        if self.node_keep < 1.0:
            import scipy.sparse as sp
            a = adj.tocsr().astype(np.float32)
            a.sort_indices()
            pos = sp.csr_matrix((np.arange(1, a.nnz + 1, dtype=np.float64), a.indices, a.indptr), shape=a.shape)
            pt = pos.T.tocsr()
            pt.sort_indices()
            self._t_of = torch.from_numpy((pt.data - 1).astype(np.int32)).to(dev)
            self._vals0 = self.A.vals.clone()
            self.edge_keep = torch.ones(max(self.A.nnz, 1), dtype=torch.uint8, device=dev)

    def _native_buffers(self):
        b = _lib.NGCFWideBuffers()
        ptr = lambda t: t.data_ptr()
        for A, sfx, ws_name in ((self.A, "", "ws_fwd"), (self.At, "_t", "ws_bwd")):
            setattr(b, "plan" + sfx, A.plan.value)
            setattr(b, "indptr" + sfx, ptr(A.indptr))
            setattr(b, "indices" + sfx, ptr(A.indices))
            setattr(b, "vals" + sfx, ptr(A.vals))
            for k in range(self.L):
                A.ensure_schedule(self.wp[k])
                ws = A._workspace(self.wp[k])
                getattr(b, ws_name)[k] = ptr(ws)
                getattr(b, ws_name + "_bytes")[k] = ws.numel()
        b.n_users, b.n_nodes, b.n_layers, b.max_batch, b.dsum, b.splits = \
            self.n_users, self.N, self.L, self.max_batch, self.dsum, self.splits
        for k in range(self.L + 1):
            b.w[k], b.wp[k] = self.w[k], self.wp[k]
            b.ego[k] = ptr(self.ego[k])
        for k in range(self.L + 2):
            b.off[k] = int(self.off[k])
        for name in ("E0p", "mE", "vE", "gE0", "Out", "dOut", "dT1", "dT2", "Y1", "Y2", "terms", "cs_ws", "rows", "flag"):
            setattr(b, name, ptr(getattr(self, name)))
        b.cs_ws_bytes = self.cs_ws.numel() * 4
        b.gemm_ws, b.gemm_ws_bytes = ptr(self.ws), self.ws.numel()
        for k in range(self.L):
            b.S[k], b.X2[k], b.T1[k], b.T2[k], b.mask[k] = (ptr(x[k]) for x in (self.S, self.X2, self.T1, self.T2, self.mask))
            pi = self.wp[k]
            b.dS[k], b.dEd[k] = ptr(self._buf(self.dS, pi)), ptr(self._buf(self.dEd, pi))
            b.dEgo[k] = ptr(self._buf(self.dEgo[k % 2], pi))
            for j in range(4):
                b.W[k][j], b.gW[k][j], b.mW[k][j], b.vW[k][j] = (ptr(x[k][j]) for x in (self.W, self.gW, self.mW, self.vW))
        b.reg, b.keep = self.reg, self.keep
        return b

    @property
    def E0(self):
        return self.E0p[:, :self.w[0]]

    def _buf(self, group, width):
        return group[sorted(set(self.wp)).index(width)]

    def _gemm(self, A, lda, a_kminor, Bm, ldb, b_kminor, M, N, K, Cm, ldc, splits=1, bias=None):
        call("nrhip_gemm_f32", _ptr(A), int(lda), int(a_kminor), _ptr(Bm), int(ldb), int(b_kminor), int(M), int(N),
             int(K), _ptr(Cm), int(ldc), 0, _ptr(bias, torch.float32, allow_none=True), -1, int(splits), _ptr(self.ws),
             self.ws.numel() if splits > 1 else 0, _stream())

    def forward(self, masks=None, node_keep_given=None):
        if node_keep_given is not None or self.node_keep < 1.0:
            self._drop_nodes(node_keep_given)
        if self.alg != "ngcf":
            return self._forward_variant(masks)
        if self._native is None:
            return self.forward_reference(masks)
        if masks is not None:
            for k in range(self.L):
                self.mask[k].copy_(masks[k])
        call("nrhip_ngcf_wide_forward", C.byref(self._native), 1 if masks is not None else 0,
             C.c_uint64(self.seed & (2**64 - 1)), C.c_uint64(self.t), _stream())
        self.t += 1
        return self.Out

    def forward_reference(self, masks=None):
        N = self.N
        E.copy2d(self.E0, self.Out[:, :self.w[0]])
        for k in range(self.L):
            wi, wo, pi, po = self.w[k], self.w[k + 1], self.wp[k], self.wp[k + 1]
            ego, S, X2 = self.ego[k], self.S[k], self.X2[k]
            self.A.matmul(ego, out=S)
            call("nrhip_ew_mul", _ptr(ego), pi, _ptr(S), pi, N, wi, _ptr(X2), pi, _stream())
            Wg, bg, Wb, bb = self.W[k]
            self._gemm(S, pi, 1, Wg, wo, 0, N, wo, wi, self.T1[k], wo, bias=bg)
            self._gemm(X2, pi, 1, Wb, wo, 0, N, wo, wi, self.T2[k], wo, bias=bb)
            if masks is not None:
                self.mask[k].copy_(masks[k])
            out_block = self.Out[:, self.off[k + 1]:self.off[k + 2]]
            call("nrhip_ngcf_act_fwd", _ptr(self.T1[k]), _ptr(self.T2[k]), wo, N, wo, po, float(self.keep),
                 _ptr(self.mask[k], torch.uint8), 1 if masks is not None else 0, C.c_uint64(self.seed & (2**64 - 1)),
                 C.c_uint64(self.t), k, _ptr(self.ego[k + 1]), po, C.c_void_p(out_block.data_ptr()), self.dsum,
                 _stream())
        self.t += 1
        return self.Out

    def final_embeddings(self, masks=None, node_keep_given=None):
        out = self.forward(masks, node_keep_given)
        return out[:self.n_users], out[self.n_users:]

    def _drop_nodes(self, given=None):
        if self.node_keep >= 1.0 and given is None:
            return
        if given is not None:
            self.edge_keep.copy_(given)
        n = self.A.nnz
        call("nrhip_edge_dropout", _ptr(self._vals0), n, float(self.node_keep), _ptr(self.edge_keep, torch.uint8),
             1 if given is not None else 0, C.c_uint64(self.seed & (2**64 - 1)), C.c_uint64(self.t), _ptr(self.A.vals),
             _stream())
        call("nrhip_gather_f32", _ptr(self.A.vals), _ptr(self._t_of, torch.int32), n, _ptr(self.At.vals), _stream())
        self.A.values_changed()
        self.At.values_changed()

    def step(self, users, pos, neg, loss_out, masks=None, plan=None, node_keep_given=None):
        if self.alg != "ngcf":
            return self._step_variant(users, pos, neg, loss_out, masks, plan)
        if node_keep_given is not None or self.node_keep < 1.0:
            self._drop_nodes(node_keep_given)
        if self._native is None:
            return self.step_reference(users, pos, neg, loss_out, masks, plan, dropped=True)
        B = users.numel()
        if B > self.max_batch:
            raise ValueError("batch larger than max_batch")
        if masks is not None:
            for k in range(self.L):
                self.mask[k].copy_(masks[k])
        st = self.adam
        call("nrhip_ngcf_wide_step", C.byref(self._native), _ptr(users, torch.int32), _ptr(pos, torch.int32),
             _ptr(neg, torch.int32), B, _ptr(plan, torch.int64, allow_none=True), 1 if masks is not None else 0,
             C.c_uint64(self.seed & (2**64 - 1)), C.c_uint64(self.t), st.alpha(), st.beta1, st.beta2, st.eps,
             _ptr(loss_out, torch.float32, allow_none=True), _stream())
        self.t += 1
        self.adam.advance()

    def step_reference(self, users, pos, neg, loss_out, masks=None, plan=None, dropped=False):
        B, N, U = users.numel(), self.N, self.n_users
        if B > self.max_batch:
            raise ValueError("batch larger than max_batch")
        if not dropped:
            self._drop_nodes()
        self.forward_reference(masks)
        rows = self.rows[:3 * B]
        E.lightgcn_mark_batch(users, pos, neg, U, rows, self.flag)
        E.bpr_mf_grad(self.Out[:U], self.Out[U:], users, pos, neg, self.reg, self.dOut[:U], self.dOut[U:], self.terms,
                      loss_out, plan)
        dego = None
        for k in range(self.L - 1, -1, -1):
            wi, wo, pi, po = self.w[k], self.w[k + 1], self.wp[k], self.wp[k + 1]
            Wg, bg, Wb, bb = self.W[k]
            gWg, gbg, gWb, gbb = self.gW[k]
            dblock = self.dOut[:, self.off[k + 1]:self.off[k + 2]]
            call("nrhip_ngcf_act_bwd", C.c_void_p(dblock.data_ptr()), self.dsum, _ptr(dego, allow_none=True), po,
                 _ptr(self.ego[k + 1]), po, _ptr(self.T1[k]), _ptr(self.T2[k]), wo, _ptr(self.mask[k], torch.uint8), N,
                 wo, float(self.keep), _ptr(self.dT1), _ptr(self.dT2), _stream())
            self._gemm(self.S[k], pi, 0, self.dT1, wo, 0, wi, wo, N, gWg, wo, splits=self.splits)
            self._gemm(self.X2[k], pi, 0, self.dT2, wo, 0, wi, wo, N, gWb, wo, splits=self.splits)
            call("nrhip_colsum_rows", _ptr(self.dT1), wo, N, wo, _ptr(gbg), _ptr(self.cs_ws), self.cs_ws.numel() * 4, _stream())
            call("nrhip_colsum_rows", _ptr(self.dT2), wo, N, wo, _ptr(gbb), _ptr(self.cs_ws), self.cs_ws.numel() * 4, _stream())
            self._gemm(self.dT1, wo, 1, Wg, wo, 1, N, wi, wo, self.Y1, wi)
            self._gemm(self.dT2, wo, 1, Wb, wo, 1, N, wi, wo, self.Y2, wi)
            dS, dEd = self._buf(self.dS, pi), self._buf(self.dEd, pi)
            call("nrhip_ngcf_mix_bwd", _ptr(self.Y1), _ptr(self.Y2), wi, _ptr(self.ego[k]), _ptr(self.S[k]), pi, N, wi,
                 pi, _ptr(dS), _ptr(dEd), _stream())
            nxt = self._buf(self.dEgo[k % 2], pi)
            self.At.matmul(dS, out=nxt, addend=dEd)
            dego = nxt
        w0 = self.w[0]
        if dego is None:
            E.copy2d(self.dOut[:, :w0], self.gE0[:, :w0])
        else:
            E.add2d(self.dOut[:, :w0], dego[:, :w0], self.gE0[:, :w0])
        tensors = [(self.E0p, self.mE, self.vE, self.gE0)] + \
            [(w, m, v, g) for k in range(self.L) for w, m, v, g in zip(self.W[k], self.mW[k], self.vW[k], self.gW[k])]
        if self.learner is None:
            E.adam_dense_multi(tensors, self.adam)
        else:
            self.learner.apply(tensors)
        E.rows_clear(rows, self.dsum, (self.dOut,), self.flag)
        self.adam.advance()

    def _act(self, T, wo, po, k, flags, out_a, out_b, masks_given):
        call("nrhip_lrelu_drop_fwd", _ptr(T), wo, self.N, wo, po, float(self.keep), _ptr(self.mask[k], torch.uint8),
             1 if masks_given else 0, C.c_uint64(self.seed & (2**64 - 1)), C.c_uint64(self.t), k, flags,
             _ptr(out_a, allow_none=True), po, None if out_b is None else C.c_void_p(out_b.data_ptr()), self.dsum, _stream())

    def _forward_variant(self, masks=None):
        N, gcmc = self.N, self.alg == "gcmc"
        if not gcmc:
            E.copy2d(self.E0, self.Out[:, :self.w[0]])
        for k in range(self.L):
            wi, wo, pi, po = self.w[k], self.w[k + 1], self.wp[k], self.wp[k + 1]
            Wg, bg, Wx, bx = self.W[k]
            self.A.matmul(self.ego[k], out=self.S[k])
            self._gemm(self.S[k], pi, 1, Wg, wo, 0, N, wo, wi, self.T1[k], wo, bias=bg)
            if masks is not None:
                self.mask[k].copy_(masks[k])
            block = self.Out[:, self.off[k + 1]:self.off[k + 2]]
            if not gcmc:
                self._act(self.T1[k], wo, po, k, 3, self.ego[k + 1], block, masks is not None)
            else:
                self._act(self.T1[k], wo, po, k, 1, self.ego[k + 1], None, False)
                self._gemm(self.ego[k + 1], po, 1, Wx, wo, 0, N, wo, wo, self.T2[k], wo, bias=bx)
                self._act(self.T2[k], wo, po, k, 2, None, block, masks is not None)
        self.t += 1
        return self.Out

    def _step_variant(self, users, pos, neg, loss_out, masks=None, plan=None):
        B, N, U, gcmc = users.numel(), self.N, self.n_users, self.alg == "gcmc"
        if B > self.max_batch:
            raise ValueError("batch larger than max_batch")
        self._forward_variant(masks)
        rows = self.rows[:3 * B]
        E.lightgcn_mark_batch(users, pos, neg, U, rows, self.flag)
        E.bpr_mf_grad(self.Out[:U], self.Out[U:], users, pos, neg, self.reg, self.dOut[:U], self.dOut[U:], self.terms,
                      loss_out, plan)
        bwd = lambda da, lda, db, ldb, T, k, flags, dT, wo: call(
            "nrhip_lrelu_drop_bwd", C.c_void_p(da.data_ptr()), lda, _ptr(db, allow_none=True), ldb, _ptr(T), wo,
            _ptr(self.mask[k], torch.uint8), N, wo, float(self.keep), flags, _ptr(dT), _stream())
        colsum = lambda src, wo, dst: call("nrhip_colsum_rows", _ptr(src), wo, N, wo, _ptr(dst), _ptr(self.cs_ws),
                                           self.cs_ws.numel() * 4, _stream())
        dego = None
        for k in range(self.L - 1, -1, -1):
            wi, wo, pi, po = self.w[k], self.w[k + 1], self.wp[k], self.wp[k + 1]
            Wg, bg, Wx, bx = self.W[k]
            gWg, gbg, gWx, gbx = self.gW[k]
            dblock = self.dOut[:, self.off[k + 1]:self.off[k + 2]]
            if not gcmc:
                bwd(dblock, self.dsum, dego, po, self.T1[k], k, 3, self.dT1, wo)
            else:
                bwd(dblock, self.dsum, None, 0, self.T2[k], k, 2, self.dT2, wo)
                self._gemm(self.ego[k + 1], po, 0, self.dT2, wo, 0, wo, wo, N, gWx, wo, splits=self.splits)
                colsum(self.dT2, wo, gbx)
                self._gemm(self.dT2, wo, 1, Wx, wo, 1, N, wo, wo, self.Y2, wo)
                y2 = self.Y2[:N * wo].view(N, wo)
                bwd(y2, wo, dego, po, self.T1[k], k, 1, self.dT1, wo)
            self._gemm(self.S[k], pi, 0, self.dT1, wo, 0, wi, wo, N, gWg, wo, splits=self.splits)
            colsum(self.dT1, wo, gbg)
            self._gemm(self.dT1, wo, 1, Wg, wo, 1, N, wi, wo, self.Y1, wi)
            dS = self._buf(self.dS, pi)
            E.copy2d(self.Y1[:N * wi].view(N, wi), dS[:, :wi])
            nxt = self._buf(self.dEgo[k % 2], pi)
            self.At.matmul(dS, out=nxt)
            dego = nxt
        w0 = self.w[0]
        if gcmc:
            E.copy2d(dego[:, :w0], self.gE0[:, :w0])
        elif dego is None:
            E.copy2d(self.dOut[:, :w0], self.gE0[:, :w0])
        else:
            E.add2d(self.dOut[:, :w0], dego[:, :w0], self.gE0[:, :w0])
        used = (0, 1) if not gcmc else (0, 1, 2, 3)
        tensors = [(self.E0p, self.mE, self.vE, self.gE0)] + \
            [(self.W[k][j], self.mW[k][j], self.vW[k][j], self.gW[k][j]) for k in range(self.L) for j in used]
        if self.learner is None:
            E.adam_dense_multi(tensors, self.adam)
        else:
            self.learner.apply(tensors)
        E.rows_clear(rows, self.dsum, (self.dOut,), self.flag)
        self.adam.advance()
```

Before: 5.599 million triplets/s.

## Pack blocked SpMM values as factored row/column codes in index words

When the adjacency values factor exactly as row_factor*col_factor (as with the symmetric D^-1/2 A D^-1/2 normalisation), the pack step encodes a column-factor code into the high bits of each column index word and stores one row factor per entry. The SpMM kernel then rebuilds each value from an LDS table instead of loading a separate per-nonzero value array. This removes one 4-byte stream per nonzero from the gather loop. In exchange it adds host-side factor detection, a bit-exact device verification pass, extra plan memory, LDS for the table and a multiply per nonzero.

Measured after the change: 5.716 million triplets/s, median of 6. 2.1% higher.

```diff
diff --git a/include/neurec_hip.h b/include/neurec_hip.h
--- a/include/neurec_hip.h
+++ b/include/neurec_hip.h
@@ -214,6 +214,11 @@
 int nrhip_spmm_blocked_tune(int gathers_in_flight);
 int nrhip_spmm_blocked_tune_store(int masked_store);
 int nrhip_spmm_blocked_pack(void* plan, const int32_t* d_indices, const float* d_vals, void* stream);
+int nrhip_spmm_blocked_pack_factored(void* plan, const int32_t* d_indices, const float* d_vals,
+                                     const float* h_row_factor, const float* h_col_factor, int64_t n_cols,
+                                     void* stream, int* packed);
+int nrhip_spmm_blocked_is_packed(const void* plan);
+int nrhip_spmm_blocked_tune_packed(int on);
 int nrhip_spmm_blocked(const void* plan, const int32_t* d_indices, const float* d_vals,
                        const float* d_X, float* d_Y, const float* d_addend, const float* d_sum_in,
                        float* d_sum_out, const uint8_t* d_x_row_nonzero,
diff --git a/neurec_amd/_lib.py b/neurec_amd/_lib.py
--- a/neurec_amd/_lib.py
+++ b/neurec_amd/_lib.py
@@ -336,6 +336,9 @@
                              p, sz, p],
     "nrhip_spmm_blocked_plan_bytes": [i64, i64, i32, psz],
     "nrhip_spmm_blocked_pack": [p, p, p, p],
+    "nrhip_spmm_blocked_pack_factored": [p, p, p, p, p, i64, p, C.POINTER(i32)],
+    "nrhip_spmm_blocked_is_packed": [p],
+    "nrhip_spmm_blocked_tune_packed": [i32],
     "nrhip_spmm_blocked_plan_create": [p, p, i64, i64, i32, i64, i32, i32, i32, i32, i32, p, sz, p,
                                        C.POINTER(p)],
     "nrhip_spmm_blocked_plan_destroy": [p],
diff --git a/neurec_amd/build.py b/neurec_amd/build.py
--- a/neurec_amd/build.py
+++ b/neurec_amd/build.py
@@ -18,7 +18,8 @@
 FILE_FLAGS = {"score_i8.hip": ["-mllvm", "-amdgpu-mfma-vgpr-form"]}
 EXP_SOURCES = ["experiments/gather_experiments.hip"]
 EXP_LIB_PATH = os.path.join(HERE, "libneurec_exp.so")
-HEADERS = ["nr_core.h", "nr_common.h", "history_common.h", "spmm_blocked_plan.h", "spmm_wanted_plan.h"]
+HEADERS = ["nr_core.h", "nr_common.h", "history_common.h", "spmm_blocked_plan.h", "spmm_blocked_factor.h",
+           "spmm_wanted_plan.h"]
 
 HIPCC = os.environ.get("HIPCC", "/opt/rocm/bin/hipcc")
 FLAGS = ["-O3", "--offload-arch=gfx950", "-std=c++17", "-fPIC", "-ffp-contract=off",
diff --git a/neurec_amd/csrc/spmm_blocked.hip b/neurec_amd/csrc/spmm_blocked.hip
--- a/neurec_amd/csrc/spmm_blocked.hip
+++ b/neurec_amd/csrc/spmm_blocked.hip
@@ -1,5 +1,6 @@
 #include "nr_common.h"
 #include "spmm_blocked_plan.h"
+#include "spmm_blocked_factor.h"
 #include "spmm_wanted_plan.h"
 #include <algorithm>
 #include <new>
@@ -16,6 +17,7 @@
 
 struct BlockedPlan : nr_plan::PlanArrays<int4> {
   int64_t n_rows, nnz, n_ent, n_cmb;
+  int pk_on, pk_codes, pk_col_bits;
   int n_wg, n_phases;
   int seg, r_max, p_max, waves, d;
   const int32_t* pk_from_idx;
@@ -56,6 +58,12 @@
 };
 
 
+static_assert(nr_plan::kMaxFactorCodes == 16 * NR_WAVE, "a 16-wave workgroup stages the factor table one entry per thread");
+struct PackedNz {
+  const uint32_t* word; const float* ent_rf; const float* table;
+  int n_codes, col_bits;
+};
+
 constexpr int kRowBits = 0x7FFFFFFF;
 constexpr int kRowUnflagged = (int)0x80000000u;
 
@@ -135,7 +143,7 @@
     const float4* __restrict__ X, float4* __restrict__ Y, const float4* __restrict__ addend,
     const float4* sum_in, float4* sum_out, const uint8_t* __restrict__ col_mask,
     const uint8_t* __restrict__ row_mask, int kRMax, AdamEpilogue ad, const int32_t* __restrict__ row_of,
-    int kPMax, const uint8_t* __restrict__ addend_flag) {
+    int kPMax, const uint8_t* __restrict__ addend_flag, PackedNz pk) {
   constexpr int LPR = D / 4;
   constexpr int GPW = NR_WAVE / LPR;
   constexpr int kGroups = kWaves * GPW;
@@ -149,6 +157,17 @@
   NR_BLK_STAMP(0);
   const int r0 = wg_row0[wg], nr = wg_nrows[wg];
   int32_t* s_rows = (int32_t*)(s_acc + (size_t)(kRMax + kPMax) * LPR);
+  const bool packed = pk.word != nullptr;
+  if (packed) indices = (const int32_t*)pk.word;
+  float* s_tab = (float*)(s_rows + kRMax);
+  const uint32_t cmask = (1u << pk.col_bits) - 1u;
+  constexpr int kTabPer = nr_plan::kMaxFactorCodes / (kWaves * NR_WAVE);
+  float tab_v[kTabPer];
+#pragma unroll
+  for (int j = 0; j < kTabPer; ++j) {
+    tab_v[j] = 0.f;
+    if (packed && tid + j * kWaves * NR_WAVE < pk.n_codes) tab_v[j] = pk.table[tid + j * kWaves * NR_WAVE];
+  }
   const uint8_t* fl = ADAM ? ad.flag_rw : addend_flag;
   for (int i = tid; i < nr; i += kWaves * NR_WAVE) {
     int row = row_of[r0 + i];
@@ -156,6 +175,9 @@
     s_rows[i] = row;
   }
   for (int i = tid; i < nr * LPR; i += kWaves * NR_WAVE) s_acc[i] = make_float4(0.f, 0.f, 0.f, 0.f);
+#pragma unroll
+  for (int j = 0; j < kTabPer; ++j)
+    if (packed && tid + j * kWaves * NR_WAVE < pk.n_codes) s_tab[tid + j * kWaves * NR_WAVE] = tab_v[j];
   __syncthreads();
   NR_BLK_STAMP(1);
   const int32_t* eoff = wg_ent_off + (int64_t)wg * (n_phases + 1);
@@ -164,7 +186,11 @@
     const int e0 = eoff[k], e1 = eoff[k + 1];
     int ei = e0 + wave * GPW + g;
     int4 cur = make_int4(0, 0, 0, 0);
-    if (ei < e1) cur = ent[ei];
+    float cur_rf = 0.f;
+    if (ei < e1) {
+      cur = ent[ei];
+      if (packed) cur_rf = pk.ent_rf[ei];
+    }
     int cur_idx[IPL];
     float cur_val[IPL];
 #pragma unroll
@@ -173,7 +199,7 @@
       cur_val[i] = 0.f;
       if (c < CL && c * IPL + i < cur.y) {
         cur_idx[i] = indices[(uint32_t)cur.z + c * IPL + i];
-        cur_val[i] = vals[(uint32_t)cur.z + c * IPL + i];
+        if (!packed) cur_val[i] = vals[(uint32_t)cur.z + c * IPL + i];
       }
     }
     int cur_want = 1;
@@ -184,7 +210,11 @@
       const bool live = ei < e1;
       const int ein = ei + kGroups;
       int4 nxt = make_int4(0, 0, 0, 0);
-      if (ein < e1) nxt = ent[ein];
+      float nxt_rf = 0.f;
+      if (ein < e1) {
+        nxt = ent[ein];
+        if (packed) nxt_rf = pk.ent_rf[ein];
+      }
       const int slot = cur.x;
       int len = cur.y;
       const uint32_t begin = (uint32_t)cur.z;
@@ -213,6 +243,11 @@
         for (int i = 0; i < IPL; ++i) {
           my_idx[i] = k0 == 0 ? cur_idx[i] : ch_idx[i];
           my_val[i] = k0 == 0 ? cur_val[i] : ch_val[i];
+          if (packed) {
+            const uint32_t w = (uint32_t)my_idx[i];
+            my_idx[i] = (int)(w & cmask);
+            my_val[i] = __fmul_rn(cur_rf, s_tab[w >> pk.col_bits]);
+          }
           if constexpr (MASKED) {
             if (col_mask && c < CL && k0 + c * IPL + i < len && col_mask[my_idx[i]] == 0)
               my_idx[i] = -1;
@@ -245,7 +280,7 @@
               ch_val[i] = 0.f;
               if (c < CL && k0 + 16 + c * IPL + i < len) {
                 ch_idx[i] = indices[begin + k0 + 16 + c * IPL + i];
-                ch_val[i] = vals[begin + k0 + 16 + c * IPL + i];
+                if (!packed) ch_val[i] = vals[begin + k0 + 16 + c * IPL + i];
               }
             }
           }
@@ -254,7 +289,7 @@
             for (int i = 0; i < IPL; ++i)
               if (c < CL && c * IPL + i < nxt.y) {
                 nxt_idx[i] = indices[(uint32_t)nxt.z + c * IPL + i];
-                nxt_val[i] = vals[(uint32_t)nxt.z + c * IPL + i];
+                if (!packed) nxt_val[i] = vals[(uint32_t)nxt.z + c * IPL + i];
               }
             if constexpr (MASKED) {
               if (row_mask && ein < e1) nxt_want = row_mask[nxt.w];
@@ -272,6 +307,7 @@
       }
       if (live) s_acc[slot * LPR + c] = acc;
       cur = nxt;
+      cur_rf = nxt_rf;
 #pragma unroll
       for (int i = 0; i < IPL; ++i) { cur_idx[i] = nxt_idx[i]; cur_val[i] = nxt_val[i]; }
       cur_want = nxt_want;
@@ -1077,6 +1113,15 @@
 constexpr int kMaskedStoreDefault = kStoreWt;
 int s_addend_by_flag = 1;
 int s_masked_store = kMaskedStoreDefault;
+int s_packed = 1;
+
+PackedNz packed_for(const BlockedPlan* p, size_t lds, size_t* extra_lds) {
+  *extra_lds = 0;
+  const size_t tab = (size_t)p->pk_codes * 4;
+  if (!p->pk_on || !s_packed || lds + tab > (size_t)kMaxLdsBytes) return PackedNz{nullptr, nullptr, nullptr, 0, 0};
+  *extra_lds = tab;
+  return PackedNz{p->pk_word, p->ent_rf, p->pk_table, p->pk_codes, p->pk_col_bits};
+}
 
 __global__ __launch_bounds__(256) void row_order_pack_kernel(const uint32_t* __restrict__ src, const uint32_t* __restrict__ dst,
                                                              int64_t n_rows, const int32_t* __restrict__ indices,
@@ -1092,12 +1137,48 @@
   }
 }
 
+__global__ __launch_bounds__(256) void row_order_pack_words_kernel(
+    const uint32_t* __restrict__ src, const uint32_t* __restrict__ dst, const int32_t* __restrict__ row_of,
+    int64_t n_rows, int64_t n_cols, const int32_t* __restrict__ indices, const float* __restrict__ vals,
+    const uint16_t* __restrict__ code, const float* __restrict__ table, int col_bits, uint32_t* __restrict__ pk_word,
+    uint32_t* __restrict__ bad) {
+  const int c = threadIdx.x & 15;
+  bool miss = false;
+  for (int64_t k = (int64_t)blockIdx.x * 16 + (threadIdx.x >> 4); k < n_rows; k += (int64_t)gridDim.x * 16) {
+    const uint32_t s0 = src[k], d0 = dst[k], len = dst[k + 1] - d0;
+    const float rf = table[code[row_of[k]]];
+    for (uint32_t j = c; j < len; j += 16) {
+      const int32_t col = indices[s0 + j];
+      uint32_t w = 0;
+      if (col < 0 || col >= n_cols) {
+        miss = true;
+      } else {
+        const uint32_t cc = code[n_rows + col];
+        if (__float_as_uint(__fmul_rn(rf, table[cc])) != __float_as_uint(vals[s0 + j])) miss = true;
+        w = (uint32_t)col | (cc << col_bits);
+      }
+      pk_word[d0 + j] = w;
+    }
+  }
+  if (miss) *bad = 1u;
+}
+
+__global__ __launch_bounds__(256) void entry_row_factor_kernel(const int4* __restrict__ ent, int64_t n_ent,
+                                                               const uint16_t* __restrict__ code,
+                                                               const float* __restrict__ table,
+                                                               float* __restrict__ ent_rf) {
+  for (int64_t e = (int64_t)blockIdx.x * 256 + threadIdx.x; e < n_ent; e += (int64_t)gridDim.x * 256)
+    ent_rf[e] = table[code[ent[e].w]];
+}
+
 static hipError_t allow_plan_lds(const BlockedPlan* p) {
   hipError_t e = hipSuccess;
   auto allow = [&](const void* fn, size_t lds) {
     if (e == hipSuccess) e = hipFuncSetAttribute(fn, hipFuncAttributeMaxDynamicSharedMemorySize, (int)lds);
   };
-  const size_t lds = (size_t)(p->r_max + p->p_max) * p->d * 4 + (size_t)p->r_max * 4;
+  const size_t tab = (size_t)nr_plan::kMaxFactorCodes * 4;
+  size_t lds = (size_t)(p->r_max + p->p_max) * p->d * 4 + (size_t)p->r_max * 4;
+  if (lds + tab <= (size_t)kMaxLdsBytes) lds += tab;
 #define NR_ALLOW(DD)                                                                                                         \
   allow((const void*)spmm_blocked_kernel<false, 16, 8, DD>, lds); allow((const void*)spmm_blocked_kernel<true, 16, 8, DD>, lds); \
   allow((const void*)spmm_blocked_kernel<false, 16, 4, DD>, lds); allow((const void*)spmm_blocked_kernel<true, 16, 4, DD>, lds); \
@@ -1164,6 +1245,8 @@
   opt.masked_fast = !(env && env[0] == '0');
   env = getenv("NEUREC_SPMM_WANTED_WAVE");
   opt.wanted_wave = !(env && env[0] == '0');
+  env = getenv("NEUREC_SPMM_PACKED");
+  if (env) s_packed = env[0] != '0';
   env = getenv("NEUREC_SPMM_WANTED_NNZ_CAP");
   opt.wanted_nnz_cap = env ? std::max(atoi(env), 1) : 0;
 
@@ -1184,6 +1267,7 @@
   p->wp_ok = h.ww_ok && opt.seg == nr_wplan::kSeg && n_rows <= nr_wplan::kMaxRows && !(env && env[0] == '0');
   if (p->wp_ok) p->wp_profile = nr_wplan::slot_profile(h_indptr, n_rows);
   std::vector<nr_plan::Section> sections = nr_plan::plan_sections(*p, h);
+  for (const nr_plan::Section& fs : nr_plan::factor_sections(*p, h)) sections.push_back(fs);
   const size_t used = nr_plan::carve_sections(&sections, d_plan_buf);
   if (used > plan_bytes) {
     delete p;
@@ -1219,6 +1303,50 @@
   }
   p->pk_from_idx = d_indices;
   p->pk_from_val = d_vals;
+  p->pk_on = 0;
+  return NR_OK;
+}
+
+int nrhip_spmm_blocked_pack_factored(void* plan, const int32_t* d_indices, const float* d_vals,
+                                     const float* h_row_factor, const float* h_col_factor, int64_t n_cols,
+                                     void* stream, int* packed) {
+  if (packed) *packed = 0;
+  NR_TRY(nrhip_spmm_blocked_pack(plan, d_indices, d_vals, stream));
+  BlockedPlan* p = (BlockedPlan*)plan;
+  if (!h_row_factor || !h_col_factor || p->nnz == 0 || n_cols <= 0 || n_cols > p->n_rows) return NR_OK;
+  nr_plan::FactorLayout lay;
+  nr_plan::Error err;
+  if (nr_plan::factor_layout(h_row_factor, p->n_rows, h_col_factor, n_cols, &lay, &err) != nr_plan::kOk) return NR_OK;
+  hipStream_t st = (hipStream_t)stream;
+  const uint32_t zero = 0;
+  NR_CHECK_HIP(hipMemcpyAsync(p->pk_table, lay.table.data(), lay.table.size() * 4, hipMemcpyHostToDevice, st));
+  NR_CHECK_HIP(hipMemcpyAsync(p->pk_code, lay.row_code.data(), (size_t)p->n_rows * 2, hipMemcpyHostToDevice, st));
+  NR_CHECK_HIP(hipMemcpyAsync(p->pk_code + p->n_rows, lay.col_code.data(), (size_t)n_cols * 2, hipMemcpyHostToDevice, st));
+  NR_CHECK_HIP(hipMemcpyAsync(p->pk_bad, &zero, 4, hipMemcpyHostToDevice, st));
+  const unsigned blocks = (unsigned)std::min<int64_t>((p->n_rows + 15) / 16, 8192);
+  hipLaunchKernelGGL(row_order_pack_words_kernel, dim3(blocks), dim3(256), 0, st, p->pk_src, p->pk_dst, p->row_of,
+                     p->n_rows, n_cols, d_indices, d_vals, p->pk_code, p->pk_table, lay.col_bits, p->pk_word, p->pk_bad);
+  NR_LAUNCH_CHECK();
+  hipLaunchKernelGGL(entry_row_factor_kernel, dim3((unsigned)std::min<int64_t>((p->n_ent + 255) / 256, 8192)),
+                     dim3(256), 0, st, p->ent, p->n_ent, p->pk_code, p->pk_table, p->ent_rf);
+  NR_LAUNCH_CHECK();
+  uint32_t bad = 1;
+  NR_CHECK_HIP(hipMemcpyAsync(&bad, p->pk_bad, 4, hipMemcpyDeviceToHost, st));
+  NR_CHECK_HIP(hipStreamSynchronize(st));
+  if (bad) return NR_OK;
+  p->pk_codes = (int)lay.table.size();
+  p->pk_col_bits = lay.col_bits;
+  p->pk_on = 1;
+  if (packed) *packed = 1;
+  return NR_OK;
+}
+
+int nrhip_spmm_blocked_is_packed(const void* plan) {
+  return plan && ((const BlockedPlan*)plan)->pk_on ? 1 : 0;
+}
+
+int nrhip_spmm_blocked_tune_packed(int on) {
+  s_packed = on ? 1 : 0;
   return NR_OK;
 }
 
@@ -1333,12 +1461,14 @@
     NR_LAUNCH_CHECK();
     return NR_OK;
   }
+  size_t tab_lds = 0;
+  const PackedNz pk = packed_for(p, lds, &tab_lds);
 #define NR_BLK(M, W, GG, DD)                                                                       \
-  hipLaunchKernelGGL((spmm_blocked_kernel<M, W, GG, DD>), grid, block, lds, st, p->wg_row0,        \
+  hipLaunchKernelGGL((spmm_blocked_kernel<M, W, GG, DD>), grid, block, lds + tab_lds, st, p->wg_row0, \
                      p->wg_nrows, p->wg_ent_off, p->wg_cmb_off, p->ent, p->cmb, p->n_phases,        \
                      p->pk_idx, p->pk_val, (const float4*)d_X, (float4*)d_Y, (const float4*)d_addend, \
                      (const float4*)d_sum_in, (float4*)d_sum_out, d_x_row_nonzero, d_y_row_wanted,  \
-                     p->r_max, AdamEpilogue{}, p->row_of, p->p_max, addend_flag)
+                     p->r_max, AdamEpilogue{}, p->row_of, p->p_max, addend_flag, pk)
 #define NR_BLK_D(DD)                                                                               \
   if (p->waves == 16) {                                                                            \
     if (masked) { if (gif == 4) NR_BLK(true, 16, 4, DD); else NR_BLK(true, 16, 8, DD); }           \
@@ -1495,12 +1625,14 @@
                   alpha, 1.0f - beta1, 1.0f - beta2, eps,
                   clear_consumed ? (float4*)d_addend : nullptr,
                   clear_consumed ? (float4*)d_grad_b : nullptr, clear_consumed ? d_row_flag : nullptr};
+  size_t tab_lds = 0;
+  const PackedNz pk = packed_for(p, lds, &tab_lds);
   hipLaunchKernelGGL((spmm_blocked_kernel<false, 16, 8, 64, true>), dim3((unsigned)p->n_wg),
-                     dim3(16 * NR_WAVE), lds, (hipStream_t)stream, p->wg_row0, p->wg_nrows,
+                     dim3(16 * NR_WAVE), lds + tab_lds, (hipStream_t)stream, p->wg_row0, p->wg_nrows,
                      p->wg_ent_off, p->wg_cmb_off, p->ent, p->cmb, p->n_phases, p->pk_idx, p->pk_val,
                      (const float4*)d_X, (float4*)nullptr, (const float4*)d_addend,
                      (const float4*)nullptr, (float4*)nullptr, (const uint8_t*)nullptr,
-                     (const uint8_t*)nullptr, p->r_max, ad, p->row_of, p->p_max, (const uint8_t*)nullptr);
+                     (const uint8_t*)nullptr, p->r_max, ad, p->row_of, p->p_max, (const uint8_t*)nullptr, pk);
   NR_LAUNCH_CHECK();
   return NR_OK;
 }
diff --git a/neurec_amd/csrc/spmm_blocked_factor.h b/neurec_amd/csrc/spmm_blocked_factor.h
--- /dev/null
+++ b/neurec_amd/csrc/spmm_blocked_factor.h
@@ -0,0 +1,59 @@
+#pragma once
+#include <stdint.h>
+#include <string.h>
+#include <algorithm>
+#include <vector>
+#include "spmm_blocked_plan.h"
+
+namespace nr_plan {
+
+constexpr int kMaxFactorCodes = kPlanFactorCodes;
+constexpr uint32_t kDroppedWord = 0xFFFFFFFFu;
+
+struct FactorLayout {
+  int col_bits = 0;
+  uint32_t col_mask = 0;
+  std::vector<float> table;
+  std::vector<uint16_t> row_code, col_code;
+};
+
+inline uint32_t factor_bits(float f) { uint32_t u; memcpy(&u, &f, 4); return u; }
+inline uint32_t factor_word(const FactorLayout& l, int64_t col, uint16_t code) {
+  return (uint32_t)col | ((uint32_t)code << l.col_bits);
+}
+inline int64_t factor_word_col(const FactorLayout& l, uint32_t w) { return (int64_t)(w & l.col_mask); }
+inline uint32_t factor_word_code(const FactorLayout& l, uint32_t w) { return w >> l.col_bits; }
+
+inline int factor_layout(const float* row_factor, int64_t n_rows, const float* col_factor, int64_t n_cols,
+                         FactorLayout* out, Error* err) {
+  NR_PLAN_REQUIRE(row_factor && col_factor && out && n_rows > 0 && n_cols > 0, kErrArg, "factor_layout: bad arguments");
+  NR_PLAN_REQUIRE(n_cols <= ((int64_t)1 << 31), kErrUnsupported, "factor_layout: %lld columns", (long long)n_cols);
+  std::vector<uint32_t> bits;
+  bits.reserve((size_t)(n_rows + n_cols));
+  for (int64_t r = 0; r < n_rows; ++r) bits.push_back(factor_bits(row_factor[r]));
+  for (int64_t c = 0; c < n_cols; ++c) bits.push_back(factor_bits(col_factor[c]));
+  std::vector<uint32_t> uniq(bits);
+  std::sort(uniq.begin(), uniq.end());
+  uniq.erase(std::unique(uniq.begin(), uniq.end()), uniq.end());
+  NR_PLAN_REQUIRE((int64_t)uniq.size() <= kMaxFactorCodes, kErrUnsupported,
+                  "factor_layout: %lld distinct factors > %d", (long long)uniq.size(), kMaxFactorCodes);
+  int cb = 1;
+  while (((int64_t)1 << cb) < n_cols) ++cb;
+  NR_PLAN_REQUIRE((uint64_t)uniq.size() < ((uint64_t)1 << (32 - cb)), kErrUnsupported,
+                  "factor_layout: %lld codes do not fit the %d bits beside a %d-bit column", (long long)uniq.size(),
+                  32 - cb, cb);
+  out->col_bits = cb;
+  out->col_mask = (uint32_t)(((uint64_t)1 << cb) - 1);
+  out->table.resize(uniq.size());
+  memcpy(out->table.data(), uniq.data(), uniq.size() * 4);
+  out->row_code.resize((size_t)n_rows);
+  out->col_code.resize((size_t)n_cols);
+  for (int64_t i = 0; i < n_rows + n_cols; ++i) {
+    const uint16_t code = (uint16_t)(std::lower_bound(uniq.begin(), uniq.end(), bits[(size_t)i]) - uniq.begin());
+    if (i < n_rows) out->row_code[(size_t)i] = code;
+    else out->col_code[(size_t)(i - n_rows)] = code;
+  }
+  return kOk;
+}
+
+}
diff --git a/neurec_amd/csrc/spmm_blocked_plan.h b/neurec_amd/csrc/spmm_blocked_plan.h
--- a/neurec_amd/csrc/spmm_blocked_plan.h
+++ b/neurec_amd/csrc/spmm_blocked_plan.h
@@ -16,6 +16,7 @@
 constexpr int kPMaxDefault = 192;
 constexpr int kMaxPhases = 32;
 constexpr int kMaxLdsBytes = 160 * 1024;
+constexpr int kPlanFactorCodes = 1024;
 constexpr int kWaveChunk = 8;
 
 struct Int4 { int32_t x, y, z, w; };
@@ -446,6 +447,11 @@
   int32_t* wg_row0; int32_t* wg_nrows;
   int32_t* row_of; uint32_t* pk_src; uint32_t* pk_dst;
   int32_t* pk_idx; float* pk_val;
+  uint32_t* pk_word;
+  float* ent_rf;
+  float* pk_table;
+  uint16_t* pk_code;
+  uint32_t* pk_bad;
   int32_t* wg_ent_off; int32_t* wg_cmb_off;
   uint32_t* wg_nnz;
   I4* w_ent; I4* w_cmb; int32_t* w_ent_off; int32_t* w_cmb_off;
@@ -505,6 +511,17 @@
   return s;
 }
 
+template <class I4>
+std::vector<Section> factor_sections(PlanArrays<I4>& p, const Plan& h) {
+  return {
+      section(p.pk_word, nullptr, (size_t)h.nnz * 4, 4),
+      section(p.ent_rf, nullptr, h.ent.size() * 4, 4),
+      section(p.pk_table, nullptr, (size_t)kPlanFactorCodes * 4),
+      section(p.pk_code, nullptr, (size_t)h.n_rows * 4),
+      section(p.pk_bad, nullptr, 4, 0, true),
+  };
+}
+
 inline size_t carve_sections(std::vector<Section>* sections, void* base) {
   size_t off = 0;
   for (Section& s : *sections) {
@@ -526,7 +543,9 @@
                     2 * align_up(max_cmb * 16 + 16, 256)  +
                     align_up(ww_seg * 256 + 256, 256)  + align_up(max_cmb * 4 + 4, 256) ;
   const size_t dealt = 3 * align_up(((size_t)n_rows + 1) * 4, 256)  +
-                       2 * align_up((size_t)nnz * 4 + 4, 256) ;
+                       3 * align_up((size_t)nnz * 4 + 4, 256)  +
+                       align_up(max_ent * 4 + 4, 256)  + align_up((size_t)kPlanFactorCodes * 4, 256) +
+                       align_up((size_t)n_rows * 4, 256)  + 256 ;
   return ww + dealt + align_up(max_ent * 16, 256)  + align_up(max_cmb * 16, 256)  +
          3 * align_up(wg * 8, 256)  +
          2 * align_up(wg * (kMaxPhases + 1) * 4, 256)  +
diff --git a/neurec_amd/engine.py b/neurec_amd/engine.py
--- a/neurec_amd/engine.py
+++ b/neurec_amd/engine.py
@@ -4,7 +4,10 @@
 import numpy as np
 import torch
 
+import scipy.sparse as _sp
+
 from . import _lib
+from . import graph as _graph
 from ._lib import call
 
 NGCF_MAX_LAYERS = _lib.NGCF_MAX_LAYERS
@@ -780,6 +783,9 @@
     call("nrhip_div_scalar", _ptr(x), float(denom), _ptr(out), x.numel(), _stream())
 
 
+_UNSET = object()
+
+
 class SpmmCSR:
 
     def __init__(self, indptr, indices, vals, n_cols=None, item_rows=0, item_nnz=0, split_row=0):
@@ -790,11 +796,15 @@
             self.indices = indices.to(dev, torch.int32).contiguous()
             self.vals = vals.to(dev, torch.float32).contiguous()
             self._h_indices = None
+            self._host_built = False
         else:
             self.h_indptr = np.ascontiguousarray(indptr, dtype=np.int64)
             idx = np.ascontiguousarray(indices, dtype=np.int32)
             val = np.ascontiguousarray(vals, dtype=np.float32)
             self._h_indices = idx
+            self._host_built = True
+            self._h_factors = _UNSET
+            self._h_vals = val
             self.indices = torch.from_numpy(idx if len(idx) else np.zeros(1, np.int32)).to(dev)
             self.vals = torch.from_numpy(val if len(val) else np.zeros(1, np.float32)).to(dev)
             self.indptr = torch.from_numpy(self.h_indptr).to(dev)
@@ -857,17 +867,38 @@
                          self.h_indices.ctypes.data_as(C.c_void_p), self.n_rows, self.split_row, d,
                          0, 0, 0, 0, 0, 0, _ptr(buf), buf.numel(), _stream(), C.byref(plan))
                     call("nrhip_spmm_plan_attach_blocked", self.plan, plan, d)
-                    call("nrhip_spmm_blocked_pack", plan, _ptr(self.indices), _ptr(self.vals), _stream())
+                    self._pack(plan)
                     self._blocked[d] = (plan, buf)
                 except NotImplementedError:
                     pass
         self.blocked = self._blocked[d][0]
         return self.blocked is not None
 
-    def values_changed(self):
+    def _pack(self, plan):
+        if self._host_built and self._h_factors is _UNSET:
+            self._h_factors = _graph.factor_values(
+                _sp.csr_matrix((self._h_vals, self._h_indices, self.h_indptr), shape=(self.n_rows, self.n_cols))) \
+                if self.nnz > 0 and self.n_cols <= self.n_rows else None
+            self._h_vals = None
+        if not self._host_built or self._h_factors is None:
+            call("nrhip_spmm_blocked_pack", plan, _ptr(self.indices), _ptr(self.vals), _stream())
+            return
+        rf, cf = (np.ascontiguousarray(f, dtype=np.float32) for f in self._h_factors)
+        call("nrhip_spmm_blocked_pack_factored", plan, _ptr(self.indices), _ptr(self.vals),
+             rf.ctypes.data_as(C.c_void_p), cf.ctypes.data_as(C.c_void_p), self.n_cols, _stream(), None)
+
+    def is_packed(self, d):
+        return bool(self.ensure_schedule(d) and _lib.lib.nrhip_spmm_blocked_is_packed(self.blocked))
+
+    def values_changed(self, factor=True):
+        if self._host_built:
+            self._h_factors = None
+            if factor and any(plan is not None and plan.value for plan, _buf in self._blocked.values()):
+                self._h_vals = self.vals[:self.nnz].cpu().numpy()
+                self._h_factors = _UNSET
         for plan, _buf in self._blocked.values():
             if plan is not None and plan.value:
-                call("nrhip_spmm_blocked_pack", plan, _ptr(self.indices), _ptr(self.vals), _stream())
+                self._pack(plan)
 
     def exact_row_nnz(self, d):
         return 64 if self.ensure_schedule(d) else 256
diff --git a/neurec_amd/graph.py b/neurec_amd/graph.py
--- a/neurec_amd/graph.py
+++ b/neurec_amd/graph.py
@@ -78,6 +78,35 @@
     return t
 
 
+def factor_values(csr):
+    a = csr.tocsr()
+    n_rows, n_cols = a.shape
+    indptr = np.asarray(a.indptr, dtype=np.int64)
+    vals = np.ascontiguousarray(a.data, dtype=np.float32)
+    if len(vals) == 0 or len(vals) != indptr[-1]:
+        return None
+    bits = vals.view(np.uint32)
+    lens = np.diff(indptr)
+    row_of = np.repeat(np.arange(n_rows), lens)
+    cols = np.asarray(a.indices, dtype=np.int64)
+
+    def accepted(rf, cf):
+        with np.errstate(invalid="ignore", over="ignore"):
+            prod = (rf[row_of] * cf[cols]).astype(np.float32)
+        return np.array_equal(prod.view(np.uint32), bits)
+
+    rf = np.zeros(n_rows, np.float32)
+    rf[lens > 0] = vals[indptr[:-1][lens > 0]]
+    cf = np.ones(n_cols, np.float32)
+    if accepted(rf, cf):
+        return rf, cf
+    if n_rows == n_cols:
+        dinv = _inv_power(lens.astype(np.float32), np.float32(-0.5)).astype(np.float32)
+        if accepted(dinv, dinv):
+            return dinv, dinv.copy()
+    return None
+
+
 def is_symmetric(a):
     return (a != a.T).nnz == 0
 
diff --git a/neurec_amd/ngcf_wide.py b/neurec_amd/ngcf_wide.py
--- a/neurec_amd/ngcf_wide.py
+++ b/neurec_amd/ngcf_wide.py
@@ -197,8 +197,8 @@
              1 if given is not None else 0, C.c_uint64(self.seed & (2**64 - 1)), C.c_uint64(self.t), _ptr(self.A.vals),
              _stream())
         call("nrhip_gather_f32", _ptr(self.A.vals), _ptr(self._t_of, torch.int32), n, _ptr(self.At.vals), _stream())
-        self.A.values_changed()
-        self.At.values_changed()
+        self.A.values_changed(factor=False)
+        self.At.values_changed(factor=False)
 
     def step(self, users, pos, neg, loss_out, masks=None, plan=None, node_keep_given=None):
         if self.alg != "ngcf":
```
